# CloudNativeDataPlane/cndp

Measured on AMD Instinct MI355X. Metric: Mpps device-resident parse+hash+LPM, 64B & IMIX, at 1/2/4/8 MI355X, higher is better.
Workload: dtype u32; 1 GPU; C3 l3fwd-graph: 64B IPv4/UDP, 1024-prefix DIR-24-8 LPM + Toeplitz + RSS queue, 16M pkts/GPU device-resident; config=c3, packets_per_gpu=16777216, frame_layout=packed 64-B slots, frame_memory=torch tensor (hipMalloc), ring_batches=4, routes=1024, parallelism=dp1 (replicated FIB, sharded batches), bins_total=32665239552

## Files before the change

__graft_entry__.py:

```python
from __future__ import annotations

import os
import subprocess
import sys

ROOT = os.path.dirname(os.path.abspath(__file__))


def build() -> None:
    env = dict(os.environ)
    env.setdefault("PYTORCH_ROCM_ARCH", "gfx950")
    jobs = str(min(16, os.cpu_count() or 4))
    subprocess.run(["make", "-j", jobs, "-C", os.path.join(ROOT, "cndp_amd", "csrc"), "ARCH=gfx950"],
                   check=True, env=env)
    subprocess.run(["make", "-C", os.path.join(ROOT, "oracle")], check=True, env=env)
    subprocess.run(["make", "-C", os.path.join(ROOT, "tests", "node_harness")], check=True, env=env)
    subprocess.run(["make", "-C", os.path.join(ROOT, "tests", "c_link")], check=True, env=env)
    subprocess.run(["make", "-C", os.path.join(ROOT, "tests", "l4_host")], check=True, env=env)
    subprocess.run(["make", "-C", os.path.join(ROOT, "tests", "tcp_host")], check=True, env=env)
    subprocess.run(["make", "-C", os.path.join(ROOT, "tests", "fwd_host")], check=True, env=env)
    subprocess.run(["make", "-C", os.path.join(ROOT, "tests", "tx_host")], check=True, env=env)
    subprocess.run(["make", "-C", os.path.join(ROOT, "tests", "tcb_host")], check=True, env=env)
    subprocess.run(["make", "-C", os.path.join(ROOT, "tests", "tcpout_host")], check=True, env=env)
    if ROOT not in sys.path:
        sys.path.insert(0, ROOT)
    import cndp_amd
    from cndp_amd import native
    native.lib()
    print(f"built {native.LIB_PATH} ({native.lib().cndp_gpu_version().decode()}); "
          f"cndp_amd {cndp_amd.__version__}")


def smoke() -> None:
    if ROOT not in sys.path:
        sys.path.insert(0, ROOT)
    import numpy as np
    import torch

    from cndp_amd import pktgen
    from cndp_amd.classify import Classifier
    from cndp_amd.fib import Fib, node_ip4_route_add
    from cndp_amd import native as N
    from oracle import oracle as O

    assert torch.cuda.is_available(), "smoke() needs a GPU"
    dev = torch.device("cuda:0")
    routes = pktgen.l3fwd_routes()
    fib = Fib("smoke", N.CNE_FIB_DIR24_8, default_nh=N.IP4_LOOKUP_NEXT_PKT_DROP << 16,
              max_routes=1024, nh_sz=N.CNE_FIB_DIR24_8_4B, num_tbl8=256)
    for ip, d, nh in routes:
        assert node_ip4_route_add(fib, ip, d, nh, N.IP4_LOOKUP_NEXT_REWRITE) == 0
    cl = Classifier(0)
    cl.set_fib(fib)
    n = 1 << 16
    fr = pktgen.packed_ipv4(n, routes=routes, device=dev)
    out = cl.classify(fr, N.CNDP_MODE_L3FWD, n_bins=64)
    torch.cuda.synchronize()

    r4 = [(ip, d, nh) for ip, d, nh in routes]
    t24, t8 = O.dir24_8_build(r4, N.IP4_LOOKUP_NEXT_PKT_DROP << 16, 256)
    ref = O.classify(O.MODE_L3FWD, fr.slab.cpu().numpy(), n, stride=64, tables4=(t24, t8), n_bins=64)
    got = {k: out[k].cpu().numpy() for k in ("nh", "hash", "queue", "edge", "bins")}
    for k, dt in (("nh", np.uint32), ("hash", np.uint32), ("queue", np.uint16), ("edge", np.uint8),
                  ("bins", np.uint64)):
        g = got[k].view(dt) if got[k].dtype != dt else got[k]
        if not np.array_equal(g, ref[k]):
            bad = int(np.sum(g != ref[k]))
            raise AssertionError(f"smoke: {k} differs from the oracle in {bad} places")
    print(f"smoke OK: {n} packets, l3fwd classify on {torch.cuda.get_device_name(0)} == oracle")

    from cndp_amd.l4 import PcbTable, seg_records
    tbl = PcbTable(4)
    assert tbl.add(laddr=0x0A040001, lport=80) == 0
    assert tbl.add(laddr=0x0A040001, lport=80, faddr=0xC6120001, fport=40000) == 1
    m = 64
    ft = pktgen.tcp_socket_frames(m, [((0x0A040001, 80), (0xC6120001, 40000)), ((0x0A040001, 80), (0xC6120002, 7))],
                                  seed=2, cksum=("ok", "ok", "ok", "bad"), flags=(0x02,), payload_lens=(0, 5),
                                  device=dev)
    rx = torch.full((m,), 14 | 20 << 7, dtype=torch.int32, device=dev)
    t = cl.tcp_input(ft, {"rxmeta": rx}, tbl, sel=torch.ones(m, dtype=torch.uint8, device=dev))
    torch.cuda.synchronize()
    raw = ft.slab.cpu().numpy().reshape(m, -1)
    edge, pcb, st = t["l4edge"].cpu().numpy(), t["pcb"].cpu().numpy().view(np.uint32), t["stats"].cpu().numpy()
    seg = seg_records(t["seg"])
    for i in range(m):
        f = raw[i].tobytes()
        l4 = int.from_bytes(f[16:18], "big") - 20
        data = f[26:34] + bytes([0, 6]) + l4.to_bytes(2, "big") + f[34:34 + l4]
        data += b"\0" * (len(data) & 1)
        c = sum(int.from_bytes(data[k:k + 2], "big") for k in range(0, len(data), 2))
        while c >> 16:
            c = (c >> 16) + (c & 0xFFFF)
        want = (0x21, 1 if f[29] == 1 else 0, int.from_bytes(f[38:42], "big")) if c == 0xFFFF else (0x20, 0xFFFFFFFF, 0)
        have = (int(edge[i]), int(pcb[i]), int(seg["seq"][i]))
        if have != want:
            raise AssertionError(f"smoke: tcp_input frame {i}: got {have} want {want}")
    assert st[0] + st[2] == m and st[0] > 0 and st[2] > 0 and st[1] == st[3] == st[4] == 0, st
    print(f"smoke OK: {m} TCP segments, tcp_input: {int(st[0])} to their connection or listener, {int(st[2])} bad checksums")

    from cndp_amd.l4 import TcbTable, opt_records

    def tcp_frame(src, sport, seq, ack, flags, wnd, opts=b"", payload=b""):
        ones = lambda b: sum(int.from_bytes(b[k:k + 2], "big") for k in range(0, len(b), 2)) % 0xFFFF
        seg = bytearray(sport.to_bytes(2, "big") + (80).to_bytes(2, "big") + seq.to_bytes(4, "big") + ack.to_bytes(4, "big")
                        + bytes([(5 + len(opts) // 4) << 4, flags]) + wnd.to_bytes(2, "big") + bytes(4) + opts + payload)
        ip = bytearray(bytes([0x45, 0]) + (20 + len(seg)).to_bytes(2, "big") + bytes(4) + bytes([64, 6, 0, 0])
# ... 105 lines not shown
```

cndp_amd/classify.py:

```python
from __future__ import annotations

import ctypes

import numpy as np

from . import native as N


class Classifier:
    def __init__(self, device: int = -1):
        self._L = N.lib()
        h = ctypes.c_void_p()
        N.check(self._L.cndp_gpu_init(device, ctypes.byref(h)), "cndp_gpu_init")
        self.h = h
        self.device = self._L.cndp_gpu_device(h)
        self.reta_size = 128
        self.fib4 = None
        self.fib6 = None

    def close(self):
        if self.h:
            self._L.cndp_gpu_fini(self.h)
            self.h = None

    def __del__(self):
        try:
            self.close()
        except Exception:
            pass

    def set_rss(self, key: bytes | None = None, reta=None, nb_queues: int = 16):
        rarr = None
        size = 0
        if reta is not None:
            rarr = np.ascontiguousarray(reta, dtype=np.uint16)
            size = len(rarr)
        N.check(self._L.cndp_gpu_set_rss(self.h, key, len(key) if key else 0,
                                         rarr.ctypes.data if rarr is not None else None, size,
                                         nb_queues), "cndp_gpu_set_rss")
        self.reta_size = size or 128

    def set_tuning(self, nt: int | None = None, unroll: int | None = None,
                   blocks_per_cu: int | None = None, tile: int | None = None,
                   dir16: int | None = None, cnet_tile: int | None = None,
                   host_chunk: int | None = None, rw_wb: int | None = None,
                   cnet_spec: int | None = None, load_nt: int | None = None,
                   spec_scan: int | None = None, mbuf_hash: int | None = None,
                   cnet_fold: int | None = None, spec_grid: int | None = None,
                   spec_lists: int | None = None, spec_types: int | None = None,
                   stream_bal: int | None = None, spec_wait: int | None = None,
                   host_window: int | None = None):
        for key, v in ((N.CNDP_TUNE_CNET_FOLD, cnet_fold), (N.CNDP_TUNE_SPEC_GRID, spec_grid),
                       (N.CNDP_TUNE_SPEC_WAIT, spec_wait), (N.CNDP_TUNE_HOST_WINDOW, host_window),
                       (N.CNDP_TUNE_SPEC_LISTS, spec_lists), (N.CNDP_TUNE_SPEC_TYPES, spec_types),
                       (N.CNDP_TUNE_STREAM_BAL, stream_bal),
                       (N.CNDP_TUNE_NT, nt), (N.CNDP_TUNE_UNROLL, unroll),
                       (N.CNDP_TUNE_BLOCKS_PER_CU, blocks_per_cu), (N.CNDP_TUNE_TILE, tile),
                       (N.CNDP_TUNE_DIR16, dir16), (N.CNDP_TUNE_CNET_TILE, cnet_tile),
                       (N.CNDP_TUNE_HOST_CHUNK, host_chunk), (N.CNDP_TUNE_RW_WB, rw_wb),
                       (N.CNDP_TUNE_CNET_SPEC, cnet_spec), (N.CNDP_TUNE_LOAD_NT, load_nt),
                       (N.CNDP_TUNE_SPEC_SCAN, spec_scan), (N.CNDP_TUNE_MBUF_HASH, mbuf_hash)):
            if v is not None:
                N.check(self._L.cndp_gpu_set_tuning(self.h, key, int(v)), "cndp_gpu_set_tuning")

    def stat(self, key: int) -> int:
        self._L.cndp_gpu_get_stat.restype = ctypes.c_int64
        return int(N.check(self._L.cndp_gpu_get_stat(self.h, key), "cndp_gpu_get_stat"))

    def set_fib(self, fib4=None, fib6=None):
        N.check(self._L.cndp_gpu_set_fib(self.h, fib4.h if fib4 else None, fib6.h if fib6 else None),
                "cndp_gpu_set_fib")
        self.fib4, self.fib6 = fib4, fib6

    def alloc_outputs(self, n: int, n_bins: int = 64, device=None, edge: bool = True, meta: bool = False):
        import torch
        dev = device if device is not None else f"cuda:{self.device}"
        out = {
            "nh": torch.empty(n, dtype=torch.int32, device=dev),
            "hash": torch.empty(n, dtype=torch.int32, device=dev),
            "queue": torch.empty(n, dtype=torch.int16, device=dev),
            "edge": torch.empty(n, dtype=torch.uint8, device=dev) if edge else None,
            "bins": torch.zeros(n_bins + 2, dtype=torch.int64, device=dev),
            "n_bins": n_bins,
        }
        if meta:
            out["ptype"] = torch.empty(n, dtype=torch.int32, device=dev)
            out["rxmeta"] = torch.empty(n, dtype=torch.int32, device=dev)
        return out

    @staticmethod
    def _ptr(t):
        return t.data_ptr() if t is not None else None

    def batch(self, frames, mode: int, out: dict, buf_len: int = 1984, offsets_t=None) -> "N.Batch":
        b = N.Batch()
        b.mode = mode
        b.n = frames.n
        b.slab = frames.slab.data_ptr()
        b.slab_len = frames.slab.numel()
        b.stride = frames.stride
        off = offsets_t if offsets_t is not None else frames.offsets
        b.offsets = off.data_ptr() if off is not None else None
        b.data_off = frames.data_off
        b.buf_len = buf_len
        b.nh = self._ptr(out.get("nh"))
        b.hash = self._ptr(out.get("hash"))
        b.queue = self._ptr(out.get("queue"))
        b.edge = self._ptr(out.get("edge"))
        b.bins = self._ptr(out.get("bins"))
        b.n_bins = out.get("n_bins", 64)
        b.ptype = self._ptr(out.get("ptype"))
        b.rxmeta = self._ptr(out.get("rxmeta"))
        return b

    def classify(self, frames, mode: int = N.CNDP_MODE_L3FWD, out: dict | None = None,
                 n_bins: int = 64, buf_len: int = 1984, stream: int | None = None) -> dict:
        import torch
        if out is None:
            out = self.alloc_outputs(frames.n, n_bins, device=frames.slab.device)
        if stream is None:
            stream = torch.cuda.current_stream(frames.slab.device).cuda_stream
        b = self.batch(frames, mode, out, buf_len)
        N.check(self._L.cndp_gpu_classify(self.h, ctypes.byref(b), stream or None), "cndp_gpu_classify")
        return out

    def stream_release(self, stream: int) -> None:
        N.check(self._L.cndp_gpu_stream_release(self.h, stream or None), "cndp_gpu_stream_release")

    @staticmethod
    def _hptr(x):
        if x is None:
            return None
        if isinstance(x, np.ndarray):
            return x.ctypes.data
        return x.data_ptr()

    def classify_host(self, slab, n: int, mode: int, stride: int = 64, offsets=None,
                      data_off: int = 0, buf_len: int = 1984, n_bins: int = 64, out: dict | None = None,
# ... 225 lines not shown
```

cndp_amd/csrc/cndp_gpu.hip:

```cpp

#include <hip/hip_runtime.h>

#include <algorithm>
#include <atomic>
#include <errno.h>
#include <pthread.h>
#include <sched.h>
#include <stdint.h>
#include <stdio.h>
#include <stdlib.h>
#include <string.h>
#include <time.h>
#include <vector>

#include "fib_internal.h"
#include "node_internal.h"
#include "../../include/cndp_gpu.h"
#include "../../include/cndp_l4.h"

#define CNDP_VERSION "cndp_amd 0.1 (gfx950)"

#define HIP_TRY(expr)                                                                            \
    do {                                                                                         \
        hipError_t e_ = (expr);                                                                  \
// ... 56 lines not shown
        e = t8[(e >> 1) * 256u + (ip & 0xffu)];
    return e >> 1;
}

template <typename TP>
__device__ __forceinline__ uint32_t tz4(TP tab, uint32_t b, uint32_t x)
{
    return tab[(b + 0) * 256 + (x & 0xffu)] ^ tab[(b + 1) * 256 + ((x >> 8) & 0xffu)] ^
           tab[(b + 2) * 256 + ((x >> 16) & 0xffu)] ^ tab[(b + 3) * 256 + (x >> 24)];
}

template <typename TP>
__device__ __forceinline__ uint32_t tz4n(TP tab, uint32_t b, uint32_t x)
{
    uint32_t h = 0;
#pragma unroll
    for (uint32_t j = 0; j < 4; j++) {
        const uint32_t v = (x >> (8 * j)) & 0xffu, q = 2 * (b + j);
        h ^= tab[q * 16 + (v >> 4)] ^ tab[(q + 1) * 16 + (v & 15u)];
    }
    return h;
}

#define CNDP_RW_MAX_NH CNDP_IP4_REWRITE_MAX_NH
#define CNDP_RW_MAX_LEN CNDP_IP4_REWRITE_MAX_LEN
#define CNDP_RW_MAX_PORTS CNDP_IP4_REWRITE_MAX_PORTS

typedef uint32_t u32x4 __attribute__((ext_vector_type(4)));
typedef uint32_t u32x4a4 __attribute__((ext_vector_type(4), aligned(4)));
typedef uint32_t u32x3a4 __attribute__((ext_vector_type(3), aligned(4)));
typedef uint32_t u32x2a4 __attribute__((ext_vector_type(2), aligned(4)));
typedef uint32_t u32x2 __attribute__((ext_vector_type(2)));

struct KArgs {
    const uint8_t *slab;
    uint64_t slab_len;
    uint64_t stride;
    const uint64_t *offsets;
    uint32_t data_off;
    uint32_t n;
    uint32_t buf_len;
    uint32_t reta_mask;
    const uint32_t *tbl24;
    const uint32_t *tbl8;
    const uint32_t *tbl24_6;
    const uint32_t *tbl8_6;
    const uint32_t *dir16;
    const uint32_t *pages;
    const uint32_t *ttab;
    const uint16_t *reta;
    uint32_t *nh;
    uint32_t *hash;
    uint16_t *queue;
    uint8_t *edge;
    unsigned long long *bins;
    uint32_t n_bins;
    uint32_t *ptype;
    uint32_t *rxmeta;
    uint32_t *iplen;
    u32x4 *win;
    uint32_t *spec_nh;
    uint32_t *spec_flags;
    uint16_t *spec_t16;
    uint32_t *wl;
    uint32_t *wl_n;
    uint32_t *spec_meta;
    uint8_t *spec_cls;
    uint32_t *spec_ticket;
    uint32_t *spec_bar;
    uint8_t *spec_tile;
    uint32_t *spec_cwl;
    uint32_t *spec_cflag;
    uint32_t *spec_hint;
    uint32_t spec_B;
    uint32_t wl_fold;
    uint32_t tail_lo;
    uint32_t spec_allow;
    uint8_t *spec_c2;
    uint32_t spec_codes;
    uint32_t spec_keep_lo;
    const struct cndp_rw_nh *rw_tbl;
    uint16_t *tx_edge;
    uint32_t rw_parts;
};

#define FAST_THREADS 256
#define SPEC_CH_K 4
#define SPEC_MX 135
#define SPEC_PTRS 151
#define SPEC_ALLOW_LISTS 2u
__device__ __forceinline__ bool nh_ready_rw(uint32_t v) { return v != 0xFFFFFFFFu && (v >> 16) == 0u; }
#define TAB4_POS 12
#define TAB_POS 36
#define TABN_OFF (TAB_POS * 256)
#define TAB_WORDS (TABN_OFF + 2 * TAB_POS * 16)

template <int MODE>
__device__ __forceinline__ uint32_t bin_of(uint32_t nh, uint32_t edge, uint32_t q, uint32_t nb)
{
    if (MODE == CNDP_MODE_HASH)
        return q < nb ? q : nb + 1;
    if (MODE == CNDP_MODE_L3FWD) {
        if (edge == 0)
            return (nh & 0xffffu) < nb ? (nh & 0xffffu) : nb + 1;
        return (edge == 1 || edge == 0xFFu) ? nb : nb + 1;
    }
    if (edge == 1)
        return (nh & 0xffffffu) < nb ? (nh & 0xffffffu) : nb + 1;
    return (edge == 0 || edge == 0x80u) ? nb : nb + 1;
}

__device__ uint32_t hash_v6_global(const uint8_t *p, uint64_t avail, uint32_t ip, bool l4,
                                   const uint32_t *__restrict__ ttab)
{
    const GAS uint32_t *gt = (const GAS uint32_t *)ttab;
    uint32_t h = 0;
    for (uint32_t k = 0; k < 8; k++)
        h ^= tz4(gt, 4 * k, gld32(p, avail, ip + 8 + 4 * k));
    if (l4)
        h ^= tz4(gt, 32, gld32(p, avail, ip + 40));
    return h;
}


template <typename T>
__device__ __forceinline__ GAS T *gp(T *p)
{
    return (GAS T *)p;
}
template <typename T>
__device__ __forceinline__ const GAS T *gp(const T *p)
{
    return (const GAS T *)p;
}

template <bool NT>
__device__ __forceinline__ u32x4 ldg4(const uint8_t *p)
{
    if (NT)
        return __builtin_nontemporal_load(gp((const u32x4 *)p));
    return *gp((const u32x4 *)p);
}
template <bool NT>
__device__ __forceinline__ u32x2 ldg2(const uint8_t *p)
{
    if (NT)
        return __builtin_nontemporal_load(gp((const u32x2 *)p));
    return *gp((const u32x2 *)p);
}
template <bool NT, typename T>
__device__ __forceinline__ void stg(T *p, T v)
{
    if (NT)
        __builtin_nontemporal_store(v, gp(p));
    else
        *p = v;
}

struct FastHdr {
    const uint8_t *p;
    uint64_t avail;
    uint32_t w3, w5, w6, w7, w8, w9;
};

template <bool NT>
__device__ __forceinline__ void fast_load(const KArgs &a, uint64_t i, FastHdr &h)
// ... 415 lines not shown
                nb.hs ^= tz4(s_t, 8, alignb(h.w9, h.w8, 2));
            else
                slow = true;
        }
    }
    if (slow)
        nb.hs = fast_hash<MODE>(a, h, s_t);
    {
        const u32x4 *g = (const u32x4 *)(base + (cn < n_tiles ? cn : n_tiles - 1u) * 4096u);
        r[P][0] = ldg4<LNT>((const uint8_t *)(g + lane));
        r[P][1] = ldg4<LNT>((const uint8_t *)(g + 64 + lane));
        r[P][2] = ldg4<LNT>((const uint8_t *)(g + 128 + lane));
        r[P][3] = ldg4<LNT>((const uint8_t *)(g + 192 + lane));
    }
    if (dD)
        fast_emit<MODE, NTS>(a, cd * 64u + lane, etD, nhD, hsD, s_reta, s_bins, count);
    sd = nd;
    sc = nc;
    sb = nb;
}

template <int MODE, bool NTS, bool LNT>
__global__ __launch_bounds__(FAST_THREADS) void k_classify_stream(KArgs a, uint64_t n_tiles)
{
    __shared__ uint32_t s_t[TAB4_POS * 256];
    __shared__ uint16_t s_reta[CNDP_RETA_MAX];
    __shared__ uint32_t s_bins[CNDP_BINS_MAX + 2];
    __shared__ __attribute__((aligned(16))) u32x4 s_tile[TILE_WAVES][256];

    const uint32_t tid = threadIdx.x;
    for (uint32_t k = tid; k < TAB4_POS * 256; k += FAST_THREADS)
        s_t[k] = a.ttab[k];
    for (uint32_t k = tid; k <= a.reta_mask; k += FAST_THREADS)
        s_reta[k] = a.reta[k];
    const bool count = a.bins != nullptr;
    if (count)
        for (uint32_t k = tid; k < a.n_bins + 2; k += FAST_THREADS)
            s_bins[k] = 0;
    __syncthreads();

    const uint32_t lane = tid & 63u, wv = tid >> 6;
    u32x4 *tile = s_tile[wv];
    const uint8_t *base = a.slab + a.data_off;
    const uint64_t wstep = (uint64_t)gridDim.x * TILE_WAVES;
    const uint64_t t0 = (uint64_t)blockIdx.x * TILE_WAVES + wv;
    const uint64_t nt_w = t0 < n_tiles ? (n_tiles - t0 + wstep - 1) / wstep : 0;
    u32x4 r[2][4];
#pragma unroll
    for (uint32_t s = 0; s < 2; s++) {
        const uint64_t ts = t0 + s * wstep;
        const u32x4 *g = (const u32x4 *)(base + (ts < n_tiles ? ts : n_tiles - 1u) * 4096u);
        r[s][0] = ldg4<LNT>((const uint8_t *)(g + lane));
        r[s][1] = ldg4<LNT>((const uint8_t *)(g + 64 + lane));
        r[s][2] = ldg4<LNT>((const uint8_t *)(g + 128 + lane));
        r[s][3] = ldg4<LNT>((const uint8_t *)(g + 192 + lane));
    }
    StreamLane sb = {0, 0, 0, 0, 0, false}, sc = sb, sd = sb;
    const uint64_t trips = nt_w ? nt_w + 3 : 0;
    for (uint64_t j = 0; j < trips; j += 2) {
        stream_trip<MODE, NTS, LNT, 0>(a, n_tiles, t0 + j * wstep, t0 + (j + 2) * wstep, t0 + (j - 3) * wstep,
                                       j >= 3 && j - 3 < nt_w, lane, tile, r, sb, sc, sd, s_t, s_reta, s_bins, count);
        if (j + 1 < trips)
            stream_trip<MODE, NTS, LNT, 1>(a, n_tiles, t0 + (j + 1) * wstep, t0 + (j + 3) * wstep,
                                           t0 + (j - 2) * wstep, j >= 2 && j - 2 < nt_w, lane, tile, r, sb, sc, sd,
                                           s_t, s_reta, s_bins, count);
    }
    const uint64_t done = n_tiles * 64u;
    for (uint64_t i = done + (uint64_t)blockIdx.x * FAST_THREADS + tid; i < a.n;
         i += (uint64_t)gridDim.x * FAST_THREADS) {
        FastHdr h;
        fast_load<false>(a, i, h);
        fast_finish<MODE, false>(a, i, h, s_t, s_reta, s_bins, count);
    }
    if (count) {
        __syncthreads();
        for (uint32_t k = tid; k < a.n_bins + 2; k += FAST_THREADS)
            if (s_bins[k])
                atomicAdd(&a.bins[k], (unsigned long long)s_bins[k]);
    }
}


#define STREAM_BW 8
template <int MODE, bool NTS, bool LNT>
__global__ __launch_bounds__(STREAM_BW * 64) void k_classify_stream_bal(KArgs a, uint64_t n_tiles)
{
    __shared__ uint32_t s_t[TAB4_POS * 256];
    __shared__ uint16_t s_reta[CNDP_RETA_MAX];
    __shared__ uint32_t s_bins[CNDP_BINS_MAX + 2];
    __shared__ __attribute__((aligned(16))) u32x4 s_tile[STREAM_BW][256];
    __shared__ uint32_t s_next;
    constexpr uint32_t NT = STREAM_BW * 64;

    const uint32_t tid = threadIdx.x;
    for (uint32_t k = tid; k < TAB4_POS * 256; k += NT)
        s_t[k] = a.ttab[k];
    for (uint32_t k = tid; k <= a.reta_mask; k += NT)
        s_reta[k] = a.reta[k];
    const bool count = a.bins != nullptr;
    if (count)
        for (uint32_t k = tid; k < a.n_bins + 2; k += NT)
            s_bins[k] = 0;
    if (tid == 0)
        s_next = 3u * STREAM_BW;
    const uint32_t lane = tid & 63u, wv = tid >> 6;
    u32x4 *tile = s_tile[wv];
    const uint8_t *base = a.slab + a.data_off;
    const uint64_t G = gridDim.x, b = blockIdx.x;
    const uint64_t NONE = ~0ull;
    const uint64_t nk = b < n_tiles ? (n_tiles - b + G - 1) / G : 0;
    auto tile_of = [&](uint64_t k) { return k < nk ? b + k * G : NONE; };
    uint64_t q0 = tile_of(wv), q1 = tile_of(wv + STREAM_BW), q2 = tile_of(wv + 2u * STREAM_BW);
    u32x4 r[2][4];
#pragma unroll
    for (uint32_t s = 0; s < 2; s++) {
        const uint64_t ts = s ? q1 : q0;
        const u32x4 *g = (const u32x4 *)(base + (ts < n_tiles ? ts : n_tiles - 1u) * 4096u);
        r[s][0] = ldg4<LNT>((const uint8_t *)(g + lane));
        r[s][1] = ldg4<LNT>((const uint8_t *)(g + 64 + lane));
        r[s][2] = ldg4<LNT>((const uint8_t *)(g + 128 + lane));
        r[s][3] = ldg4<LNT>((const uint8_t *)(g + 192 + lane));
    }
    __syncthreads();
    auto draw = [&](uint64_t prev) -> uint32_t {
        uint32_t v = 0;
        if (prev != NONE && lane == 0)
            v = atomicAdd(&s_next, 1u);
        return v;
    };
    uint32_t kv = draw(q2);
    uint64_t h1 = NONE, h2 = NONE, h3 = NONE;
    StreamLane sb = {0, 0, 0, 0, 0, false}, sc = sb, sd = sb;
    for (;;) {
        if (q0 == NONE && h1 == NONE && h2 == NONE && h3 == NONE)
            break;
        stream_trip<MODE, NTS, LNT, 0>(a, n_tiles, q0, q2, h3, h3 != NONE, lane, tile, r, sb, sc, sd, s_t, s_reta,
                                       s_bins, count);
        {
            const uint64_t qn = q2 == NONE ? NONE : tile_of(__builtin_amdgcn_readfirstlane(kv));
            kv = draw(qn);
            h3 = h2;
            h2 = h1;
            h1 = q0;
            q0 = q1;
            q1 = q2;
            q2 = qn;
        }
        if (q0 == NONE && h1 == NONE && h2 == NONE && h3 == NONE)
            break;
        stream_trip<MODE, NTS, LNT, 1>(a, n_tiles, q0, q2, h3, h3 != NONE, lane, tile, r, sb, sc, sd, s_t, s_reta,
                                       s_bins, count);
        {
            const uint64_t qn = q2 == NONE ? NONE : tile_of(__builtin_amdgcn_readfirstlane(kv));
            kv = draw(qn);
            h3 = h2;
            h2 = h1;
            h1 = q0;
            q0 = q1;
            q1 = q2;
            q2 = qn;
        }
    }
    const uint64_t done = n_tiles * 64u;
    for (uint64_t i = done + (uint64_t)blockIdx.x * NT + tid; i < a.n; i += (uint64_t)gridDim.x * NT) {
        FastHdr h;
        fast_load<false>(a, i, h);
        fast_finish<MODE, false>(a, i, h, s_t, s_reta, s_bins, count);
    }
    if (count) {
        __syncthreads();
        for (uint32_t k = tid; k < a.n_bins + 2; k += NT)
            if (s_bins[k])
                atomicAdd(&a.bins[k], (unsigned long long)s_bins[k]);
    }
}

#define CNET_THREADS 512
#define WIN_DW 16
#define ROW_DW 17

struct Win {
    const uint32_t *row;
    const uint8_t *g;
    uint64_t avail;
    __device__ __forceinline__ uint32_t ld32(uint32_t o) const
    {
        if (o + 4 <= 64) {
            const uint32_t lo = row[o >> 2], hi = row[(o >> 2) + 1];
            return alignb(hi, lo, o & 3u);
        }
        return gld32(g, avail, o);
    }
    __device__ __forceinline__ uint32_t b8(uint32_t o) const
    {
        return o < 64 ? (row[o >> 2] >> ((o & 3u) * 8)) & 0xffu : gbyte(g, avail, o);
    }
    __device__ __forceinline__ uint32_t raw16(uint32_t o) const { return ld32(o) & 0xffffu; }
    __device__ __forceinline__ uint32_t be16(uint32_t o) const { return bswap16(ld32(o) & 0xffffu); }
    __device__ __forceinline__ uint32_t be32(uint32_t o) const { return bswap32(ld32(o)); }
};

#define BE16C(x) ((uint32_t)((((x) & 0xffu) << 8) | (((x) >> 8) & 0xffu)))

struct Lens {
    uint32_t l2, l3, l4;
};

__device__ __forceinline__ uint32_t pt_l3_ip(uint32_t vihl)
{
    return vihl == 0x45u ? 0x10u : (vihl >= 0x46u && vihl <= 0x4fu) ? 0x30u : 0u;
}
__device__ __forceinline__ uint32_t pt_l4(uint32_t p)
{
    return (p == 17u ? 0x200u : 0u) | (p == 6u ? 0x100u : 0u) | (p == 132u ? 0x400u : 0u);
}
__device__ __forceinline__ bool v6_ext(uint32_t p)
{
    return p == 0u || p == 43u || p == 44u || p == 50u || p == 51u || p == 60u;
}


template <class W>
__device__ int skip_v6_ext(const W &w, uint32_t proto, uint32_t &off, int &frag)
{
    frag = 0;
    for (int i = 0; i < 5; i++) {
        if (proto == 0u || proto == 43u || proto == 60u) {
            const uint32_t x = w.ld32(off);
            proto = x & 0xffu;
            off += (((x >> 8) & 0xffu) + 1u) * 8u;
        } else if (proto == 44u) {
            proto = w.b8(off);
            off += 8;
            frag = 1;
            return (int)proto;
        } else if (proto == 59u) {
            return 0;
        } else {
            return (int)proto;
        }
    }
    return -1;
}

// ... 2751 lines not shown
                s_wave[q] = acc;
                acc += t;
            }
        }
        __syncthreads();
        const uint32_t excl = s_carry + s_wave[wv] + x - v;
        if (k < total) {
            hist[k] = excl;
            if (k % tiles == 0)
                bin_start[k / tiles] = excl;
        }
        __syncthreads();
        if (threadIdx.x == 1023)
            s_carry = excl + v;
        __syncthreads();
    }
    if (threadIdx.x == 0)
        bin_start[nbt] = s_carry;
}

__global__ __launch_bounds__(PART_THREADS) void k_part_scatter(const uint16_t *__restrict__ bin_of,
                                                               uint32_t n, uint32_t nbt,
                                                               uint32_t tiles,
                                                               const uint32_t *__restrict__ off,
                                                               uint32_t *__restrict__ order)
{
    __shared__ uint32_t cur[CNDP_PART_BINS_MAX + 2];
    for (uint32_t k = threadIdx.x; k < nbt; k += PART_THREADS)
        cur[k] = off[(uint64_t)k * tiles + blockIdx.x];
    __syncthreads();
    const uint32_t lane = threadIdx.x & 63u, wv = threadIdx.x >> 6;
    const uint64_t lt_mask = lane ? (~0ULL >> (64 - lane)) : 0ULL;
    const uint32_t t0 = blockIdx.x * PART_TILE;
    for (uint32_t chunk = 0; chunk < PART_TILE; chunk += PART_THREADS) {
        for (uint32_t turn = 0; turn < PART_THREADS / 64u; turn++) {
            if (wv == turn) {
                const uint32_t i = t0 + chunk + threadIdx.x;
                const bool valid = i < n;
                const uint32_t b = valid ? bin_of[i] : 0xFFFFFFFFu;
                uint64_t todo = __ballot(valid);
                uint32_t dst = 0;
                while (todo) {
                    const uint32_t leader = (uint32_t)__builtin_ctzll(todo);
                    const uint32_t lb = __shfl(b, leader, 64);
                    const uint64_t peers = __ballot(valid && b == lb);
                    const uint32_t cnt = (uint32_t)__builtin_popcountll(peers);
                    uint32_t basev = 0;
                    if (lane == leader)
                        basev = cur[lb];
                    basev = __shfl(basev, leader, 64);
                    if (b == lb && valid)
                        dst = basev + (uint32_t)__builtin_popcountll(peers & lt_mask);
                    if (lane == leader)
                        cur[lb] = basev + cnt;
                    todo &= ~peers;
                }
                if (valid)
                    order[dst] = i;
            }
            __syncthreads();
        }
    }
}

#define CNDP_MAX_REGIONS 16
struct cndp_gpu_ctx {
    int dev;
    uint32_t *mq_iplen;
    u32x4 *mq_win;
    uint8_t key[CNDP_RSS_KEY_LEN];
    uint32_t *d_ttab;
    uint16_t *d_reta;
    uint32_t reta_size;
    struct cne_fib *fib4;
    struct cne_fib6 *fib6;
    uint32_t *d_part;
    size_t part_cap;
    int num_cu;
    int tune_nt;
    int tune_unroll;
    int tune_bpc;
    int tune_tile;
    int tune_dir16;
    int tune_cnet_tile;
    int tune_lnt;
    int tune_spec_scan;
    int tune_cnet_fold;
    int tune_spec_grid;
    int tune_spec_wait_us;
    int tune_host_window;
    int tune_spec_lists;
    int sf_clean, wl_clean;
    uint32_t host_chunk;
    int tune_rw_wb;
    uint32_t spec_burst;
    int spec_reset;
    int mbuf_hash;
    hipEvent_t ev_scratch;
    hipStream_t scratch_stream;
    int scratch_used;
    int scratch_armed;
    struct {
        uint8_t *host, *dev;
        uint64_t len;
        int refs;
    } reg[CNDP_MAX_REGIONS];
    int n_reg;
    uint32_t *sp_small;
    uint32_t *cs_wl;
    uint64_t cs_wl_cap;
    uint8_t *sp_class;
    uint32_t *sp_pt, *sp_nh, *sp_S, *sp_T, *sp_U;
    uint8_t *sp_done;
    uint32_t *sp_cwl;
    uint32_t *sp_cflag;
    uint8_t *sp_tile;
    uint8_t *sp_c2;
    int tune_spec_types;
    int tune_stream_bal;
    uint32_t *sp_hint, *sp_hint_d;
    uint64_t sp_n_cap, sp_b_cap;
    hipStream_t hs[3];
    uint8_t *h_slab;
    uint64_t h_slab_cap;
    uint64_t *h_off;
    uint64_t h_off_cap;
    uint8_t *h_out;
    uint64_t h_out_cap;
    uint8_t *m_hwin, *m_dwin;
    uint32_t *m_hres, *m_dres;
    uint32_t m_cap;
    struct cndp_rw_nh rw_tbl[CNDP_RW_MAX_NH];
    uint16_t rw_next[CNDP_RW_MAX_PORTS];
    struct cndp_rw_nh *d_rw_tbl;
    int rw_dirty;
    int rw_local;
    uint64_t rw_gen_seen;
    uint32_t rw_parts;
};

static const uint8_t ms_default_key[CNDP_RSS_KEY_LEN] = {
    0x6d, 0x5a, 0x56, 0xda, 0x25, 0x5b, 0x0e, 0xc2, 0x41, 0x67, 0x25, 0x3d, 0x43, 0xa3,
    0x8f, 0xb0, 0xd0, 0xca, 0x2b, 0xcb, 0xae, 0x7b, 0x30, 0xb4, 0x77, 0xcb, 0x2d, 0xa3,
    0x80, 0x30, 0xf2, 0x0c, 0x6a, 0x42, 0xb7, 0x3b, 0xbe, 0xac, 0x01, 0xfa};

static uint32_t key_window(const uint8_t *key, uint32_t s)
{
    uint64_t v = 0;
    for (uint32_t k = 0; k < 5; k++) {
        const uint32_t byte = s / 8 + k;
        v = (v << 8) | (byte < CNDP_RSS_KEY_LEN ? key[byte] : 0u);
    }
    return (uint32_t)(v >> (8 - (s % 8)));
}

static void build_ttab(const uint8_t *key, uint32_t *tab)
{
    for (uint32_t b = 0; b < TAB_POS; b++) {
        uint32_t wbit[8];
        for (uint32_t k = 0; k < 8; k++)
            wbit[k] = key_window(key, 8 * b + k);
        for (uint32_t v = 0; v < 256; v++) {
            uint32_t h = 0;
            for (uint32_t k = 0; k < 8; k++)
                if (v & (0x80u >> k))
                    h ^= wbit[k];
            tab[b * 256 + v] = h;
        }
    }
    for (uint32_t q = 0; q < 2 * TAB_POS; q++)
        for (uint32_t u = 0; u < 16; u++) {
            uint32_t h = 0;
            for (uint32_t k = 0; k < 4; k++)
                if (u & (0x8u >> k))
                    h ^= key_window(key, 4 * q + k);
            tab[TABN_OFF + q * 16 + u] = h;
        }
}

static int set_device(int dev)
{
    HIP_TRY(hipSetDevice(dev));
    return 0;
}

static int scratch_acquire(cndp_gpu_ctx_t *c, hipStream_t s)
{
    if (c->scratch_used && (c->scratch_armed || s != c->scratch_stream)) {
        if (!c->scratch_armed)
            HIP_TRY(hipEventRecord(c->ev_scratch, c->scratch_stream));
        HIP_TRY(hipStreamWaitEvent(s, c->ev_scratch, 0));
    }
    return 0;
}
static int scratch_release(cndp_gpu_ctx_t *c, hipStream_t s)
{
    c->scratch_stream = s;
    c->scratch_used = 1;
    c->scratch_armed = 0;
    return 0;
}

extern "C" int cndp_gpu_stream_release(cndp_gpu_ctx_t *c, void *stream)
{
    if (!c)
        return -EINVAL;
    if (!c->scratch_used || c->scratch_armed || c->scratch_stream != (hipStream_t)stream)
        return 0;
    int r;
    if ((r = set_device(c->dev)))
        return r;
    HIP_TRY(hipEventRecord(c->ev_scratch, c->scratch_stream));
    c->scratch_armed = 1;
    c->scratch_stream = nullptr;
    return 0;
}

extern "C" int cndp_gpu_init(int device, cndp_gpu_ctx_t **out)
{
    if (!out)
        return -EINVAL;
    *out = nullptr;
    int ndev = 0;
    if (hipGetDeviceCount(&ndev) != hipSuccess || ndev <= 0)
        return -ENODEV;
    if (device < 0)
        HIP_TRY(hipGetDevice(&device));
    if (device >= ndev)
        return -ENODEV;
    int r = set_device(device);
    if (r)
        return r;
    cndp_gpu_ctx_t *c = (cndp_gpu_ctx_t *)calloc(1, sizeof(*c));
    if (!c)
        return -ENOMEM;
    c->dev = device;
    c->tune_nt = 1;
    c->tune_unroll = 1;
    c->tune_bpc = 0;
    c->tune_tile = 1;
    c->tune_dir16 = 1;
    c->tune_cnet_tile = 1;
    c->tune_lnt = 1;
    c->tune_spec_lists = 1;
    c->tune_spec_wait_us = 1000000;
    c->tune_host_window = 1;
    c->host_chunk = 1u << 20;
    c->spec_burst = 256;
    c->tune_rw_wb = 2;
    hipDeviceProp_t prop;
    if (hipGetDeviceProperties(&prop, device) == hipSuccess)
        c->num_cu = prop.multiProcessorCount;
    if (c->num_cu <= 0)
        c->num_cu = 256;
    if (hipMalloc((void **)&c->d_ttab, TAB_WORDS * 4) != hipSuccess ||
        hipMalloc((void **)&c->d_reta, CNDP_RETA_MAX * 2) != hipSuccess ||
        hipEventCreateWithFlags(&c->ev_scratch, hipEventDisableTiming) != hipSuccess) {
        cndp_gpu_fini(c);
        return -ENOMEM;
    }
    r = cndp_gpu_set_rss(c, nullptr, 0, nullptr, 0, 16);
    if (r) {
        cndp_gpu_fini(c);
        return r;
    }
    *out = c;
    return 0;
}

extern "C" void cndp_gpu_fini(cndp_gpu_ctx_t *c)
{
    if (!c)
        return;
    hipSetDevice(c->dev);
    hipDeviceSynchronize();
    while (c->n_reg > 0)
        cndp_gpu_host_unregister(c, c->reg[0].host);
    if (c->ev_scratch)
        hipEventDestroy(c->ev_scratch);
    for (int k = 0; k < 3; k++)
        if (c->hs[k])
            hipStreamDestroy(c->hs[k]);
    if (c->h_slab)
        hipFree(c->h_slab);
    if (c->h_off)
        hipFree(c->h_off);
    if (c->h_out)
        hipFree(c->h_out);
    if (c->m_hwin)
        hipHostFree(c->m_hwin);
    if (c->m_hres)
        hipHostFree(c->m_hres);
    if (c->m_dwin)
        hipFree(c->m_dwin);
    if (c->m_dres)
        hipFree(c->m_dres);
    if (c->d_rw_tbl)
        hipFree(c->d_rw_tbl);
    void *sp[] = {c->sp_small, c->sp_class, c->sp_pt,   c->sp_nh,  c->sp_S,    c->sp_T,
                  c->sp_U,     c->sp_done,  c->sp_tile, c->sp_cwl, c->sp_cflag, c->sp_c2};
    for (void *q : sp)
        if (q)
            hipFree(q);
    if (c->sp_hint)
        hipHostFree(c->sp_hint);
    if (c->d_ttab)
        hipFree(c->d_ttab);
    if (c->d_reta)
        hipFree(c->d_reta);
    if (c->d_part)
        hipFree(c->d_part);
    if (c->cs_wl)
        hipFree(c->cs_wl);
    free(c);
}

extern "C" int cndp_gpu_device(const cndp_gpu_ctx_t *c) { return c ? c->dev : -EINVAL; }

extern "C" int cndp_gpu_set_rss(cndp_gpu_ctx_t *c, const uint8_t *key, uint32_t key_len,
                                const uint16_t *reta, uint32_t reta_size, uint32_t nb_queues)
{
    if (!c)
        return -EINVAL;
    if (key && key_len != CNDP_RSS_KEY_LEN)
        return -EINVAL;
    uint16_t rt[CNDP_RETA_MAX];
    if (reta) {
        if (reta_size == 0 || reta_size > CNDP_RETA_MAX || (reta_size & (reta_size - 1)))
            return -EINVAL;
        memcpy(rt, reta, reta_size * 2);
    } else {
        if (nb_queues == 0)
            return -EINVAL;
        reta_size = 128;
        for (uint32_t i = 0; i < reta_size; i++)
            rt[i] = (uint16_t)(i % nb_queues);
    }
    memcpy(c->key, key ? key : ms_default_key, CNDP_RSS_KEY_LEN);
    uint32_t *tab = (uint32_t *)malloc(TAB_WORDS * 4);
    if (!tab)
        return -ENOMEM;
    build_ttab(c->key, tab);
    int r = set_device(c->dev);
    if (!r && (hipMemcpy(c->d_ttab, tab, TAB_WORDS * 4, hipMemcpyHostToDevice) != hipSuccess ||
               hipMemcpy(c->d_reta, rt, reta_size * 2, hipMemcpyHostToDevice) != hipSuccess))
        r = -EIO;
    free(tab);
    if (!r)
        c->reta_size = reta_size;
    return r;
}

extern "C" int cndp_gpu_set_fib(cndp_gpu_ctx_t *c, struct cne_fib *f4, struct cne_fib6 *f6)
{
    if (!c)
        return -EINVAL;
    if (f4 && f4->t.nh_sz != 2)
        return -ENOTSUP;
    if (f6 && f6->t.nh_sz != 2)
        return -ENOTSUP;
    c->fib4 = f4;
    c->fib6 = f6;
    return 0;
}

extern "C" void cndp_tbl_dev_free(struct cndp_tbl *t)
{
    if (!t)
        return;
    for (uint32_t k = 0; k < CNDP_LK_SLOTS; k++) {
        struct cndp_tbl::cndp_lk_slot &sl = t->lk[k];
        if (sl.stream)
            hipStreamDestroy((hipStream_t)sl.stream);
        if (sl.host)
            hipHostFree(sl.host);
        if (sl.ticket)
            hipFree(sl.ticket);
        memset(&sl, 0, sizeof(sl));
    }
    if (t->paint_host)
        hipHostFree(t->paint_host);
    t->paint_host = nullptr;
    t->paint_cap = 0;
    if (t->dev_id < 0)
        return;
    int cur = 0;
    hipGetDevice(&cur);
    hipSetDevice(t->dev_id);
    if (t->dev_tbl24)
        hipFree(t->dev_tbl24);
    if (t->dev_tbl8)
        hipFree(t->dev_tbl8);
    if (t->dev_dir16)
        hipFree(t->dev_dir16);
    if (t->dev_pages)
        hipFree(t->dev_pages);
    if (t->lk_stream)
        hipStreamDestroy((hipStream_t)t->lk_stream);
    if (t->lk_dbuf)
        hipFree(t->lk_dbuf);
    t->lk_stream = nullptr;
    t->lk_dbuf = nullptr;
    for (uint32_t k = 0; k < t->n_old; k++)
        hipFree(t->dev_old[k]);
    free(t->dev_old);
    t->dev_old = nullptr;
    t->n_old = t->cap_old = 0;
    hipSetDevice(cur);
    t->dev_dir16 = t->dev_pages = nullptr;
    t->dev_cap_pages = 0;
    t->dev_tbl24 = t->dev_tbl8 = nullptr;
    t->dev_id = -1;
    t->dev_groups = 0;
}

static int dir16_page_alloc(struct cndp_tbl *t)
{
    if (t->n_free)
        return (int)t->page_free[--t->n_free];
    if (t->page_hwm == t->cap_pages) {
        const uint32_t ncap = t->cap_pages ? t->cap_pages * 2 : 64;
        uint32_t *np = (uint32_t *)realloc(t->pages, (size_t)ncap * 256 * 4);
        uint32_t *nf = (uint32_t *)realloc(t->page_free, (size_t)ncap * 4);
        if (!np || !nf) {
            if (np)
                t->pages = np;
            if (nf)
                t->page_free = nf;
            return -ENOMEM;
        }
        t->pages = np;
        t->page_free = nf;
        t->cap_pages = ncap;
    }
    return (int)t->page_hwm++;
}

static int dir16_update(struct cndp_tbl *t, uint32_t k0, uint32_t k1)
{
    if (!t->dir16) {
        t->dir16 = (uint32_t *)calloc(65536, 4);
        t->page_of = (int32_t *)malloc(65536 * 4);
        if (!t->dir16 || !t->page_of)
            return -ENOMEM;
        for (uint32_t k = 0; k < 65536; k++)
            t->page_of[k] = -1;
        k0 = 0;
        k1 = 65535;
        t->dd_lo = t->dp_lo = ~0ULL;
        t->dd_hi = t->dp_hi = 0;
    }
    const uint32_t *t24 = (const uint32_t *)t->tbl24;
    for (uint32_t k = k0; k <= k1; k++) {
        const uint32_t *e = t24 + (size_t)k * 256;
        const uint32_t v = e[0];
        bool uni = !(v & 1u);
        for (uint32_t b = 1; uni && b < 256; b++)
            uni = e[b] == v;
        uint32_t nd;
        if (uni) {
            if (t->page_of[k] >= 0) {
                t->page_free[t->n_free++] = (uint32_t)t->page_of[k];
                t->page_of[k] = -1;
                t->n_pages_used--;
            }
            nd = v;
        } else {
            if (t->page_of[k] < 0) {
                const int pg = dir16_page_alloc(t);
                if (pg < 0)
                    return pg;
                t->page_of[k] = pg;
                t->n_pages_used++;
            }
            const uint64_t pe = (uint64_t)t->page_of[k] * 256;
            memcpy(t->pages + pe, e, 256 * 4);
            if (pe < t->dp_lo)
                t->dp_lo = pe;
            if (pe + 256 > t->dp_hi)
                t->dp_hi = pe + 256;
            nd = ((uint32_t)t->page_of[k] << 1) | 1u;
        }
        if (t->dir16[k] != nd || t->dd_hi == 0) {
            t->dir16[k] = nd;
            if (k < t->dd_lo)
                t->dd_lo = k;
            if ((uint64_t)k + 1 > t->dd_hi)
                t->dd_hi = (uint64_t)k + 1;
        }
    }
    return 0;
}

static int tbl_dev_sweep(struct cndp_tbl *t)
{
    if (t->n_old && __atomic_load_n(&t->views, __ATOMIC_ACQUIRE) == 0) {
        const uint32_t n = t->n_old;
        t->n_old = 0;
        for (uint32_t k = 0; k < n; k++)
            HIP_TRY(hipFree(t->dev_old[k]));
    }
    return 0;
}

static int tbl_dev_retire(struct cndp_tbl *t, void *p)
{
    if (!p)
        return 0;
    if (t->n_old == t->cap_old) {
        const uint32_t cap = t->cap_old ? 2 * t->cap_old : 8;
        void **n = (void **)realloc(t->dev_old, cap * sizeof(void *));
        if (!n)
            return -ENOMEM;
        t->dev_old = n;
        t->cap_old = cap;
    }
    t->dev_old[t->n_old++] = p;
    return tbl_dev_sweep(t);
}

static int dir16_sync(struct cndp_tbl *t, hipStream_t s, const struct cndp_range *rg, uint32_t nr)
{
    for (uint32_t k = 0; k < nr || (!t->dir16 && k == 0); k++) {
        const uint64_t lo = k < nr ? rg[k].lo : 0, hi = k < nr ? rg[k].hi : 0;
        if (hi > lo || !t->dir16) {
            int r = dir16_update(t, (uint32_t)(lo >> 8), (uint32_t)((hi ? hi - 1 : 0) >> 8));
            if (r)
                return r;
        }
    }
    if (!t->dev_dir16) {
        HIP_TRY(hipMalloc(&t->dev_dir16, 65536 * 4));
        t->dd_lo = 0;
        t->dd_hi = 65536;
    }
    if (!t->dev_pages || t->dev_cap_pages < t->cap_pages) {
        int r = tbl_dev_retire(t, t->dev_pages);
        if (r)
            return r;
        t->dev_pages = nullptr;
        const uint32_t cap = t->cap_pages > 64 ? t->cap_pages : 64;
        HIP_TRY(hipMalloc(&t->dev_pages, (size_t)cap * 256 * 4));
        t->dev_cap_pages = cap;
        t->dp_lo = 0;
        t->dp_hi = (uint64_t)t->page_hwm * 256;
    }
    if (t->dd_hi > t->dd_lo)
        HIP_TRY(hipMemcpyAsync((uint32_t *)t->dev_dir16 + t->dd_lo, t->dir16 + t->dd_lo,
                               (t->dd_hi - t->dd_lo) * 4, hipMemcpyHostToDevice, s));
    if (t->dp_hi > t->dp_lo)
        HIP_TRY(hipMemcpyAsync((uint32_t *)t->dev_pages + t->dp_lo, t->pages + t->dp_lo,
                               (t->dp_hi - t->dp_lo) * 4, hipMemcpyHostToDevice, s));
    t->dd_lo = t->dp_lo = ~0ULL;
    t->dd_hi = t->dp_hi = 0;
    return 0;
}

struct TblCmd {
    uint64_t first;
    uint32_t count;
    uint32_t op;
    uint64_t arg;
};
#define PAINT_RUN_MIN 8u
#define PAINT_FILL_MAX 65536u

template <typename T>
__global__ __launch_bounds__(256) void k_tbl_paint(const TblCmd *cmds, uint32_t n, const uint8_t *payload, T *t24,
                                                   T *t8)
{
    for (uint32_t c = blockIdx.x; c < n; c += gridDim.x) {
        const TblCmd k = cmds[c];
        T *const dst = ((k.op & 1u) ? t8 : t24) + k.first;
        if (k.op & 2u) {
            const T *const src = (const T *)(payload + k.arg);
            for (uint32_t i = threadIdx.x; i < k.count; i += blockDim.x)
                dst[i] = src[i];
        } else {
            const T v = (T)k.arg;
            for (uint32_t i = threadIdx.x; i < k.count; i += blockDim.x)
                dst[i] = v;
        }
    }
}

static inline uint64_t host_ent(const uint8_t *base, uint32_t nh_sz, uint64_t i)
{
    switch (nh_sz) {
    case 0:
        return base[i];
    case 1:
        return ((const uint16_t *)(const void *)base)[i];
    case 2:
        return ((const uint32_t *)(const void *)base)[i];
    default:
        return ((const uint64_t *)(const void *)base)[i];
    }
}

static uint32_t paint_merge(struct cndp_range *r, uint32_t n)
{
    std::sort(r, r + n, [](const cndp_range &a, const cndp_range &b) { return a.lo < b.lo; });
    uint32_t m = 0;
    for (uint32_t k = 0; k < n; k++) {
        if (m && r[k].lo <= r[m - 1].hi) {
            if (r[k].hi > r[m - 1].hi)
                r[m - 1].hi = r[k].hi;
        } else {
            r[m++] = r[k];
        }
    }
    return m;
}

static void paint_plan(const struct cndp_tbl *t, uint32_t which, const uint8_t *img, const struct cndp_range *r,
                       uint32_t n, std::vector<TblCmd> &cmds, std::vector<uint8_t> &payload)
{
    const uint32_t esz = 1u << t->nh_sz;
    auto copy = [&](uint64_t lo, uint64_t hi) {
        if (hi <= lo)
            return;
        const uint64_t off = (payload.size() + 7u) & ~7ull;
        payload.resize(off + (hi - lo) * esz);
        memcpy(payload.data() + off, img + lo * esz, (hi - lo) * esz);
        for (uint64_t f = lo; f < hi; f += PAINT_FILL_MAX) {
            const uint64_t c = hi - f < PAINT_FILL_MAX ? hi - f : PAINT_FILL_MAX;
            cmds.push_back(TblCmd{f, (uint32_t)c, which | 2u, off + (f - lo) * esz});
        }
    };
    for (uint32_t k = 0; k < n; k++) {
        uint64_t i = r[k].lo, cs = i;
        while (i < r[k].hi) {
            const uint64_t v = host_ent(img, t->nh_sz, i);
            uint64_t j = i + 1;
            while (j < r[k].hi && host_ent(img, t->nh_sz, j) == v)
                j++;
            if (j - i >= PAINT_RUN_MIN) {
                copy(cs, i);
                for (uint64_t f = i; f < j; f += PAINT_FILL_MAX) {
                    const uint64_t c = j - f < PAINT_FILL_MAX ? j - f : PAINT_FILL_MAX;
                    cmds.push_back(TblCmd{f, (uint32_t)c, which, v});
                }
                cs = j;
            }
            i = j;
        }
        copy(cs, r[k].hi);
    }
}

static int tbl_dev_paint(struct cndp_tbl *t, hipStream_t s, bool paint24, bool paint8)
{
    std::vector<TblCmd> cmds;
    std::vector<uint8_t> payload;
    const uint32_t esz = 1u << t->nh_sz;
    if (paint24)
        paint_plan(t, 0, t->tbl24, t->log24, paint_merge(t->log24, t->n_log24), cmds, payload);
    if (paint8)
        paint_plan(t, 1, t->tbl8, t->log8, paint_merge(t->log8, t->n_log8), cmds, payload);
    const uint64_t cmd_bytes = cmds.size() * sizeof(TblCmd), bytes = cmd_bytes + payload.size();
    const uint64_t span = ((paint24 && t->d24_hi > t->d24_lo) ? (t->d24_hi - t->d24_lo) * esz : 0) +
                          ((paint8 && t->d8_hi > t->d8_lo) ? (t->d8_hi - t->d8_lo) * esz : 0);
    if (cmds.empty() || bytes >= span)
        return 0;
    if (bytes > t->paint_cap) {
        if (t->paint_host)
            HIP_TRY(hipHostFree(t->paint_host));
        t->paint_host = nullptr;
        t->paint_cap = 0;
        const uint64_t cap = bytes > (1u << 16) ? bytes + bytes / 2 : (1u << 16);
        HIP_TRY(hipHostMalloc(&t->paint_host, cap, hipHostMallocMapped));
        t->paint_cap = cap;
    }
    uint8_t *h = (uint8_t *)t->paint_host;
    memcpy(h, cmds.data(), cmd_bytes);
    if (!payload.empty())
        memcpy(h + cmd_bytes, payload.data(), payload.size());
    void *hd = nullptr;
    HIP_TRY(hipHostGetDevicePointer(&hd, t->paint_host, 0));
    const TblCmd *dc = (const TblCmd *)hd;
    const uint8_t *dp = (const uint8_t *)hd + cmd_bytes;
    const uint32_t n = (uint32_t)cmds.size(), g = n < 1024u ? n : 1024u;
    switch (t->nh_sz) {
    case 0:
        hipLaunchKernelGGL(k_tbl_paint<uint8_t>, dim3(g), dim3(256), 0, s, dc, n, dp, (uint8_t *)t->dev_tbl24,
                           (uint8_t *)t->dev_tbl8);
        break;
    case 1:
        hipLaunchKernelGGL(k_tbl_paint<uint16_t>, dim3(g), dim3(256), 0, s, dc, n, dp, (uint16_t *)t->dev_tbl24,
                           (uint16_t *)t->dev_tbl8);
        break;
    case 2:
        hipLaunchKernelGGL(k_tbl_paint<uint32_t>, dim3(g), dim3(256), 0, s, dc, n, dp, (uint32_t *)t->dev_tbl24,
                           (uint32_t *)t->dev_tbl8);
        break;
    default:
        hipLaunchKernelGGL(k_tbl_paint<uint64_t>, dim3(g), dim3(256), 0, s, dc, n, dp, (uint64_t *)t->dev_tbl24,
                           (uint64_t *)t->dev_tbl8);
        break;
    }
    HIP_TRY(hipGetLastError());
    t->sync_bytes += bytes;
    t->sync_cmds += n;
    return 1;
}

static int tbl_dev_sync_locked(struct cndp_tbl *t, void *stream)
{
    if (!t || !t->tbl24)
        return -EINVAL;
    int dev = 0;
    if (hipGetDevice(&dev) != hipSuccess)
        return -ENODEV;
    const size_t esz = (size_t)1 << t->nh_sz;
    const uint32_t groups = t->cap_groups + 1;
    if (t->dev_id >= 0 && t->dev_id != dev)
        return -EXDEV;
    int rs = tbl_dev_sweep(t);
    if (rs)
        return rs;
    hipStream_t s = (hipStream_t)stream;
    bool paint24 = t->dev_id >= 0, paint8 = t->dev_id >= 0 && t->dev_groups == groups;
    if (t->dev_id < 0) {
        HIP_TRY(hipMalloc(&t->dev_tbl24, (size_t)CNDP_TBL24_ENT * esz));
        HIP_TRY(hipMalloc(&t->dev_tbl8, (size_t)groups * CNDP_TBL8_GRP * esz));
        t->dev_id = dev;
        t->dev_groups = groups;
        t->d24_lo = 0;
        t->d24_hi = CNDP_TBL24_ENT;
        t->d8_lo = 0;
        t->d8_hi = (uint64_t)groups * CNDP_TBL8_GRP;
    } else if (t->dev_groups != groups) {
        void *n8 = nullptr;
        HIP_TRY(hipMalloc(&n8, (size_t)groups * CNDP_TBL8_GRP * esz));
        int r = tbl_dev_retire(t, t->dev_tbl8);
        if (r) {
            hipFree(n8);
            return r;
        }
        t->dev_tbl8 = n8;
        t->dev_groups = groups;
        t->d8_lo = 0;
        t->d8_hi = (uint64_t)groups * CNDP_TBL8_GRP;
    }
    const char *pe = getenv("CNDP_FIB_PAINT");
    const bool paint_on = !pe || atoi(pe) != 0;
    paint24 = paint_on && paint24 && t->n_log24 <= CNDP_TBL_LOG && t->d24_hi > t->d24_lo;
    if (paint24)
        t->n_log24 = paint_merge(t->log24, t->n_log24);
    paint8 = paint_on && paint8 && t->n_log8 <= CNDP_TBL_LOG && t->d8_hi > t->d8_lo;
    int painted = 0;
    if (paint24 || paint8) {
        painted = tbl_dev_paint(t, s, paint24, paint8);
        if (painted < 0)
            return painted;
    }
    if (t->d24_hi > t->d24_lo && !(painted && paint24)) {
        HIP_TRY(hipMemcpyAsync((uint8_t *)t->dev_tbl24 + t->d24_lo * esz, t->tbl24 + t->d24_lo * esz,
                               (t->d24_hi - t->d24_lo) * esz, hipMemcpyHostToDevice, s));
        t->sync_bytes += (t->d24_hi - t->d24_lo) * esz;
    }
    if (t->d8_hi > t->d8_lo && !(painted && paint8)) {
        HIP_TRY(hipMemcpyAsync((uint8_t *)t->dev_tbl8 + t->d8_lo * esz, t->tbl8 + t->d8_lo * esz,
                               (t->d8_hi - t->d8_lo) * esz, hipMemcpyHostToDevice, s));
        t->sync_bytes += (t->d8_hi - t->d8_lo) * esz;
    }
    const bool has_dir16 = !t->is_trie && t->nh_sz == 2;
    const bool dirty = t->d24_hi > t->d24_lo || t->d8_hi > t->d8_lo || (has_dir16 && !t->dev_dir16);
    if (has_dir16) {
        const struct cndp_range whole = {t->d24_lo, t->d24_hi};
        const bool logged = paint24 && t->dir16;
        int r = dir16_sync(t, s, logged ? t->log24 : &whole, logged ? t->n_log24 : 1u);
        if (r)
            return r;
    }
    if (dirty)
        HIP_TRY(hipStreamSynchronize(s));
    t->d24_lo = t->d8_lo = ~0ULL;
    t->d24_hi = t->d8_hi = 0;
    t->n_log24 = t->n_log8 = 0;
    return 0;
}

extern "C" int cndp_tbl_dev_sync(struct cndp_tbl *t, void *stream)
{
    if (!t || !t->tbl24)
        return -EINVAL;
    pthread_mutex_lock(&t->dev_lock);
    const int r = tbl_dev_sync_locked(t, stream);
    pthread_mutex_unlock(&t->dev_lock);
    return r;
}

static inline uint32_t blocks_for(uint64_t n, uint32_t threads)
{
    return (uint32_t)((n + threads - 1) / threads);
}

struct TblView {
    const void *t24, *t8;
    uint32_t nh_sz;
    const uint32_t *d16, *pages;
};
static inline TblView tbl_view(const struct cndp_tbl *t)
{
    const bool dir = t->dev_dir16 && t->dev_pages;
    return TblView{t->dev_tbl24, t->dev_tbl8, t->nh_sz, dir ? (const uint32_t *)t->dev_dir16 : nullptr,
                   dir ? (const uint32_t *)t->dev_pages : nullptr};
}
static int tbl_acquire(struct cndp_tbl *t, hipStream_t s, TblView *v)
{
    pthread_mutex_lock(&t->dev_lock);
    const int r = tbl_dev_sync_locked(t, s);
    if (!r) {
        *v = tbl_view(t);
        __atomic_add_fetch(&t->views, 1u, __ATOMIC_RELAXED);
    }
    pthread_mutex_unlock(&t->dev_lock);
    return r;
}
static inline void tbl_release(struct cndp_tbl *t)
{
    __atomic_sub_fetch(&t->views, 1u, __ATOMIC_RELEASE);
}
static int tbl_lookup4_launch(TblView v, const uint32_t *ips, uint64_t *nh, uint32_t n, hipStream_t s,
                              LkDone d = LkDone{nullptr, nullptr, 0});
static int tbl_lookup6_launch(TblView v, const uint8_t *ips, uint64_t *nh, uint32_t n, hipStream_t s,
                              LkDone d = LkDone{nullptr, nullptr, 0});

extern "C" int cndp_tbl_lookup4_dev(struct cndp_tbl *t, const uint32_t *ips, uint64_t *nh,
                                    uint32_t n, void *stream)
{
    TblView v{};
    int r = tbl_acquire(t, (hipStream_t)stream, &v);
    if (r)
        return r;
    r = tbl_lookup4_launch(v, ips, nh, n, (hipStream_t)stream);
    tbl_release(t);
    return r;
}

extern "C" int cndp_tbl_lookup6_dev(struct cndp_tbl *t, const uint8_t *ips, uint64_t *nh, uint32_t n,
                                    void *stream)
{
    TblView v{};
    int r = tbl_acquire(t, (hipStream_t)stream, &v);
    if (r)
        return r;
    r = tbl_lookup6_launch(v, ips, nh, n, (hipStream_t)stream);
    tbl_release(t);
    return r;
}

static int tbl_lookup4_launch(TblView v, const uint32_t *ips, uint64_t *nh, uint32_t n, hipStream_t s,
                              LkDone d)
{
    if (n == 0)
        return 0;
    const uint32_t g = blocks_for(n, 256);
    switch (v.nh_sz) {
    case 0:
        hipLaunchKernelGGL(k_lookup4<uint8_t>, dim3(g), dim3(256), 0, s, (const uint8_t *)v.t24,
                           (const uint8_t *)v.t8, ips, nh, n, d);
        break;
    case 1:
        hipLaunchKernelGGL(k_lookup4<uint16_t>, dim3(g), dim3(256), 0, s,
                           (const uint16_t *)v.t24, (const uint16_t *)v.t8, ips, nh, n, d);
        break;
    case 2:
        hipLaunchKernelGGL(k_lookup4<uint32_t>, dim3(g), dim3(256), 0, s,
                           (const uint32_t *)v.t24, (const uint32_t *)v.t8, ips, nh, n, d);
        break;
    default:
        hipLaunchKernelGGL(k_lookup4<uint64_t>, dim3(g), dim3(256), 0, s,
                           (const uint64_t *)v.t24, (const uint64_t *)v.t8, ips, nh, n, d);
        break;
    }
    HIP_TRY(hipGetLastError());
    return 0;
}

static int tbl_lookup6_launch(TblView v, const uint8_t *ips, uint64_t *nh, uint32_t n, hipStream_t s,
                              LkDone d)
{
    if (n == 0)
        return 0;
    const uint32_t g = blocks_for(n, 256);
    switch (v.nh_sz) {
    case 1:
        hipLaunchKernelGGL(k_lookup6<uint16_t>, dim3(g), dim3(256), 0, s,
                           (const uint16_t *)v.t24, (const uint16_t *)v.t8, ips, nh, n, d);
        break;
    case 2:
        hipLaunchKernelGGL(k_lookup6<uint32_t>, dim3(g), dim3(256), 0, s,
                           (const uint32_t *)v.t24, (const uint32_t *)v.t8, ips, nh, n, d);
        break;
// ... 168 lines not shown
{
    return lookup_host_common(t, ips, 16, nh, n, 1);
}

static int validate_batch(const cndp_gpu_ctx_t *c, const struct cndp_batch *b)
{
    if (!c || !b)
        return -EINVAL;
    if (b->mode != CNDP_MODE_L3FWD && b->mode != CNDP_MODE_CNET && b->mode != CNDP_MODE_HASH)
        return -EINVAL;
    if (b->n && !b->slab)
        return -EINVAL;
    if (b->bins && b->n_bins > CNDP_BINS_MAX)
        return -EINVAL;
    if (b->mode != CNDP_MODE_HASH && !c->fib4)
        return -EINVAL;
    if (b->mode == CNDP_MODE_CNET && !c->fib6)
        return -EINVAL;
    return 0;
}

static int spec_scratch(cndp_gpu_ctx_t *c, uint64_t n, uint64_t nb)
{
    if (!c->sp_small) {
        HIP_TRY(hipMalloc((void **)&c->sp_small, 1024 * 4));
        HIP_TRY(hipMemset(c->sp_small, 0, 1024 * 4));
        HIP_TRY(hipMalloc((void **)&c->sp_class, 2048));
        HIP_TRY(hipHostMalloc((void **)&c->sp_hint, 64, hipHostMallocMapped));
        memset(c->sp_hint, 0, 64);
        HIP_TRY(hipHostGetDevicePointer((void **)&c->sp_hint_d, c->sp_hint, 0));
    }
    if (n > c->sp_n_cap) {
        if (c->sp_pt)
            HIP_TRY(hipFree(c->sp_pt));
        if (c->sp_nh)
            HIP_TRY(hipFree(c->sp_nh));
        if (c->sp_tile)
            HIP_TRY(hipFree(c->sp_tile));
        if (c->sp_c2)
            HIP_TRY(hipFree(c->sp_c2));
        c->sp_pt = c->sp_nh = nullptr;
        c->sp_tile = c->sp_c2 = nullptr;
        c->sp_n_cap = 0;
        const uint64_t cap = n + (n >> 3) + 1024;
        HIP_TRY(hipMalloc((void **)&c->sp_pt, cap * 2));
        HIP_TRY(hipMalloc((void **)&c->sp_nh, cap * 4));
        HIP_TRY(hipMalloc((void **)&c->sp_tile, cap / 64 + 1));
        HIP_TRY(hipMalloc((void **)&c->sp_c2, (cap / 64 + 1) * 16));
        c->sp_n_cap = cap;
    }
    if (nb > c->sp_b_cap) {
        if (c->sp_S)
            HIP_TRY(hipFree(c->sp_S));
        if (c->sp_T)
            HIP_TRY(hipFree(c->sp_T));
        if (c->sp_U)
            HIP_TRY(hipFree(c->sp_U));
        if (c->sp_done)
            HIP_TRY(hipFree(c->sp_done));
        if (c->sp_cwl)
            HIP_TRY(hipFree(c->sp_cwl));
        if (c->sp_cflag)
            HIP_TRY(hipFree(c->sp_cflag));
        c->sp_S = c->sp_T = c->sp_U = c->sp_cwl = c->sp_cflag = nullptr;
        c->sp_done = nullptr;
        c->sp_b_cap = 0;
        const uint64_t cap = nb + (nb >> 3) + 64;
        HIP_TRY(hipMalloc((void **)&c->sp_S, cap * 4));
        HIP_TRY(hipMalloc((void **)&c->sp_done, cap));
        HIP_TRY(hipMalloc((void **)&c->sp_cwl, (cap + 1) * 4));
        HIP_TRY(hipMemset(c->sp_cwl, 0, (cap + 1) * 4));
        HIP_TRY(hipMalloc((void **)&c->sp_cflag, cap * 4));
        HIP_TRY(hipMemset(c->sp_cflag, 0, cap * 4));
        const uint64_t ptrs[2] = {(uint64_t)(uintptr_t)c->sp_cwl, (uint64_t)(uintptr_t)c->sp_cflag};
        HIP_TRY(hipMemcpy(c->sp_small + 1 + SPEC_PTRS, ptrs, sizeof(ptrs), hipMemcpyHostToDevice));
        HIP_TRY(hipMalloc((void **)&c->sp_T, cap * SPEC_KMAX * 4));
        HIP_TRY(hipMalloc((void **)&c->sp_U, (cap * SPEC_KMAX + (cap / SPEC_BLK + 2) * (SPEC_KMAX + 1)) * 4));
        c->sp_b_cap = cap;
    }
    return 0;
}

static int classify_cnet(cndp_gpu_ctx_t *c, const struct cndp_batch *b, KArgs &a, hipStream_t s);
static int classify_l3(cndp_gpu_ctx_t *c, const struct cndp_batch *b, KArgs &a, hipStream_t s, uint16_t *rw_tx,
                       bool *fused);

static int classify_launch(cndp_gpu_ctx_t *c, const struct cndp_batch *b, void *stream, uint16_t *rw_tx,
                           bool *fused, const TblView *v4, const TblView *v6);

static int classify_impl(cndp_gpu_ctx_t *c, const struct cndp_batch *b, void *stream, uint16_t *rw_tx,
                         bool *fused)
{
    int r = validate_batch(c, b);
    if (r)
        return r;
    r = set_device(c->dev);
    if (r)
        return r;
    struct cndp_tbl *t4 = b->mode != CNDP_MODE_HASH ? &c->fib4->t : nullptr;
    struct cndp_tbl *t6 = b->mode == CNDP_MODE_CNET ? &c->fib6->t : nullptr;
    TblView v4{}, v6{};
    if (t4 && (r = tbl_acquire(t4, (hipStream_t)stream, &v4)))
        return r;
    if (t6 && (r = tbl_acquire(t6, (hipStream_t)stream, &v6))) {
        tbl_release(t4);
        return r;
    }
    r = b->n ? classify_launch(c, b, stream, rw_tx, fused, t4 ? &v4 : nullptr, t6 ? &v6 : nullptr) : 0;
    if (t4)
        tbl_release(t4);
    if (t6)
        tbl_release(t6);
    return r;
}

static int classify_launch(cndp_gpu_ctx_t *c, const struct cndp_batch *b, void *stream, uint16_t *rw_tx,
                           bool *fused, const TblView *v4, const TblView *v6)
{
    int r;
    KArgs a;
    memset(&a, 0, sizeof(a));
    a.slab = (const uint8_t *)b->slab;
    a.slab_len = b->slab_len;
    a.stride = b->stride;
    a.offsets = b->offsets;
    a.data_off = b->data_off;
    a.n = b->n;
    a.buf_len = b->buf_len;
    a.reta_mask = c->reta_size - 1;
    if (v4) {
        a.tbl24 = (const uint32_t *)v4->t24;
        a.tbl8 = (const uint32_t *)v4->t8;
        if (c->tune_dir16 && v4->d16) {
            a.dir16 = v4->d16;
            a.pages = v4->pages;
        }
    }
    if (v6) {
        a.tbl24_6 = (const uint32_t *)v6->t24;
        a.tbl8_6 = (const uint32_t *)v6->t8;
    }
    a.ttab = c->d_ttab;
    a.reta = c->d_reta;
    a.nh = b->nh;
    a.hash = b->hash;
    a.queue = b->queue;
    a.edge = b->edge;
    a.bins = (unsigned long long *)b->bins;
    a.n_bins = b->n_bins;
    a.ptype = b->ptype;
    a.rxmeta = b->mode == CNDP_MODE_CNET ? b->rxmeta : nullptr;
    a.iplen = b->mode == CNDP_MODE_CNET && b->rxmeta ? c->mq_iplen : nullptr;
    a.win = b->mode == CNDP_MODE_CNET && b->rxmeta ? c->mq_win : nullptr;
    hipStream_t s = (hipStream_t)stream;
    if (b->mode == CNDP_MODE_CNET) {
        if ((r = scratch_acquire(c, s)))
            return r;
        r = classify_cnet(c, b, a, s);
        const int r2 = scratch_release(c, s);
        return r ? r : r2;
    }
    return classify_l3(c, b, a, s, rw_tx, fused);
}

static int classify_cnet(cndp_gpu_ctx_t *c, const struct cndp_batch *b, KArgs &a, hipStream_t s)
{
    int r;
    {
        uint32_t g = blocks_for(b->n, CNET_THREADS);
        const uint32_t cap = (uint32_t)c->num_cu * 2u;
        if (g > cap)
            g = cap;
        const uint32_t B = c->spec_burst;
        if (B && (r = spec_scratch(c, b->n, ((uint64_t)b->n + B - 1) / B)))
            return r;
        if (c->spec_reset && c->sp_small) {
            HIP_TRY(hipMemsetAsync(c->sp_small, 0, 4, s));
            c->spec_reset = 0;
        }
        if (B) {
            a.spec_t16 = (uint16_t *)c->sp_pt;
            a.spec_nh = c->sp_nh;
            a.spec_flags = c->sp_small + 66;
            if (!c->sf_clean)
                HIP_TRY(hipMemsetAsync(a.spec_flags, 0, 64 * 4, s));
            c->sf_clean = 0;
            a.spec_meta = c->sp_small + 1;
            a.spec_cls = c->sp_class;
            a.spec_ticket = c->sp_small + 512;
            a.spec_bar = c->sp_small + 142;
            a.spec_B = B;
            a.spec_allow = c->tune_spec_scan == 0 ? 1u : 0u;
            a.spec_hint = c->sp_hint_d;
        }
        if (c->tune_cnet_tile && b->n < (1u << 30)) {
            if ((uint64_t)b->n + 1 > c->cs_wl_cap) {
                if (c->cs_wl)
                    HIP_TRY(hipFree(c->cs_wl));
                c->cs_wl = nullptr;
                c->cs_wl_cap = 0;
                const uint64_t wcap = (uint64_t)b->n + (b->n >> 3) + 1024;
                HIP_TRY(hipMalloc((void **)&c->cs_wl, wcap * 4));
                c->cs_wl_cap = wcap;
                c->wl_clean = 0;
            }
            a.wl_n = c->cs_wl;
            a.wl = c->cs_wl + 1;
            if (!c->wl_clean)
                HIP_TRY(hipMemsetAsync(a.wl_n, 0, 4, s));
            c->wl_clean = 0;
            const uint64_t n_tiles = ((uint64_t)b->n + 63u) / 64u;
            const bool bal = c->tune_lnt && (c->tune_stream_bal == 2 || (c->tune_stream_bal == 0 && !b->offsets));
            const uint32_t nthr = bal ? CD_BAL_THREADS : CT_THREADS;
            uint64_t gd = (n_tiles + nthr / 64u - 1) / (nthr / 64u);
            const uint32_t bpc = c->tune_bpc ? (uint32_t)c->tune_bpc : bal ? 1u : 2u;
            if (gd > (uint64_t)c->num_cu * bpc)
                gd = (uint64_t)c->num_cu * bpc;
            static void (*const dfns[2][2][2])(KArgs, uint32_t) = {
                {{k_cnet_defer<false, false, false, false>, k_cnet_defer<false, false, false, false>},
                 {k_cnet_defer<false, true, false, false>, k_cnet_defer<false, true, false, false>}},
                {{k_cnet_defer<true, false, false, false>, k_cnet_defer<true, false, true, false>},
                 {k_cnet_defer<true, true, false, false>, k_cnet_defer<true, true, true, false>}}};
            static void (*const bfns[2][2])(KArgs, uint32_t) = {
                {k_cnet_defer<true, false, false, true>, k_cnet_defer<true, false, true, true>},
                {k_cnet_defer<true, true, false, true>, k_cnet_defer<true, true, true, true>}};
            const bool meta_out = a.ptype != nullptr || a.rxmeta != nullptr;
            a.spec_tile = B ? c->sp_tile : nullptr;
            if (B && B <= 256 && (B & 3u) == 0 && c->tune_spec_lists && c->tune_spec_scan == 0) {
                a.spec_cwl = c->sp_cwl;
                a.spec_cflag = c->sp_cflag;
                a.spec_allow |= SPEC_ALLOW_LISTS;
            }
            a.wl_fold = 0;
            const bool fold = c->tune_cnet_fold == 1 ||
                              (c->tune_cnet_fold == 0 && c->sp_hint && ((volatile uint32_t *)c->sp_hint)[0] == 0u);
            if (B && fold) {
                const uint64_t nb = ((uint64_t)b->n + B - 1) / B;
                const uint64_t t0 = nb > SPEC_TAIL ? (nb - SPEC_TAIL) * B : 0;
                a.wl_fold = 1;
                a.tail_lo = (uint32_t)t0;
            }
            if (a.spec_tile && B <= 256) {
                const uint64_t nb = ((uint64_t)b->n + B - 1) / B;
                a.spec_c2 = c->sp_c2;
                a.spec_keep_lo = nb > SPEC_TAIL ? (uint32_t)((nb - SPEC_TAIL) * B) : 0u;
                a.spec_codes = c->tune_spec_types == 2 ||
                               (c->tune_spec_types == 0 && c->sp_hint && ((volatile uint32_t *)c->sp_hint)[1]);
            }
            if (!c->tune_lnt)
                a.spec_codes = 0;
            hipLaunchKernelGGL(bal ? bfns[meta_out ? 1 : 0][a.spec_codes ? 1 : 0]
                                   : dfns[c->tune_lnt ? 1 : 0][meta_out ? 1 : 0][a.spec_codes ? 1 : 0],
                               dim3((uint32_t)gd), dim3(nthr), 0, s, a, (uint32_t)n_tiles);
            if (!a.wl_fold)
                hipLaunchKernelGGL(k_classify_cnet<true>, dim3(g), dim3(CNET_THREADS), 0, s, a);
            if (a.spec_codes)
                hipLaunchKernelGGL(k_spec_expand, dim3((uint32_t)c->num_cu * 2u), dim3(256), 0, s, a,
                                   (uint32_t)n_tiles, (const uint32_t *)(c->sp_small + 1));
        } else {
            hipLaunchKernelGGL(k_classify_cnet<false>, dim3(g), dim3(CNET_THREADS), 0, s, a);
        }
        if (B) {
            const uint64_t nb = ((uint64_t)b->n + B - 1) / B;
            uint32_t *state = c->sp_small, *meta = c->sp_small + 1;
            uint32_t *ticket = c->sp_small + 140;
            c->sf_clean = 1;
            c->wl_clean = a.wl_n != nullptr;
            const uint32_t gw = (uint32_t)((nb + 3) / 4);
            const uint32_t kfast = c->tune_spec_scan == 0 ? SPEC_KFAST : 0u;
            const uint32_t kmax = c->tune_spec_scan == 2 ? 0u : SPEC_KMAX;
            if (B <= 256) {
                const uint64_t nch = (nb + SPEC_CH - 1) / SPEC_CH;
                const uint32_t gated = c->tune_spec_scan == 0 ? 1u : 0u;
                const uint64_t nblk = (nch + SPEC_BLK - 1) / SPEC_BLK;
                uint32_t *P = c->sp_U, *Bt = c->sp_U + nch * SPEC_KMAX, *Sblk = Bt + nblk * SPEC_KMAX;
                if (gated && a.spec_tile) {
                    uint32_t gl = (uint32_t)((nch + 4 * SPEC_LQ - 1) / (4 * SPEC_LQ));
                    const bool shrink = c->tune_spec_grid == 1 ||
                                        (c->tune_spec_grid == 0 && c->sp_hint && ((volatile uint32_t *)c->sp_hint)[1]);
                    const uint32_t cap = c->tune_spec_grid == 1 ? 2u : (uint32_t)c->num_cu * 4u;
                    if (shrink && gl > cap)
                        gl = cap;
                    hipLaunchKernelGGL(k_spec_local_t<SPEC_CH>, dim3(gl), dim3(256), 0, s, a, B, nb, nch, meta,
                                       c->sp_done);
                } else if (gated) {
                    auto lo = k_spec_local<SPEC_CH, SPEC_WPB>;
                    const uint32_t gl = (uint32_t)((nch + SPEC_WPB - 1) / SPEC_WPB);
                    hipLaunchKernelGGL(lo, dim3(gl), dim3(SPEC_WPB * 64), 0, s, a, B, nb, nch, meta, c->sp_done);
                }
                hipLaunchKernelGGL(k_spec_fallback<SPEC_CH>, dim3((uint32_t)c->num_cu), dim3(256), 0, s, a, B, nb,
                                   nch, meta, (const uint8_t *)c->sp_class, c->sp_T, P, Bt, Sblk, c->sp_S,
                                   (const uint8_t *)c->sp_done, a.spec_bar, kfast, kmax, gated,
                                   c->tune_spec_wait_us < 0 ? 0u : (uint32_t)c->tune_spec_wait_us * 100u);
            } else {
                hipLaunchKernelGGL(k_spec_tables, dim3(gw), dim3(256), 0, s, (const uint16_t *)a.spec_t16, b->n, B,
                                   nb, (const uint32_t *)meta, (const uint8_t *)c->sp_class, c->sp_T);
                const uint64_t nblk = (nb + SPEC_BLK - 1) / SPEC_BLK;
                uint32_t *P = c->sp_U, *Bt = c->sp_U + nb * SPEC_KMAX, *Sblk = Bt + nblk * SPEC_KMAX;
                hipLaunchKernelGGL(k_spec_scan, dim3((uint32_t)nblk), dim3(SPEC_BLK), 0, s, nb,
                                   (const uint32_t *)meta, (const uint32_t *)c->sp_T, P, Bt,
                                   (const uint8_t *)c->sp_class, Sblk, state, ticket,
                                   (const uint16_t *)a.spec_t16, b->n, B, nb, c->sp_S, kfast, kmax, 0u);
                hipLaunchKernelGGL(k_spec_emit, dim3(gw), dim3(256), 0, s, a, B, nb, kfast, kmax,
                                   (const uint32_t *)meta, (const uint8_t *)c->sp_class, (const uint32_t *)P,
                                   (const uint32_t *)Sblk, (const uint32_t *)c->sp_S);
            }
        }
    }
    HIP_TRY(hipGetLastError());
    return 0;
}

static int classify_l3(cndp_gpu_ctx_t *c, const struct cndp_batch *b, KArgs &a, hipStream_t s, uint16_t *rw_tx,
                       bool *fused)
{
    {
        uint32_t g = blocks_for(b->n, FAST_THREADS);
        const uint32_t bpc = c->tune_bpc ? (uint32_t)c->tune_bpc : !rw_tx ? 2u : 4u;
        const uint32_t cap = (uint32_t)c->num_cu * bpc;
        if (g > cap)
            g = cap;
        const uint64_t n_tiles = b->n / 64u;
        const bool tile_ok = c->tune_tile && !b->offsets && b->stride == 64 &&
                             (((uintptr_t)b->slab + b->data_off) & 15u) == 0 && n_tiles > 0 &&
                             b->data_off + n_tiles * 4096u <= b->slab_len;
        const int mi = b->mode == CNDP_MODE_L3FWD ? 0 : 1, nti = c->tune_nt ? 1 : 0, li = c->tune_lnt ? 1 : 0;
        if (tile_ok) {
            uint32_t gt = (uint32_t)((n_tiles + TILE_WAVES - 1) / TILE_WAVES);
            if (gt > cap)
                gt = cap;
            typedef void (*tile_fn)(KArgs, uint64_t);
            if (rw_tx && b->mode == CNDP_MODE_L3FWD && b->n % 256u == 0 && c->d_rw_tbl) {
                static const tile_fn rfns[2][2] = {
                    {k_classify_tile<CNDP_MODE_L3FWD, 2, false, true, false>,
                     k_classify_tile<CNDP_MODE_L3FWD, 2, false, true, true>},
                    {k_classify_tile<CNDP_MODE_L3FWD, 2, true, true, false>,
                     k_classify_tile<CNDP_MODE_L3FWD, 2, true, true, true>}};
                a.rw_tbl = c->d_rw_tbl;
                a.tx_edge = rw_tx;
                a.rw_parts = c->tune_rw_wb == 1 ? 4u : c->tune_rw_wb == 2 ? 5u : c->rw_parts;
                *fused = true;
                hipLaunchKernelGGL(rfns[nti][li], dim3(gt), dim3(FAST_THREADS), 0, s, a, n_tiles);
                HIP_TRY(hipGetLastError());
                return 0;
            }
            if (c->tune_stream_bal != 1) {
                static const tile_fn bfns[2][2][2] = {
                    {{k_classify_stream_bal<CNDP_MODE_L3FWD, false, false>,
                      k_classify_stream_bal<CNDP_MODE_L3FWD, false, true>},
                     {k_classify_stream_bal<CNDP_MODE_L3FWD, true, false>,
                      k_classify_stream_bal<CNDP_MODE_L3FWD, true, true>}},
                    {{k_classify_stream_bal<CNDP_MODE_HASH, false, false>,
                      k_classify_stream_bal<CNDP_MODE_HASH, false, true>},
                     {k_classify_stream_bal<CNDP_MODE_HASH, true, false>,
                      k_classify_stream_bal<CNDP_MODE_HASH, true, true>}}};
                uint32_t gb = (uint32_t)c->num_cu * (c->tune_bpc ? (uint32_t)c->tune_bpc : 1u);
                if ((uint64_t)gb > n_tiles)
                    gb = (uint32_t)n_tiles;
                hipLaunchKernelGGL(bfns[mi][nti][li], dim3(gb), dim3(STREAM_BW * 64), 0, s, a, n_tiles);
                HIP_TRY(hipGetLastError());
                return 0;
            }
            static const tile_fn sfns[2][2][2] = {
                {{k_classify_stream<CNDP_MODE_L3FWD, false, false>, k_classify_stream<CNDP_MODE_L3FWD, false, true>},
                 {k_classify_stream<CNDP_MODE_L3FWD, true, false>, k_classify_stream<CNDP_MODE_L3FWD, true, true>}},
                {{k_classify_stream<CNDP_MODE_HASH, false, false>, k_classify_stream<CNDP_MODE_HASH, false, true>},
                 {k_classify_stream<CNDP_MODE_HASH, true, false>, k_classify_stream<CNDP_MODE_HASH, true, true>}}};
            hipLaunchKernelGGL(sfns[mi][nti][li], dim3(gt), dim3(FAST_THREADS), 0, s, a, n_tiles);
            HIP_TRY(hipGetLastError());
            return 0;
        }
        typedef void (*fast_fn)(KArgs);
        static const fast_fn ffns[2][2] = {{k_classify_fast<CNDP_MODE_L3FWD, false, 1>, k_classify_fast<CNDP_MODE_L3FWD, true, 1>},
                                           {k_classify_fast<CNDP_MODE_HASH, false, 1>, k_classify_fast<CNDP_MODE_HASH, true, 1>}};
        hipLaunchKernelGGL(ffns[mi][nti], dim3(g), dim3(FAST_THREADS), 0, s, a);
    }
    HIP_TRY(hipGetLastError());
    return 0;
}

static bool spec_err_take(cndp_gpu_ctx_t *c)
{
    if (!c->sp_hint || !__atomic_load_n(&c->sp_hint[SPEC_HINT_ERR], __ATOMIC_ACQUIRE))
        return false;
    __atomic_store_n(&c->sp_hint[SPEC_HINT_ERR], 0u, __ATOMIC_RELAXED);
    c->spec_reset = 1;
    return true;
}

extern "C" int cndp_gpu_classify(cndp_gpu_ctx_t *c, const struct cndp_batch *b, void *stream)
{
    if (c && b && b->mode == CNDP_MODE_CNET && spec_err_take(c))
        return -EIO;
    return classify_impl(c, b, stream, nullptr, nullptr);
}

static int grow(void **buf, uint64_t *cap, uint64_t need)
{
    if (*cap >= need && *buf)
        return 0;
    if (*buf)
        HIP_TRY(hipFree(*buf));
    *buf = nullptr;
    *cap = 0;
    const uint64_t sz = need + (need >> 3) + 4096;
    HIP_TRY(hipMalloc(buf, sz));
    *cap = sz;
    return 0;
}

#define CNDP_HOST_SEG (64ull << 20)
#define CNDP_HOST_REACH (16ull << 10)
#define CNDP_HOST_WIN 64ull

extern "C" int cndp_gpu_classify_host(cndp_gpu_ctx_t *c, const struct cndp_batch *hb)
{
    int r = validate_batch(c, hb);
    if (r)
        return r;
    if ((r = set_device(c->dev)))
        return r;
    const uint64_t n = hb->n;
    const uint64_t o_nh = 0, o_hash = o_nh + n * 4, o_q = o_hash + n * 4, o_e = o_q + ((n * 2 + 15) & ~15ull),
                   o_b = o_e + ((n + 15) & ~15ull), o_pt = o_b + ((uint64_t)hb->n_bins + 2) * 8,
                   o_rm = o_pt + n * 4, out_bytes = o_rm + n * 4;
    for (int k = 0; k < 3; k++)
// ... 2104 lines not shown
    MqSlot *op = &q->slot[q->open];
    if (op->state == MQ_OPEN && op->n) {
        const uint64_t age = now_ns() - op->t_open_ns, dmax = (uint64_t)q->conf.max_delay_us * 1000u;
        const bool idle = q->in_flight == 0 && (op->n >= q->conf.batch / 2u || age >= dmax / 2u);
        if (idle || age >= dmax) {
            const int r = mq_launch(q);
            if (r)
                q->err = r;
        }
    }
    uint32_t got = 0;
    while (got < max) {
        const uint32_t hi = q->head;
        MqSlot *sl = &q->slot[hi];
        if (sl->state == MQ_FLIGHT) {
            if (__atomic_load_n(&q->flags[hi * 16u], __ATOMIC_ACQUIRE) != sl->seq)
                break;
            sl->state = MQ_DONE;
            q->in_flight--;
            if (q->conf.mode == CNDP_MQ_CNET && spec_err_take(q->c)) {
                sl->failed = 1;
                uint16_t *ed = (uint16_t *)(sl->h + q->h_edge);
                for (uint32_t i = 0; i < sl->n; i++)
                    ed[i] = (uint16_t)MQ_EDGE_NONE;
                q->err = -EIO;
            }
        }
        if (sl->state != MQ_DONE)
            break;
        const uint32_t take = sl->n - sl->polled < max - got ? sl->n - sl->polled : max - got;
        if (!sl->failed)
            mq_writeback(q, sl, sl->polled, sl->polled + take);
        memcpy(mbufs + got, sl->mb + sl->polled, (size_t)take * sizeof(void *));
        memcpy(edges + got, (const uint16_t *)(sl->h + q->h_edge) + sl->polled, (size_t)take * 2);
        sl->polled += take;
        got += take;
        q->pending -= take;
        if (sl->polled == sl->n) {
            sl->state = MQ_FREE;
            q->head = (q->head + 1) % q->conf.depth;
        }
    }
    return (int)got;
}

extern "C" int64_t cndp_gpu_mq_stat(const cndp_gpu_mq_t *q, int key)
{
    if (!q)
        return -EINVAL;
    switch (key) {
    case CNDP_MQ_STAT_BATCHES:
        return (int64_t)q->n_batches;
    case CNDP_MQ_STAT_MBUFS:
        return (int64_t)q->n_mbufs;
    default:
        return -EINVAL;
    }
}

#define CNDP_MQ_WAIT_S 30
extern "C" int cndp_gpu_mq_wait(cndp_gpu_mq_t *q)
{
    if (!q)
        return -EINVAL;
    const uint32_t hi = q->head;
    MqSlot *sl = &q->slot[hi];
    if (sl->state != MQ_FLIGHT)
        return 0;
    const uint64_t t0 = now_ns();
    for (uint32_t spin = 0; __atomic_load_n(&q->flags[hi * 16u], __ATOMIC_ACQUIRE) != sl->seq; spin++) {
        if ((spin & 255u) == 255u) {
            if (now_ns() - t0 > CNDP_MQ_WAIT_S * 1000000000ull)
                return -ETIMEDOUT;
            sched_yield();
        } else {
            __builtin_ia32_pause();
        }
    }
    return 0;
}

extern "C" int64_t cndp_gpu_get_stat(cndp_gpu_ctx_t *c, int key)
{
    if (!c || (key != CNDP_STAT_CNET_WORKLIST && key != CNDP_STAT_CNET_UNIFORM && key != CNDP_STAT_SPEC_ERR))
        return -EINVAL;
    if (!c->sp_hint)
        return 0;
    return ((volatile uint32_t *)c->sp_hint)[key == CNDP_STAT_CNET_WORKLIST ? 0
                                             : key == CNDP_STAT_CNET_UNIFORM ? 1
                                                                             : SPEC_HINT_ERR];
}

extern "C" int cndp_gpu_set_tuning(cndp_gpu_ctx_t *c, int key, int value)
{
    if (!c)
        return -EINVAL;
    switch (key) {
    case CNDP_TUNE_NT:
        c->tune_nt = value ? 1 : 0;
        return 0;
    case CNDP_TUNE_UNROLL:
        if (value != 1)
            return -EINVAL;
        c->tune_unroll = value;
        return 0;
    case CNDP_TUNE_BLOCKS_PER_CU:
        if (value < 0 || value > 64)
            return -EINVAL;
        c->tune_bpc = value;
        return 0;
    case CNDP_TUNE_TILE:
        if (value < 0 || value > 1)
            return -EINVAL;
        c->tune_tile = value;
        return 0;
    case CNDP_TUNE_DIR16:
        c->tune_dir16 = value ? 1 : 0;
        return 0;
    case CNDP_TUNE_CNET_TILE:
        if (value < 0 || value > 1)
            return -EINVAL;
        c->tune_cnet_tile = value;
        return 0;
    case CNDP_TUNE_LOAD_NT:
        c->tune_lnt = value ? 1 : 0;
        return 0;
    case CNDP_TUNE_SPEC_SCAN:
        if (value < 0 || value > 2)
            return -EINVAL;
        c->tune_spec_scan = value;
        return 0;
    case CNDP_TUNE_RW_WB:
        if (value < 0 || value > 2)
            return -EINVAL;
        c->tune_rw_wb = value;
        return 0;
    case CNDP_TUNE_CNET_SPEC:
        if (value < 0)
            return -EINVAL;
        c->spec_burst = (uint32_t)value;
        c->spec_reset = 1;
        return 0;
    case CNDP_TUNE_MBUF_HASH:
        c->mbuf_hash = value ? 1 : 0;
        return 0;
    case CNDP_TUNE_CNET_FOLD:
        if (value < 0 || value > 2)
            return -EINVAL;
        c->tune_cnet_fold = value;
        return 0;
    case CNDP_TUNE_SPEC_GRID:
        if (value < 0 || value > 2)
            return -EINVAL;
        c->tune_spec_grid = value;
        return 0;
    case CNDP_TUNE_SPEC_LISTS:
        if (value < 0 || value > 1)
            return -EINVAL;
        c->tune_spec_lists = value;
        return 0;
    case CNDP_TUNE_SPEC_TYPES:
        if (value < 0 || value > 2)
            return -EINVAL;
        c->tune_spec_types = value;
        return 0;
    case CNDP_TUNE_STREAM_BAL:
        if (value < 0 || value > 2)
            return -EINVAL;
        c->tune_stream_bal = value;
        return 0;
    case CNDP_TUNE_HOST_WINDOW:
        c->tune_host_window = value ? 1 : 0;
        return 0;
    case CNDP_TUNE_SPEC_WAIT:
        if (value == 0 || value < -1 || value > 40000000)
            return -EINVAL;
        c->tune_spec_wait_us = value;
        return 0;
    case CNDP_TUNE_HOST_CHUNK:
        if (value < 1024)
            return -EINVAL;
        c->host_chunk = (uint32_t)value;
        return 0;
    default:
        return -EINVAL;
    }
}

#if CD_STAMP
extern "C" int cndp_gpu_debug_stamps(unsigned long long *out, uint32_t n)
{
    if (n > CD_STAMP_WAVES * 16)
        n = CD_STAMP_WAVES * 16;
    HIP_TRY(hipDeviceSynchronize());
    HIP_TRY(hipMemcpyFromSymbol(out, HIP_SYMBOL(cd_stamps), (size_t)n * 8));
    return 0;
}

extern "C" int cndp_gpu_debug_spec_stamps(unsigned long long *out, uint32_t n)
{
    if (n > SP_STAMP_BLOCKS * 16 + 8)
        n = SP_STAMP_BLOCKS * 16 + 8;
    HIP_TRY(hipDeviceSynchronize());
    HIP_TRY(hipMemcpyFromSymbol(out, HIP_SYMBOL(sp_stamps), (size_t)n * 8));
    return 0;
}
#endif

extern "C" const char *cndp_gpu_version(void) { return CNDP_VERSION; }
```

cndp_amd/csrc/fib.c:

```c
#include "fib_internal.h"

#include <errno.h>
#include <stdio.h>
#include <stdlib.h>
#include <string.h>

typedef unsigned __int128 u128;

static inline uint64_t ent_get(const struct cndp_tbl *t, const uint8_t *base, uint64_t i)
{
    switch (t->nh_sz) {
    case 0:
        return base[i];
    case 1:
        return ((const uint16_t *)(const void *)base)[i];
    case 2:
        return ((const uint32_t *)(const void *)base)[i];
    default:
        return ((const uint64_t *)(const void *)base)[i];
    }
}

static inline void ent_set(struct cndp_tbl *t, uint8_t *base, uint64_t i, uint64_t v)
{
// ... 25 lines not shown
            return;
        }
    }
    if (*n < CNDP_TBL_LOG) {
        log[*n].lo = lo;
        log[*n].hi = hi;
    }
    (*n)++;
}

static inline void dirty24(struct cndp_tbl *t, uint64_t lo, uint64_t hi)
{
    if (lo < t->d24_lo)
        t->d24_lo = lo;
    if (hi > t->d24_hi)
        t->d24_hi = hi;
    log_range(t->log24, &t->n_log24, lo, hi);
}

static inline void dirty8(struct cndp_tbl *t, uint64_t lo, uint64_t hi)
{
    if (lo < t->d8_lo)
        t->d8_lo = lo;
    if (hi > t->d8_hi)
        t->d8_hi = hi;
    log_range(t->log8, &t->n_log8, lo, hi);
}

static inline uint64_t t24_get(const struct cndp_tbl *t, uint64_t i) { return ent_get(t, t->tbl24, i); }
static inline void t24_set(struct cndp_tbl *t, uint64_t i, uint64_t v)
{
    ent_set(t, t->tbl24, i, v);
    dirty24(t, i, i + 1);
}
static inline uint64_t t8_get(const struct cndp_tbl *t, uint64_t i) { return ent_get(t, t->tbl8, i); }
static inline void t8_set(struct cndp_tbl *t, uint64_t i, uint64_t v)
{
    ent_set(t, t->tbl8, i, v);
    dirty8(t, i, i + 1);
}

static int tbl_init(struct cndp_tbl *t, uint32_t nh_sz, uint32_t is_trie, uint32_t num_tbl8,
                    uint64_t def_nh)
{
    memset(t, 0, sizeof(*t));
    pthread_mutex_init(&t->dev_lock, NULL);
    t->def_nh = def_nh;
    t->nh_sz = nh_sz;
    t->is_trie = is_trie;
    t->num_tbl8 = num_tbl8;
    t->cap_groups = num_tbl8 ? num_tbl8 : 64;
    t->dev_id = -1;
    size_t esz = (size_t)1 << nh_sz;
    t->tbl24 = malloc((size_t)CNDP_TBL24_ENT * esz);
    t->tbl8 = calloc((size_t)(t->cap_groups + 1) * CNDP_TBL8_GRP, esz);
    t->used = calloc((t->cap_groups + 63) / 64, sizeof(uint64_t));
    if (!t->tbl24 || !t->tbl8 || !t->used) {
        free(t->tbl24);
        free(t->tbl8);
        free(t->used);
        pthread_mutex_destroy(&t->dev_lock);
        return -ENOMEM;
    }
    uint64_t v = def_nh << 1;
    for (uint64_t i = 0; i < CNDP_TBL24_ENT; i++)
        ent_set(t, t->tbl24, i, v);
    t->d24_lo = 0;
    t->d24_hi = CNDP_TBL24_ENT;
    t->d8_lo = 0;
    t->d8_hi = (uint64_t)(t->cap_groups + 1) * CNDP_TBL8_GRP;
    return 0;
}

static void tbl_fini(struct cndp_tbl *t)
{
    cndp_tbl_dev_free(t);
    free(t->tbl24);
    free(t->tbl8);
    free(t->used);
    free(t->dir16);
    free(t->page_of);
    free(t->pages);
    free(t->page_free);
    pthread_mutex_destroy(&t->dev_lock);
    memset(t, 0, sizeof(*t));
}

static int grow_pool(struct cndp_tbl *t)
{
    uint32_t ncap = t->cap_groups * 2;
    size_t esz = (size_t)1 << t->nh_sz;
    uint8_t *n8 = realloc(t->tbl8, (size_t)(ncap + 1) * CNDP_TBL8_GRP * esz);
    if (!n8)
        return -ENOMEM;
    memset(n8 + (size_t)(t->cap_groups + 1) * CNDP_TBL8_GRP * esz, 0,
           (size_t)(ncap - t->cap_groups) * CNDP_TBL8_GRP * esz);
    t->tbl8 = n8;
    uint64_t *nu = realloc(t->used, ((ncap + 63) / 64) * sizeof(uint64_t));
    if (!nu)
        return -ENOMEM;
    memset(nu + (t->cap_groups + 63) / 64, 0,
           (((ncap + 63) / 64) - (t->cap_groups + 63) / 64) * sizeof(uint64_t));
    t->used = nu;
    dirty8(t, (uint64_t)(t->cap_groups + 1) * CNDP_TBL8_GRP, (uint64_t)(ncap + 1) * CNDP_TBL8_GRP);
    t->cap_groups = ncap;
    return 0;
}

static int group_alloc(struct cndp_tbl *t)
{
    for (;;) {
        uint32_t words = (t->cap_groups + 63) / 64;
        for (uint32_t w = 0; w < words; w++) {
            if (t->used[w] == ~0ULL)
                continue;
            uint32_t b = (uint32_t)__builtin_ctzll(~t->used[w]);
            uint32_t g = w * 64 + b;
            if (g >= t->cap_groups)
                break;
            t->used[w] |= 1ULL << b;
            t->cur_tbl8s++;
            return (int)g;
        }
        if (t->num_tbl8)
            return -ENOSPC;
        if (grow_pool(t))
            return -ENOMEM;
    }
}

static void group_free(struct cndp_tbl *t, uint64_t g)
{
    uint64_t base = g * CNDP_TBL8_GRP;
    memset(t->tbl8 + (base << t->nh_sz), 0, (size_t)CNDP_TBL8_GRP << t->nh_sz);
    dirty8(t, base, base + CNDP_TBL8_GRP);
    t->used[g / 64] &= ~(1ULL << (g % 64));
    t->cur_tbl8s--;
}

static void trie_free_chain(struct cndp_tbl *t, uint64_t e)
{
    if (!(e & 1u))
        return;
    uint64_t g = e >> 1;
    for (uint32_t k = 0; k < CNDP_TBL8_GRP; k++)
        trie_free_chain(t, t8_get(t, g * CNDP_TBL8_GRP + k));
    group_free(t, g);
}

static int group_uniform(const struct cndp_tbl *t, uint64_t g, uint64_t *v)
{
    uint64_t base = g * CNDP_TBL8_GRP;
    uint64_t first = t8_get(t, base);
    if (t->is_trie && (first & 1u))
        return 0;
    for (uint32_t k = 1; k < CNDP_TBL8_GRP; k++)
        if (t8_get(t, base + k) != first)
            return 0;
    *v = first;
    return 1;
}

static int dir24_install(struct cndp_tbl *t, uint32_t p, uint32_t len, uint64_t nh)
{
    if (len <= 24) {
        uint64_t first = p >> 8, cnt = 1ull << (24 - len);
// ... 809 lines not shown
```

cndp_amd/csrc/fib_internal.h:

```cpp
#ifndef CNDP_FIB_INTERNAL_H
#define CNDP_FIB_INTERNAL_H

#include <pthread.h>
#include <stddef.h>
#include <stdint.h>

#include "rib.h"
#include "../../include/cndp_fib.h"

#ifdef __cplusplus
extern "C" {
#endif

#define CNDP_TBL24_ENT (1u << 24)
#define CNDP_TBL8_GRP 256u
#define CNDP_LK_SLOTS 16u
#define CNDP_TBL_LOG 1024u

struct cndp_range {
    uint64_t lo, hi;
};

struct cndp_tbl {
    uint32_t nh_sz;
    uint32_t is_trie;
    uint8_t *tbl24;
    uint8_t *tbl8;
    uint64_t *used;
    uint32_t num_tbl8;
    uint32_t cap_groups;
    uint32_t cur_tbl8s;
    uint64_t d24_lo, d24_hi, d8_lo, d8_hi;
    struct cndp_range log24[CNDP_TBL_LOG], log8[CNDP_TBL_LOG];
    uint32_t n_log24, n_log8;
    uint64_t sync_bytes;
    uint64_t sync_cmds;
    void *paint_host;
    uint64_t paint_cap;
    int dev_id;
    void *dev_tbl24;
    void *dev_tbl8;
    uint32_t dev_groups;
    uint32_t *dir16;
    int32_t *page_of;
    uint32_t *pages;
    uint32_t cap_pages;
    uint32_t *page_free;
    uint32_t n_free, n_pages_used, page_hwm;
    uint64_t dd_lo, dd_hi;
    uint64_t dp_lo, dp_hi;
    void *dev_dir16;
    void *dev_pages;
    uint32_t dev_cap_pages;
    uint64_t def_nh;
    pthread_mutex_t dev_lock;
    struct cndp_lk_slot {
        int busy;
        void *stream;
        uint8_t *host;
        uint8_t *hdev;
        uint32_t *ticket;
        uint32_t seq;
    } lk[CNDP_LK_SLOTS];
    void *lk_stream;
    uint8_t *lk_dbuf;
    void **dev_old;
    uint32_t n_old, cap_old;
    uint32_t views;
};

struct cne_fib {
    char name[64];
    enum cne_fib_type type;
    uint64_t def_nh;
    int lookup_type;
    uint32_t rsvd_tbl8s;
    struct cndp_rib rib;
    struct cndp_tbl t;
};

struct cne_fib6 {
    char name[64];
    enum cne_fib_type type;
    uint64_t def_nh;
    int lookup_type;
    uint32_t rsvd_tbl8s;
    struct cndp_rib rib;
    struct cndp_tbl t;
};

int cndp_tbl_dev_sync(struct cndp_tbl *t, void *stream);
void cndp_tbl_dev_free(struct cndp_tbl *t);
int cndp_tbl_lookup4_host(struct cndp_tbl *t, const uint32_t *ips, uint64_t *nh, uint32_t n);
int cndp_tbl_lookup6_host(struct cndp_tbl *t, const uint8_t *ips16, uint64_t *nh, uint32_t n);
int cndp_tbl_lookup4_dev(struct cndp_tbl *t, const uint32_t *ips, uint64_t *nh, uint32_t n,
                         void *stream);
int cndp_tbl_lookup6_dev(struct cndp_tbl *t, const uint8_t *ips16, uint64_t *nh, uint32_t n,
                         void *stream);

#ifdef __cplusplus
}
#endif
#endif
```

cndp_amd/fib.py:

```python
from __future__ import annotations

import ctypes

import numpy as np

from . import native as N


def _conf(type_, default_nh, max_routes, nh_sz, num_tbl8):
    c = N.FibConf()
    c.type = type_
    c.default_nh = default_nh
    c.max_routes = max_routes
    c.dir24_8.nh_sz = nh_sz
    c.dir24_8.num_tbl8 = num_tbl8
    return c


class Fib:

    def __init__(self, name="fib", type=N.CNE_FIB_DIR24_8, default_nh=0, max_routes=1024,
                 nh_sz=N.CNE_FIB_DIR24_8_4B, num_tbl8=256, lookup=None):
        self._L = N.lib()
        conf = _conf(type, default_nh, max_routes, nh_sz, num_tbl8)
        self.h = self._L.cne_fib_create(name.encode() if name is not None else None,
                                        ctypes.byref(conf))
        if not self.h:
            raise ValueError("cne_fib_create rejected the configuration")
        self.type = type
        self.default_nh = default_nh
        if lookup is not None:
            N.check(self.select_lookup(lookup), "cne_fib_select_lookup")

    @staticmethod
    def create_raw(name, conf: "N.FibConf"):
        return N.lib().cne_fib_create(name, ctypes.byref(conf) if conf is not None else None)

    def close(self):
        if self.h:
            self._L.cne_fib_free(self.h)
            self.h = None

    def __del__(self):
        try:
            self.close()
        except Exception:
            pass

    def add(self, ip: int, depth: int, nh: int) -> int:
        return self._L.cne_fib_add(self.h, ip & 0xFFFFFFFF, depth, nh)

    def delete(self, ip: int, depth: int) -> int:
        return self._L.cne_fib_delete(self.h, ip & 0xFFFFFFFF, depth)

    def lookup_bulk(self, ips) -> np.ndarray:
        ips = np.ascontiguousarray(ips, dtype=np.uint32)
        out = np.zeros(len(ips), dtype=np.uint64)
        N.check(self._L.cne_fib_lookup_bulk(self.h, ips.ctypes.data, out.ctypes.data, len(ips)),
                "cne_fib_lookup_bulk")
        return out

    def lookup_dev(self, ips_ptr: int, out_ptr: int, n: int, stream: int = 0) -> None:
        N.check(self._L.cndp_fib_lookup_dev(self.h, ips_ptr, out_ptr, n, stream or None),
                "cndp_fib_lookup_dev")

    def select_lookup(self, t: int) -> int:
        return self._L.cne_fib_select_lookup(self.h, t)

    def sync(self, stream: int = 0) -> None:
        N.check(self._L.cndp_fib_sync(self.h, stream or None), "cndp_fib_sync")

    def image(self):
        im = N.FibImage()
        N.check(self._L.cndp_fib_image(self.h, ctypes.byref(im)), "cndp_fib_image")
        dt = {0: np.uint8, 1: np.uint16, 2: np.uint32, 3: np.uint64}[im.nh_sz]
        esz = 1 << im.nh_sz
        t24 = np.ctypeslib.as_array((ctypes.c_uint8 * ((1 << 24) * esz)).from_address(im.tbl24))
        t8 = np.ctypeslib.as_array((ctypes.c_uint8 * (im.tbl8_groups * 256 * esz)).from_address(im.tbl8))
        return t24.view(dt), t8.view(dt)

    def stats(self):
        r, u, s = ctypes.c_uint32(), ctypes.c_uint32(), ctypes.c_uint32()
        N.check(self._L.cndp_fib_stats(self.h, ctypes.byref(r), ctypes.byref(u), ctypes.byref(s)),
                "cndp_fib_stats")
        return {"routes": r.value, "tbl8_used": u.value, "rsvd_tbl8s": s.value}


class Fib6:

    def __init__(self, name="fib6", type=N.CNE_FIB_TRIE, default_nh=0, max_routes=1024,
                 nh_sz=N.CNE_FIB_TRIE_4B, num_tbl8=1 << 15, lookup=None):
        self._L = N.lib()
        conf = _conf(type, default_nh, max_routes, nh_sz, num_tbl8)
        self.h = self._L.cne_fib6_create(name.encode() if name is not None else None,
                                         ctypes.byref(conf))
        if not self.h:
            raise ValueError("cne_fib6_create rejected the configuration")
        self.type = type
        self.default_nh = default_nh
        if lookup is not None:
            N.check(self.select_lookup(lookup), "cne_fib6_select_lookup")

    @staticmethod
    def create_raw(name, conf):
        return N.lib().cne_fib6_create(name, ctypes.byref(conf) if conf is not None else None)

    def close(self):
        if self.h:
            self._L.cne_fib6_free(self.h)
            self.h = None

    def __del__(self):
        try:
            self.close()
        except Exception:
            pass

    @staticmethod
    def _ip(ip) -> bytes:
        if isinstance(ip, int):
            return ip.to_bytes(16, "big")
        b = bytes(ip)
        assert len(b) == 16
        return b

    def add(self, ip, depth: int, nh: int) -> int:
        return self._L.cne_fib6_add(self.h, self._ip(ip), depth, nh)

    def delete(self, ip, depth: int) -> int:
        return self._L.cne_fib6_delete(self.h, self._ip(ip), depth)

    def lookup_bulk(self, ips) -> np.ndarray:
        ips = np.ascontiguousarray(ips, dtype=np.uint8).reshape(-1, 16)
        out = np.zeros(len(ips), dtype=np.uint64)
        N.check(self._L.cne_fib6_lookup_bulk(self.h, ips.ctypes.data, out.ctypes.data, len(ips)),
                "cne_fib6_lookup_bulk")
        return out

    def lookup_dev(self, ips_ptr: int, out_ptr: int, n: int, stream: int = 0) -> None:
        N.check(self._L.cndp_fib6_lookup_dev(self.h, ips_ptr, out_ptr, n, stream or None),
                "cndp_fib6_lookup_dev")

    def select_lookup(self, t: int) -> int:
        return self._L.cne_fib6_select_lookup(self.h, t)

    def sync(self, stream: int = 0) -> None:
        N.check(self._L.cndp_fib6_sync(self.h, stream or None), "cndp_fib6_sync")

    def image(self):
        im = N.FibImage()
        N.check(self._L.cndp_fib6_image(self.h, ctypes.byref(im)), "cndp_fib6_image")
        dt = {1: np.uint16, 2: np.uint32, 3: np.uint64}[im.nh_sz]
        esz = 1 << im.nh_sz
        t24 = np.ctypeslib.as_array((ctypes.c_uint8 * ((1 << 24) * esz)).from_address(im.tbl24))
        t8 = np.ctypeslib.as_array((ctypes.c_uint8 * (im.tbl8_groups * 256 * esz)).from_address(im.tbl8))
        return t24.view(dt), t8.view(dt)

    def stats(self):
        r, u, s = ctypes.c_uint32(), ctypes.c_uint32(), ctypes.c_uint32()
        N.check(self._L.cndp_fib6_stats(self.h, ctypes.byref(r), ctypes.byref(u), ctypes.byref(s)),
                "cndp_fib6_stats")
        return {"routes": r.value, "tbl8_used": u.value, "rsvd_tbl8s": s.value}

# ... 37 lines not shown
```

cndp_amd/native.py:

```python
from __future__ import annotations

import ctypes
import os
from ctypes import (POINTER, Structure, Union, c_char_p, c_int, c_uint8, c_uint16,
                    c_uint32, c_uint64, c_void_p)

HERE = os.path.dirname(os.path.abspath(__file__))
LIB_PATH = os.environ.get("CNDP_GPU_LIB") or os.path.join(HERE, "lib", "libcndp_gpu.so")

CNE_FIB_DUMMY, CNE_FIB_DIR24_8, CNE_FIB_TRIE = 0, 1, 2
CNE_FIB_DIR24_8_1B, CNE_FIB_DIR24_8_2B, CNE_FIB_DIR24_8_4B, CNE_FIB_DIR24_8_8B = 0, 1, 2, 3
CNE_FIB_TRIE_2B, CNE_FIB_TRIE_4B, CNE_FIB_TRIE_8B = 1, 2, 3
(CNE_FIB_LOOKUP_DEFAULT, CNE_FIB_LOOKUP_DIR24_8_SCALAR_MACRO, CNE_FIB_LOOKUP_DIR24_8_SCALAR_INLINE,
 CNE_FIB_LOOKUP_DIR24_8_SCALAR_UNI, CNE_FIB_LOOKUP_DIR24_8_VECTOR_AVX512, CNE_FIB_LOOKUP_TRIE_SCALAR,
 CNE_FIB_LOOKUP_TRIE_VECTOR_AVX512, CNE_FIB_LOOKUP_GPU) = range(8)
CNE_FIB_MAXDEPTH = 32
CNE_FIB6_MAXDEPTH = 128

CNDP_MODE_L3FWD, CNDP_MODE_CNET, CNDP_MODE_HASH = 0, 1, 2
CNDP_NH_INVALID = 0xFFFFFFFF
CNDP_EDGE_CLS_DROP = 0xFF
CNDP_RSS_KEY_LEN = 40
CNDP_RETA_MAX = 512
CNDP_BINS_MAX = 1024
CNDP_PART_BINS_MAX = 4096
CNDP_FRAMES_CACHED = 1
CNDP_TUNE_NT, CNDP_TUNE_UNROLL, CNDP_TUNE_BLOCKS_PER_CU, CNDP_TUNE_TILE, CNDP_TUNE_DIR16 = 1, 2, 3, 4, 5
CNDP_TUNE_CNET_TILE = 6
CNDP_TUNE_HOST_CHUNK = 7
CNDP_TUNE_RW_WB = 8
CNDP_TUNE_CNET_SPEC = 9
CNDP_TUNE_LOAD_NT = 10
CNDP_TUNE_SPEC_SCAN = 11
CNDP_STAT_CNET_WORKLIST, CNDP_STAT_CNET_UNIFORM, CNDP_STAT_SPEC_ERR = 1, 2, 3
CNDP_TUNE_MBUF_HASH = 12
CNDP_TUNE_CNET_FOLD = 13
CNDP_TUNE_SPEC_GRID = 14
CNDP_TUNE_SPEC_LISTS = 15
CNDP_TUNE_SPEC_TYPES = 16
CNDP_TUNE_STREAM_BAL = 17
CNDP_TUNE_SPEC_WAIT = 18
CNDP_TUNE_HOST_WINDOW = 19
CNDP_MQ_IP4_LOOKUP, CNDP_MQ_CNET, CNDP_MQ_MAC_SWAP, CNDP_MQ_IP4_REWRITE = 0, 1, 2, 3
CNDP_MQ_F_HASH, CNDP_MQ_F_NO_METADATA, CNDP_MQ_F_DEVICE_HEADERS, CNDP_MQ_F_RX_PARSE = 1, 2, 4, 8
CNDP_MQ_F_REWRITE = 16
CNDP_MQ_F_HOST_WRITEBACK = 1 << 5
CNDP_MQ_EDGE_NONE = 0xFFFF
CNDP_MQ_EDGE_CLS_DROP = 0xFFFE
CNDP_MQ_EDGE_LOOKUP_DROP = 0xFFFD
CNDP_MQ_STAT_BATCHES, CNDP_MQ_STAT_MBUFS = 1, 2
CNDP_MQ_NODE_PTYPE, CNDP_MQ_NODE_IP4, CNDP_MQ_NODE_IP6 = 0, 1, 2
CNDP_MBUF_EDGE_CLS_DROP = 0xFFFF

IP4_LOOKUP_NEXT_REWRITE, IP4_LOOKUP_NEXT_PKT_DROP = 0, 1
IP4_INPUT_NEXT_PKT_DROP, IP4_INPUT_NEXT_FORWARD, IP4_INPUT_NEXT_PROTO = 0, 1, 2

CNDP_PCB_MAX_ENTRIES = 4096
CNDP_PCB_NONE = 0xFFFFFFFF
CNDP_UDP_CHKSUM_FLAG = 0x0080
CNDP_L4_NODE_IP4_PROTO, CNDP_L4_NODE_UDP_INPUT = 0, 1
CNDP_L4_EDGE_NONE = 0xFF
CNDP_IP4_PROTO_DROP, CNDP_IP4_PROTO_TCP = 0, 2
CNDP_UDP_INPUT_PKT_DROP, CNDP_UDP_INPUT_CHNL_RECV, CNDP_UDP_INPUT_PKT_PUNT = 0, 1, 2
CNDP_L4_STAT_RECV, CNDP_L4_STAT_NOMATCH, CNDP_L4_STAT_CKSUM, CNDP_L4_STAT_PROTO_DROP = 0, 1, 2, 3

CNDP_L4_NODE_TCP_INPUT = 2
CNDP_TCP_INPUT_PKT_DROP, CNDP_TCP_INPUT_SEGMENT, CNDP_TCP_INPUT_PKT_PUNT = 0, 1, 2
(CNDP_TCP_STAT_SEGMENT, CNDP_TCP_STAT_NOMATCH, CNDP_TCP_STAT_CKSUM, CNDP_TCP_STAT_BADOFF,
 CNDP_TCP_STAT_RSVD) = range(5)
CNDP_TCP_NSTATS = 5

(CNDP_TCPS_FREE, CNDP_TCPS_CLOSED, CNDP_TCPS_LISTEN, CNDP_TCPS_SYN_SENT, CNDP_TCPS_SYN_RCVD, CNDP_TCPS_ESTABLISHED,
 CNDP_TCPS_CLOSE_WAIT, CNDP_TCPS_FIN_WAIT_1, CNDP_TCPS_CLOSING, CNDP_TCPS_LAST_ACK, CNDP_TCPS_FIN_WAIT_2,
 CNDP_TCPS_TIME_WAIT) = range(12)
CNDP_TCB_REASS_EMPTY = 1
CNDP_SEG_TS_PRESENT, CNDP_SEG_MSS_PRESENT, CNDP_SEG_WS_PRESENT, CNDP_SEG_SACK_PERMIT = 0x8000, 0x4000, 0x2000, 0x1000
CNDP_SEG_REQ_SCALE = 0x000F
(CNDP_TCPSEG_NONE, CNDP_TCPSEG_RESET, CNDP_TCPSEG_CLOSED, CNDP_TCPSEG_BADOPT, CNDP_TCPSEG_SLOW,
 CNDP_TCPSEG_PRED_ACK, CNDP_TCPSEG_PRED_DATA, CNDP_TCPSEG_PRED_NONE) = range(8)
CNDP_TCPSEG_NSTATS = 8
CNDP_TCPSEG_VERDICT, CNDP_TCPSEG_TS_UPDATE, CNDP_TCPSEG_FIRST = 0x0F, 0x40, 0x80

CNDP_TCBF_REQ_SCALE, CNDP_TCBF_RCVD_SCALE, CNDP_TCBF_REQ_TSTAMP, CNDP_TCBF_RCVD_TSTAMP = 0x01, 0x02, 0x04, 0x08
CNDP_TCPOUT_SEGMENT, CNDP_TCPOUT_RESPOND = 0, 1
(CNDP_TCPOUT_STAT_SENT, CNDP_TCPOUT_STAT_NOTSEL, CNDP_TCPOUT_STAT_NOPCB, CNDP_TCPOUT_STAT_NOLADDR,
 CNDP_TCPOUT_STAT_TOOBIG, CNDP_TCPOUT_STAT_RST_IN, CNDP_TCPOUT_STAT_MCAST, CNDP_TCPOUT_STAT_OPTS) = range(8)
CNDP_TCPOUT_NSTATS = 8

CNDP_FWD_OBJS_MAX = 1 << 24
CNDP_FWD_NETIFS = 256
CNDP_FWD_NONE = 0xFFFFFFFF
CNDP_FWD_EDGE_PKT_DROP, CNDP_FWD_EDGE_ARP_REQUEST, CNDP_FWD_EDGE_OUTPUT = 0, 1, 2
CNDP_FWD_EDGE_NONE = 0xFFFF
CNDP_FWD_STAT_DIRECT, CNDP_FWD_STAT_GATEWAY, CNDP_FWD_STAT_ARP_REQUEST = 0, 1, 2

CNDP_TX_UDP, CNDP_TX_IP4 = 0, 1
CNDP_TX_EDGE_PKT_DROP, CNDP_TX_EDGE_ARP_REQUEST, CNDP_TX_EDGE_OUTPUT = 0, 1, 2
CNDP_TX_EDGE_NONE = 0xFFFF
(CNDP_TX_STAT_SENT, CNDP_TX_STAT_ARP_REQUEST, CNDP_TX_STAT_DROP_HEADROOM, CNDP_TX_STAT_DROP_NOROUTE,
 CNDP_TX_STAT_DROP_PROTO, CNDP_TX_STAT_CKSUM) = range(6)
CNDP_TX_NSTATS = 6


def CNDP_L4_EDGE(node: int, e: int) -> int:
    return (node << 4) | e


MS_RSS_KEY = bytes.fromhex(
    "6d5a56da255b0ec24167253d43a38fb0d0ca2bcbae7b30b477cb2da38030f20c6a42b73bbeac01fa")


class _Dir24(Structure):
    _fields_ = [("nh_sz", c_int), ("num_tbl8", c_uint32)]


class _ConfU(Union):
    _fields_ = [("dir24_8", _Dir24), ("trie", _Dir24)]


class FibConf(Structure):
    _anonymous_ = ("u",)
    _fields_ = [("type", c_int), ("default_nh", c_uint64), ("max_routes", c_int), ("u", _ConfU)]


class FibImage(Structure):
    _fields_ = [("nh_sz", c_uint32), ("tbl8_groups", c_uint32), ("tbl24", c_void_p),
                ("tbl8", c_void_p), ("def_nh", c_uint64)]


class Batch(Structure):
    _fields_ = [("mode", c_uint32), ("n", c_uint32), ("slab", c_void_p), ("slab_len", c_uint64),
                ("stride", c_uint64), ("offsets", c_void_p), ("data_off", c_uint32),
                ("buf_len", c_uint32), ("nh", c_void_p), ("hash", c_void_p), ("queue", c_void_p),
                ("edge", c_void_p), ("bins", c_void_p), ("n_bins", c_uint32), ("ptype", c_void_p),
                ("rxmeta", c_void_p)]


class MqConf(Structure):
    _fields_ = [("mode", c_uint32), ("flags", c_uint32), ("batch", c_uint32), ("depth", c_uint32),
                ("max_delay_us", c_uint32), ("stage_max", c_uint32), ("umem", c_void_p),
                ("lport", c_uint16), ("rsvd", c_uint16 * 3), ("metadata", c_void_p)]


class PcbEntry(Structure):
    _fields_ = [("laddr", c_uint32), ("faddr", c_uint32), ("lport", c_uint16), ("fport", c_uint16),
                ("opt_flag", c_uint16)]


class L4Io(Structure):
    _fields_ = [("sel", c_void_p), ("l4edge", c_void_p), ("pcb", c_void_p), ("ports", c_void_p),
                ("payload_off", c_void_p), ("bin_of", c_void_p), ("n_bins", c_uint32),
                ("stats", c_void_p)]


class TcpIo(Structure):
    _fields_ = [("sel", c_void_p), ("l4edge", c_void_p), ("pcb", c_void_p), ("ports", c_void_p),
                ("seg", c_void_p), ("bin_of", c_void_p), ("n_bins", c_uint32), ("stats", c_void_p)]


class Tcb(Structure):
    _fields_ = [("rcv_nxt", c_uint32), ("snd_una", c_uint32), ("snd_nxt", c_uint32), ("snd_max", c_uint32),
                ("snd_wnd", c_uint32), ("snd_cwnd", c_uint32), ("ts_recent", c_uint32),
                ("last_ack_sent", c_uint32), ("rcv_space", c_uint32), ("max_mss", c_uint16), ("state", c_uint8),
                ("snd_scale", c_uint8), ("flags", c_uint8), ("rsvd", c_uint8 * 7)]


class TcpSegIo(Structure):
    _fields_ = [("sel", c_void_p), ("l4edge", c_void_p), ("pcb", c_void_p), ("seg", c_void_p),
                ("opt", c_void_p), ("verdict", c_void_p), ("stats", c_void_p)]


class TcbTx(Structure):
    _fields_ = [("tflags", c_uint8), ("req_recv_scale", c_uint8), ("rcv_scale", c_uint8), ("rsvd", c_uint8)]


class TcpOutIo(Structure):
    _fields_ = [("sel", c_void_p), ("pcb", c_void_p), ("txseg", c_void_p), ("seg", c_void_p), ("verdict", c_void_p),
                ("rxmeta", c_void_p), ("snd", c_void_p), ("snd_len", c_uint64), ("src_off", c_void_p),
                ("len", c_void_p), ("faddr", c_void_p), ("laddr", c_void_p), ("taken", c_void_p),
                ("stats", c_void_p)]


class FwdArp(Structure):
    _fields_ = [("netif_idx", c_uint16), ("ha", c_uint8 * 6)]


class FwdRt(Structure):
    _fields_ = [("gateway", c_uint32), ("netif_idx", c_uint16)]


class FwdIo(Structure):
    _fields_ = [("sel", c_void_p), ("fwd_edge", c_void_p), ("arp_idx", c_void_p), ("bin_of", c_void_p),
                ("n_bins", c_uint32), ("stats", c_void_p)]


class PcbTx(Structure):
    _fields_ = [("tos", c_uint8), ("ttl", c_uint8), ("ip_proto", c_uint8)]


class TxIo(Structure):
    _fields_ = [("sel", c_void_p), ("pcb", c_void_p), ("faddr", c_void_p), ("laddr", c_void_p),
                ("ports", c_void_p), ("len", c_void_p), ("tx_edge", c_void_p), ("bin_of", c_void_p),
                ("n_bins", c_uint32), ("stats", c_void_p)]


class NativeLibraryMissing(RuntimeError):
    pass


_lib = None


def lib():
    global _lib
    if _lib is not None:
        return _lib
    if not os.path.exists(LIB_PATH):
        raise NativeLibraryMissing(
            f"{LIB_PATH} is missing: build it with `python -c 'import __graft_entry__ as g; g.build()'`"
            " (no CPU fallback exists)")
    L = ctypes.CDLL(LIB_PATH)
    sig = {
        "cne_fib_create": (c_void_p, [c_char_p, POINTER(FibConf)]),
        "cne_fib_free": (None, [c_void_p]),
        "cne_fib_add": (c_int, [c_void_p, c_uint32, c_uint8, c_uint64]),
        "cne_fib_delete": (c_int, [c_void_p, c_uint32, c_uint8]),
        "cne_fib_lookup_bulk": (c_int, [c_void_p, c_void_p, c_void_p, c_int]),
        "cne_fib_get_dp": (c_void_p, [c_void_p]),
        "cne_fib_get_rib": (c_void_p, [c_void_p]),
        "cne_fib_select_lookup": (c_int, [c_void_p, c_int]),
        "cne_fib6_create": (c_void_p, [c_char_p, POINTER(FibConf)]),
        "cne_fib6_free": (None, [c_void_p]),
        "cne_fib6_add": (c_int, [c_void_p, c_void_p, c_uint8, c_uint64]),
        "cne_fib6_delete": (c_int, [c_void_p, c_void_p, c_uint8]),
        "cne_fib6_lookup_bulk": (c_int, [c_void_p, c_void_p, c_void_p, c_int]),
        "cne_fib6_get_dp": (c_void_p, [c_void_p]),
        "cne_fib6_get_rib": (c_void_p, [c_void_p]),
        "cne_fib6_select_lookup": (c_int, [c_void_p, c_int]),
        "cndp_fib_image": (c_int, [c_void_p, POINTER(FibImage)]),
        "cndp_fib6_image": (c_int, [c_void_p, POINTER(FibImage)]),
        "cndp_fib_sync": (c_int, [c_void_p, c_void_p]),
        "cndp_fib6_sync": (c_int, [c_void_p, c_void_p]),
        "cndp_fib_lookup_dev": (c_int, [c_void_p, c_void_p, c_void_p, c_uint32, c_void_p]),
        "cndp_fib6_lookup_dev": (c_int, [c_void_p, c_void_p, c_void_p, c_uint32, c_void_p]),
        "cndp_fib_stats": (c_int, [c_void_p, POINTER(c_uint32), POINTER(c_uint32), POINTER(c_uint32)]),
        "cndp_fib6_stats": (c_int, [c_void_p, POINTER(c_uint32), POINTER(c_uint32), POINTER(c_uint32)]),
        "cndp_fib_sync_stats": (c_int, [c_void_p, POINTER(c_uint64), POINTER(c_uint64)]),
        "cndp_fib6_sync_stats": (c_int, [c_void_p, POINTER(c_uint64), POINTER(c_uint64)]),
        "cne_node_ip4_route_add": (c_int, [c_uint32, c_uint8, c_uint16, c_int]),
        "cne_node_ip4_rewrite_add": (c_int, [c_uint16, c_void_p, c_uint8, c_uint16]),
        "ip4_rewrite_set_next": (c_int, [c_uint16, c_uint16]),
        "cne_node_ip4_add_input": (c_int, [c_void_p, c_uint32, c_uint8, c_uint32]),
        "cne_node_ip6_add_input": (c_int, [c_void_p, c_void_p, c_uint8, c_uint32]),
        "cndp_node_ip4_lookup_init": (c_int, []),
        "cndp_node_ip4_lookup_fib": (c_void_p, []),
        "cndp_node_ip4_lookup_fini": (None, []),
        "cndp_node_ip4_rewrite_get": (c_int, [c_uint16, c_void_p, POINTER(c_uint16), POINTER(c_uint16),
                                              POINTER(c_uint16)]),
        "cndp_node_ip4_rewrite_reset": (None, []),
        "cndp_node_gpu_umem_add": (c_int, [c_void_p, c_uint64]),
        "cndp_node_gpu_umem_get": (c_int, [c_uint32, POINTER(c_void_p), POINTER(c_uint64)]),
        "cndp_node_gpu_umem_reset": (None, []),
        "cndp_gpu_init": (c_int, [c_int, POINTER(c_void_p)]),
        "cndp_gpu_fini": (None, [c_void_p]),
        "cndp_gpu_device": (c_int, [c_void_p]),
        "cndp_gpu_set_rss": (c_int, [c_void_p, c_char_p, c_uint32, c_void_p, c_uint32, c_uint32]),
        "cndp_gpu_set_fib": (c_int, [c_void_p, c_void_p, c_void_p]),
        "cndp_gpu_classify": (c_int, [c_void_p, POINTER(Batch), c_void_p]),
        "cndp_gpu_stream_release": (c_int, [c_void_p, c_void_p]),
        "cndp_gpu_classify_host": (c_int, [c_void_p, POINTER(Batch)]),
        "cndp_gpu_host_register": (c_int, [c_void_p, c_void_p, c_uint64, POINTER(c_void_p)]),
        "cndp_gpu_host_unregister": (c_int, [c_void_p, c_void_p]),
        "cndp_gpu_frames_alloc": (c_int, [c_int, c_uint64, c_uint32, POINTER(c_void_p)]),
        "cndp_gpu_frames_free": (c_int, [c_void_p]),
        "cndp_gpu_l3fwd_mbufs": (c_int, [c_void_p, c_void_p, c_uint32, c_void_p, c_void_p]),
        "cndp_gpu_ip4_rewrite_set_next": (c_int, [c_void_p, c_uint16, c_uint16]),
        "cndp_gpu_ip4_rewrite_add": (c_int, [c_void_p, c_uint16, c_void_p, c_uint8, c_uint16]),
        "cndp_gpu_ip4_rewrite": (c_int, [c_void_p, POINTER(Batch), c_uint32, c_void_p, c_void_p]),
        "cndp_gpu_mac_swap": (c_int, [c_void_p, POINTER(Batch), c_void_p]),
        "cndp_gpu_classify_rewrite": (c_int, [c_void_p, POINTER(Batch), c_uint32, c_void_p, c_void_p]),
        "cndp_gpu_bin_partition": (c_int, [c_void_p, c_void_p, c_uint32, c_uint32, c_void_p,
                                           c_void_p, c_void_p]),
        "cndp_gpu_bin_ids": (c_int, [c_void_p, c_uint32, c_void_p, c_void_p, c_void_p, c_uint32,
                                     c_uint32, c_void_p, c_void_p]),
        "cndp_gpu_set_tuning": (c_int, [c_void_p, c_int, c_int]),
        "cndp_gpu_mq_create": (c_int, [c_void_p, POINTER(MqConf), POINTER(c_void_p)]),
        "cndp_gpu_mq_free": (None, [c_void_p]),
        "cndp_gpu_mq_submit": (c_int, [c_void_p, c_void_p, c_uint32]),
        "cndp_gpu_mq_flush": (c_int, [c_void_p]),
        "cndp_gpu_mq_poll": (c_int, [c_void_p, c_void_p, c_void_p, c_uint32]),
        "cndp_gpu_mq_wait": (c_int, [c_void_p]),
        "cndp_gpu_mq_pending": (c_uint32, [c_void_p]),
        "cndp_gpu_mq_stat": (ctypes.c_int64, [c_void_p, c_int]),
        "cndp_gpu_get_stat": (ctypes.c_int64, [c_void_p, c_int]),
        "cndp_gpu_version": (c_char_p, []),
        "cndp_pcb_create": (c_int, [c_uint32, POINTER(c_void_p)]),
        "cndp_pcb_free": (None, [c_void_p]),
        "cndp_pcb_add": (c_int, [c_void_p, POINTER(PcbEntry)]),
        "cndp_pcb_del": (c_int, [c_void_p, c_uint32]),
        "cndp_pcb_set_flags": (c_int, [c_void_p, c_int, c_int]),
        "cndp_pcb_count": (c_int, [c_void_p]),
        "cndp_pcb_lookup": (c_int, [c_void_p, c_void_p, c_uint32, c_void_p]),
        "cndp_gpu_udp_input": (c_int, [c_void_p, c_void_p, POINTER(Batch), POINTER(L4Io), c_void_p]),
        "cndp_pcb_lookup_indexed": (c_int, [c_void_p, c_void_p, c_uint32, c_void_p]),
        "cndp_gpu_tcp_input": (c_int, [c_void_p, c_void_p, POINTER(Batch), POINTER(TcpIo), c_void_p]),
        "cndp_tcb_tbl_create": (c_int, [c_void_p, POINTER(c_void_p)]),
        "cndp_tcb_tbl_destroy": (None, [c_void_p]),
        "cndp_tcb_set": (c_int, [c_void_p, c_uint32, POINTER(Tcb)]),
        "cndp_tcb_clear": (c_int, [c_void_p, c_uint32]),
        "cndp_tcb_get": (c_int, [c_void_p, c_uint32, POINTER(Tcb)]),
        "cndp_gpu_tcp_segment": (c_int, [c_void_p, c_void_p, POINTER(Batch), POINTER(TcpSegIo), c_uint32, c_void_p]),
        "cndp_tcp_segment_host": (c_int, [c_void_p, c_uint32, POINTER(Batch), POINTER(TcpSegIo)]),
        "cndp_tcb_tx_set": (c_int, [c_void_p, c_uint32, POINTER(TcbTx)]),
        "cndp_tcb_tx_get": (c_int, [c_void_p, c_uint32, POINTER(TcbTx)]),
        "cndp_tcp_output_host": (c_int, [c_void_p, c_uint32, c_uint32, c_void_p, c_uint64, c_uint64, c_void_p,
                                         c_uint32, c_uint32, POINTER(TcpOutIo)]),
        "cndp_tcp_send_optlen": (c_uint32, [c_uint8, c_uint8]),
        "cndp_fwd_create": (c_int, [c_void_p, c_void_p, c_uint32, c_uint32, POINTER(c_void_p)]),
        "cndp_fwd_free": (None, [c_void_p]),
        "cndp_fwd_arp_set": (c_int, [c_void_p, c_uint32, POINTER(FwdArp)]),
        "cndp_fwd_arp_clear": (c_int, [c_void_p, c_uint32]),
        "cndp_fwd_rt_set": (c_int, [c_void_p, c_uint32, POINTER(FwdRt)]),
        "cndp_fwd_rt_clear": (c_int, [c_void_p, c_uint32]),
        "cndp_fwd_netif_set": (c_int, [c_void_p, c_uint32, c_void_p]),
        "cndp_fwd_max_netif": (c_int, [c_void_p]),
        "cndp_fwd_lookup": (c_int, [c_void_p, c_void_p, c_uint32, c_void_p]),
        "cndp_gpu_ip4_forward": (c_int, [c_void_p, c_void_p, POINTER(Batch), c_uint32, POINTER(FwdIo), c_void_p]),
        "cndp_pcb_tx_set": (c_int, [c_void_p, c_uint32, POINTER(PcbTx)]),
        "cndp_pcb_tx_get": (c_int, [c_void_p, c_uint32, POINTER(PcbTx)]),
        "cndp_fwd_netif_ident_set": (c_int, [c_void_p, c_uint32, c_uint16]),
        "cndp_fwd_netif_ident_get": (c_int, [c_void_p, c_uint32, POINTER(c_uint16)]),
# ... 36 lines not shown
```

include/cndp_fib.h:

```cpp
#ifndef CNDP_FIB_H
#define CNDP_FIB_H

#include <stdint.h>

#ifdef __cplusplus
extern "C" {
#endif

struct cne_fib;
struct cne_fib6;
struct cne_rib;
struct cne_rib6;

#ifndef CNE_FIB6_MAXDEPTH
#define CNE_FIB6_MAXDEPTH 128
#endif

#ifndef _CNE_FIB_H_
#define _CNE_FIB_H_
#define CNE_FIB_MAXDEPTH 32
#define IPV6_ADDR_LEN 16

enum cne_fib_type {
    CNE_FIB_DUMMY,
// ... 16 lines not shown
    CNE_FIB_DIR24_8_2B,
    CNE_FIB_DIR24_8_4B,
    CNE_FIB_DIR24_8_8B,
};

enum cne_fib_trie_nh_sz { CNE_FIB_TRIE_2B = 1, CNE_FIB_TRIE_4B, CNE_FIB_TRIE_8B };

enum cne_fib_lookup_type {
    CNE_FIB_LOOKUP_DEFAULT,
    CNE_FIB_LOOKUP_DIR24_8_SCALAR_MACRO,
    CNE_FIB_LOOKUP_DIR24_8_SCALAR_INLINE,
    CNE_FIB_LOOKUP_DIR24_8_SCALAR_UNI,
    CNE_FIB_LOOKUP_DIR24_8_VECTOR_AVX512,
    CNE_FIB_LOOKUP_TRIE_SCALAR,
    CNE_FIB_LOOKUP_TRIE_VECTOR_AVX512,
    CNE_FIB_LOOKUP_GPU
};

struct cne_fib_conf {
    enum cne_fib_type type;
    uint64_t default_nh;
    int max_routes;
    union {
        struct {
            enum cne_fib_dir24_8_nh_sz nh_sz;
            uint32_t num_tbl8;
        } dir24_8;
        struct {
            enum cne_fib_trie_nh_sz nh_sz;
            uint32_t num_tbl8;
        } trie;
    };
};
#endif
#ifndef _CNE_FIB6_H_
#define _CNE_FIB6_H_
#endif
#define CNDP_FIB_LOOKUP_GPU 7

struct cne_fib *cne_fib_create(const char *name, struct cne_fib_conf *conf);
void cne_fib_free(struct cne_fib *fib);
int cne_fib_add(struct cne_fib *fib, uint32_t ip, uint8_t depth, uint64_t next_hop);
int cne_fib_delete(struct cne_fib *fib, uint32_t ip, uint8_t depth);
int cne_fib_lookup_bulk(struct cne_fib *fib, uint32_t *ips, uint64_t *next_hops, int n);
void *cne_fib_get_dp(struct cne_fib *fib);
struct cne_rib *cne_fib_get_rib(struct cne_fib *fib);
int cne_fib_select_lookup(struct cne_fib *fib, enum cne_fib_lookup_type type);

struct cne_fib6 *cne_fib6_create(const char *name, struct cne_fib_conf *conf);
void cne_fib6_free(struct cne_fib6 *fib);
int cne_fib6_add(struct cne_fib6 *fib, const uint8_t ip[IPV6_ADDR_LEN], uint8_t depth,
                 uint64_t next_hop);
int cne_fib6_delete(struct cne_fib6 *fib, const uint8_t ip[IPV6_ADDR_LEN], uint8_t depth);
int cne_fib6_lookup_bulk(struct cne_fib6 *fib, uint8_t ips[][IPV6_ADDR_LEN], uint64_t *next_hops,
                         int n);
void *cne_fib6_get_dp(struct cne_fib6 *fib);
struct cne_rib6 *cne_fib6_get_rib(struct cne_fib6 *fib);
int cne_fib6_select_lookup(struct cne_fib6 *fib, enum cne_fib_lookup_type type);

struct cndp_fib_image {
    uint32_t nh_sz;
    uint32_t tbl8_groups;
    const void *tbl24;
    const void *tbl8;
    uint64_t def_nh;
};
int cndp_fib_image(struct cne_fib *fib, struct cndp_fib_image *out);
int cndp_fib6_image(struct cne_fib6 *fib, struct cndp_fib_image *out);

int cndp_fib_sync(struct cne_fib *fib, void *stream);
int cndp_fib6_sync(struct cne_fib6 *fib, void *stream);

int cndp_fib_lookup_dev(struct cne_fib *fib, const uint32_t *ips, uint64_t *next_hops, uint32_t n,
                        void *stream);
int cndp_fib6_lookup_dev(struct cne_fib6 *fib, const uint8_t *ips16, uint64_t *next_hops,
                         uint32_t n, void *stream);

int cndp_fib_stats(struct cne_fib *fib, uint32_t *routes, uint32_t *tbl8_used, uint32_t *rsvd);
int cndp_fib6_stats(struct cne_fib6 *fib, uint32_t *routes, uint32_t *tbl8_used, uint32_t *rsvd);

int cndp_fib_sync_stats(struct cne_fib *fib, uint64_t *bytes, uint64_t *cmds);
int cndp_fib6_sync_stats(struct cne_fib6 *fib, uint64_t *bytes, uint64_t *cmds);

#ifdef __cplusplus
}
#endif
#endif
```

include/cndp_gpu.h:

```cpp
#ifndef CNDP_GPU_H
#define CNDP_GPU_H

#include <stdint.h>

#include "cndp_fib.h"

#ifdef __cplusplus
extern "C" {
#endif

#define CNDP_MODE_L3FWD 0u
#define CNDP_MODE_CNET 1u
#define CNDP_MODE_HASH 2u

#define CNDP_NH_INVALID 0xFFFFFFFFu
#define CNDP_EDGE_CLS_DROP 0xFFu
#define CNDP_RSS_KEY_LEN 40u
#define CNDP_RETA_MAX 512u
#define CNDP_BINS_MAX 1024u
#define CNDP_PART_BINS_MAX 4096u

typedef struct cndp_gpu_ctx cndp_gpu_ctx_t;

struct cndp_batch {
// ... 46 lines not shown
#define CNDP_MQ_F_HASH (1u << 0)
#define CNDP_MQ_F_NO_METADATA (1u << 1)
#define CNDP_MQ_F_DEVICE_HEADERS (1u << 2)
#define CNDP_MQ_F_RX_PARSE (1u << 3)
#define CNDP_MQ_EDGE_CLS_DROP 0xFFFEu
#define CNDP_MQ_F_REWRITE (1u << 4)
#define CNDP_MQ_F_HOST_WRITEBACK (1u << 5)
#define CNDP_MQ_EDGE_LOOKUP_DROP 0xFFFDu
#define CNDP_MQ_NODE_PTYPE 0u
#define CNDP_MQ_NODE_IP4 1u
#define CNDP_MQ_NODE_IP6 2u
#define CNDP_MQ_EDGE(node, e) ((uint16_t)(((node) << 8) | (e)))
#define CNDP_MQ_EDGE_NONE 0xFFFFu
#define CNDP_MQ_DEPTH_MAX 16u

struct cndp_mq_conf {
    uint32_t mode;
    uint32_t flags;
    uint32_t batch;
    uint32_t depth;
    uint32_t max_delay_us;
    uint32_t stage_max;
    void *umem;
    uint16_t lport;
    uint16_t rsvd[3];
    void *(*metadata)(const void *m);
};

int cndp_gpu_mq_create(cndp_gpu_ctx_t *ctx, const struct cndp_mq_conf *conf, cndp_gpu_mq_t **out);
void cndp_gpu_mq_free(cndp_gpu_mq_t *q);
int cndp_gpu_mq_submit(cndp_gpu_mq_t *q, void *const *mbufs, uint32_t n);
int cndp_gpu_mq_flush(cndp_gpu_mq_t *q);
int cndp_gpu_mq_poll(cndp_gpu_mq_t *q, void **mbufs, uint16_t *edges, uint32_t max);
int cndp_gpu_mq_wait(cndp_gpu_mq_t *q);
uint32_t cndp_gpu_mq_pending(const cndp_gpu_mq_t *q);
#define CNDP_MQ_STAT_BATCHES 1
#define CNDP_MQ_STAT_MBUFS 2
int64_t cndp_gpu_mq_stat(const cndp_gpu_mq_t *q, int key);

int cndp_gpu_ip4_rewrite_set_next(cndp_gpu_ctx_t *ctx, uint16_t port_id, uint16_t next_index);
int cndp_gpu_ip4_rewrite_add(cndp_gpu_ctx_t *ctx, uint16_t next_hop, const uint8_t *rewrite_data,
                             uint8_t rewrite_len, uint16_t dst_port);
int cndp_gpu_ip4_rewrite(cndp_gpu_ctx_t *ctx, const struct cndp_batch *b, uint32_t burst,
                         uint16_t *tx_edge, void *stream);

int cndp_gpu_classify_rewrite(cndp_gpu_ctx_t *ctx, const struct cndp_batch *b, uint32_t burst,
                              uint16_t *tx_edge, void *stream);

int cndp_gpu_mac_swap(cndp_gpu_ctx_t *ctx, const struct cndp_batch *b, void *stream);

int cndp_gpu_host_register(cndp_gpu_ctx_t *ctx, void *ptr, uint64_t len, void **dev_ptr);
int cndp_gpu_host_unregister(cndp_gpu_ctx_t *ctx, void *ptr);

#define CNDP_FRAMES_CACHED 1u
int cndp_gpu_frames_alloc(int device, uint64_t bytes, uint32_t flags, void **dptr);
int cndp_gpu_frames_free(void *dptr);

int cndp_gpu_bin_partition(cndp_gpu_ctx_t *ctx, const uint16_t *bin_of, uint32_t n,
                           uint32_t n_bins, uint32_t *bin_start, uint32_t *order, void *stream);

int cndp_gpu_bin_ids(cndp_gpu_ctx_t *ctx, uint32_t mode, const uint32_t *nh, const uint8_t *edge,
                     const uint16_t *queue, uint32_t n, uint32_t n_bins, uint16_t *bin_of,
                     void *stream);

#define CNDP_TUNE_NT 1
#define CNDP_TUNE_UNROLL 2
#define CNDP_TUNE_BLOCKS_PER_CU 3
#define CNDP_TUNE_TILE 4
#define CNDP_TUNE_DIR16 5
#define CNDP_TUNE_CNET_TILE 6
#define CNDP_TUNE_HOST_CHUNK 7
#define CNDP_TUNE_RW_WB 8
#define CNDP_TUNE_CNET_SPEC 9
#define CNDP_TUNE_LOAD_NT 10
#define CNDP_TUNE_SPEC_SCAN 11
#define CNDP_TUNE_MBUF_HASH 12
#define CNDP_TUNE_CNET_FOLD 13
#define CNDP_TUNE_SPEC_GRID 14
#define CNDP_TUNE_SPEC_LISTS 15
#define CNDP_TUNE_SPEC_TYPES 16
#define CNDP_TUNE_STREAM_BAL 17
#define CNDP_TUNE_SPEC_WAIT 18
#define CNDP_TUNE_HOST_WINDOW 19
int cndp_gpu_set_tuning(cndp_gpu_ctx_t *ctx, int key, int value);

#define CNDP_STAT_CNET_WORKLIST 1
#define CNDP_STAT_CNET_UNIFORM 2
#define CNDP_STAT_SPEC_ERR 3
int64_t cndp_gpu_get_stat(cndp_gpu_ctx_t *ctx, int key);

const char *cndp_gpu_version(void);

#ifdef __cplusplus
}
#endif
#endif
```

Before: 80670 Mpps.

## Stage compact multi-level FIB image in LDS for stream classify kernel

Adds a host-built compact near image of the LPM table (a top-level 256-entry directory, mid-level pages, and dir16 pages) that fits in shared memory. A new stream kernel copies this image into LDS per block and resolves the first three LPM levels from LDS, going to global memory only for the tbl8 level. The aim is to cut random global-memory lookups per packet for small route sets. The cost is a per-block LDS fill, higher LDS use that may lower occupancy, and extra host-side table maintenance. The path is on by default and is guarded by a fits check.

```diff
diff --git a/__graft_entry__.py b/__graft_entry__.py
--- a/__graft_entry__.py
+++ b/__graft_entry__.py
@@ -22,6 +22,7 @@
     subprocess.run(["make", "-C", os.path.join(ROOT, "tests", "tx_host")], check=True, env=env)
     subprocess.run(["make", "-C", os.path.join(ROOT, "tests", "tcb_host")], check=True, env=env)
     subprocess.run(["make", "-C", os.path.join(ROOT, "tests", "tcpout_host")], check=True, env=env)
+    subprocess.run(["make", "-C", os.path.join(ROOT, "tests", "fib_near_host")], check=True, env=env)
     if ROOT not in sys.path:
         sys.path.insert(0, ROOT)
     import cndp_amd
diff --git a/cndp_amd/classify.py b/cndp_amd/classify.py
--- a/cndp_amd/classify.py
+++ b/cndp_amd/classify.py
@@ -49,11 +49,11 @@
                    cnet_fold: int | None = None, spec_grid: int | None = None,
                    spec_lists: int | None = None, spec_types: int | None = None,
                    stream_bal: int | None = None, spec_wait: int | None = None,
-                   host_window: int | None = None):
+                   host_window: int | None = None, fib_lds: int | None = None):
         for key, v in ((N.CNDP_TUNE_CNET_FOLD, cnet_fold), (N.CNDP_TUNE_SPEC_GRID, spec_grid),
                        (N.CNDP_TUNE_SPEC_WAIT, spec_wait), (N.CNDP_TUNE_HOST_WINDOW, host_window),
                        (N.CNDP_TUNE_SPEC_LISTS, spec_lists), (N.CNDP_TUNE_SPEC_TYPES, spec_types),
-                       (N.CNDP_TUNE_STREAM_BAL, stream_bal),
+                       (N.CNDP_TUNE_STREAM_BAL, stream_bal), (N.CNDP_TUNE_FIB_LDS, fib_lds),
                        (N.CNDP_TUNE_NT, nt), (N.CNDP_TUNE_UNROLL, unroll),
                        (N.CNDP_TUNE_BLOCKS_PER_CU, blocks_per_cu), (N.CNDP_TUNE_TILE, tile),
                        (N.CNDP_TUNE_DIR16, dir16), (N.CNDP_TUNE_CNET_TILE, cnet_tile),
diff --git a/cndp_amd/csrc/cndp_gpu.hip b/cndp_amd/csrc/cndp_gpu.hip
--- a/cndp_amd/csrc/cndp_gpu.hip
+++ b/cndp_amd/csrc/cndp_gpu.hip
@@ -162,6 +162,12 @@
     const struct cndp_rw_nh *rw_tbl;
     uint16_t *tx_edge;
     uint32_t rw_parts;
+};
+
+struct NearArgs {
+    const uint32_t *img;
+    uint32_t n_mid;
+    uint32_t n_pages;
 };
 
 #define FAST_THREADS 256
@@ -743,6 +749,8 @@
 
 
 #define STREAM_BW 8
+#define CNDP_FIB_LDS_DEFAULT 1
+#define CNDP_FIB_LDS_SD 2
 template <int MODE, bool NTS, bool LNT>
 __global__ __launch_bounds__(STREAM_BW * 64) void k_classify_stream_bal(KArgs a, uint64_t n_tiles)
 {
@@ -821,6 +829,208 @@
             q1 = q2;
             q2 = qn;
         }
+    }
+    const uint64_t done = n_tiles * 64u;
+    for (uint64_t i = done + (uint64_t)blockIdx.x * NT + tid; i < a.n; i += (uint64_t)gridDim.x * NT) {
+        FastHdr h;
+        fast_load<false>(a, i, h);
+        fast_finish<MODE, false>(a, i, h, s_t, s_reta, s_bins, count);
+    }
+    if (count) {
+        __syncthreads();
+        for (uint32_t k = tid; k < a.n_bins + 2; k += NT)
+            if (s_bins[k])
+                atomicAdd(&a.bins[k], (unsigned long long)s_bins[k]);
+    }
+}
+
+struct ImgLane {
+    uint32_t et, hs;
+    uint32_t e;
+    uint32_t raw;
+};
+
+template <bool NTS, bool LNT, int P, int SD>
+__device__ __forceinline__ void stream_trip_img(const KArgs &a, uint64_t n_tiles, uint64_t c, uint64_t cn, uint64_t cd,
+                                                bool dD, uint32_t lane, u32x4 *tile, u32x4 (&r)[2][4],
+                                                ImgLane (&st)[SD], const uint32_t *s_t, const uint16_t *s_reta,
+                                                uint32_t *s_bins, bool count, const uint32_t *s_img,
+                                                uint32_t pg_off)
+{
+    constexpr int MODE = CNDP_MODE_L3FWD;
+    const uint8_t *base = a.slab + a.data_off;
+    const uint32_t fr_in_k = lane >> 2, part = lane & 3u;
+    const ImgLane od = st[SD - 1];
+    uint32_t nhD = CNDP_NH_INVALID;
+    if (od.et == 0x0800u)
+        nhD = ((od.e & 1u) ? od.raw : od.e) >> 1;
+#pragma unroll
+    for (uint32_t k = 0; k < 4; k++) {
+        const uint32_t f = 16u * k + fr_in_k;
+        tile[f * 4u + (part ^ ((f >> 2) & 3u))] = r[P][k];
+    }
+    __builtin_amdgcn_wave_barrier();
+    const uint32_t sw = (lane >> 2) & 3u;
+    const u32x4 p0 = tile[lane * 4u + (0u ^ sw)];
+    const u32x4 p1 = tile[lane * 4u + (1u ^ sw)];
+    const u32x4 p2 = tile[lane * 4u + (2u ^ sw)];
+    __builtin_amdgcn_wave_barrier();
+    FastHdr h;
+    const uint64_t i = (c < n_tiles ? c : n_tiles - 1u) * 64u + lane;
+    h.p = base + i * 64u;
+    h.avail = a.slab_len - (a.data_off + i * 64u);
+    h.w3 = p0.w;
+    h.w5 = p1.y;
+    h.w6 = p1.z;
+    h.w7 = p1.w;
+    h.w8 = p2.x;
+    h.w9 = p2.y;
+    const uint32_t et = bswap16(h.w3 & 0xffffu);
+    const uint32_t dst = alignb(h.w8, h.w7, 2);
+    const uint32_t ip = bswap32(dst);
+    ImgLane nb;
+    nb.et = et;
+    uint32_t e = 0;
+    if (et == 0x0800u) {
+        e = s_img[ip >> 24];
+        if (e & 1u)
+            e = s_img[256u + (e >> 1) * 256u + ((ip >> 16) & 0xffu)];
+        if (e & 1u)
+            e = s_img[pg_off + (e >> 1) * 256u + ((ip >> 8) & 0xffu)];
+    }
+    nb.e = e;
+    nb.raw = a.tbl8[(e & 1u) ? (e >> 1) * 256u + (ip & 0xffu) : 0u];
+    nb.hs = 0;
+    bool slow = et == 0x86DDu;
+    if (et == 0x0800u) {
+        const uint32_t ihl = (h.w3 >> 16) & 0xfu;
+        const uint32_t proto = h.w5 >> 24;
+        const uint32_t frag = bswap16(h.w5 & 0xffffu) & 0x3fffu;
+        nb.hs = tz4(s_t, 0, alignb(h.w7, h.w6, 2)) ^ tz4(s_t, 4, dst);
+        if (ihl >= 5 && (proto == 6u || proto == 17u) && frag == 0) {
+            if (ihl == 5)
+                nb.hs ^= tz4(s_t, 8, alignb(h.w9, h.w8, 2));
+            else
+                slow = true;
+        }
+    }
+    if (slow)
+        nb.hs = fast_hash<MODE>(a, h, s_t);
+    {
+        const u32x4 *g = (const u32x4 *)(base + (cn < n_tiles ? cn : n_tiles - 1u) * 4096u);
+        r[P][0] = ldg4<LNT>((const uint8_t *)(g + lane));
+        r[P][1] = ldg4<LNT>((const uint8_t *)(g + 64 + lane));
+        r[P][2] = ldg4<LNT>((const uint8_t *)(g + 128 + lane));
+        r[P][3] = ldg4<LNT>((const uint8_t *)(g + 192 + lane));
+    }
+    if (dD)
+        fast_emit<MODE, NTS>(a, cd * 64u + lane, od.et, nhD, od.hs, s_reta, s_bins, count);
+#pragma unroll
+    for (int k = SD - 1; k > 0; k--)
+        st[k] = st[k - 1];
+    st[0] = nb;
+}
+
+static int stream_img_init(void);
+static void stream_img_launch(bool nts, uint32_t blocks, uint32_t lds, hipStream_t s, const KArgs &a,
+                              uint64_t n_tiles, const NearArgs &nr);
+
+extern __shared__ __attribute__((aligned(16))) uint32_t s_near_img[];
+
+template <bool NTS, bool LNT, int SD>
+__global__ __launch_bounds__(STREAM_BW * 64) void k_classify_stream_img(KArgs a, uint64_t n_tiles, NearArgs nr)
+{
+    __shared__ uint32_t s_t[TAB4_POS * 256];
+    __shared__ uint16_t s_reta[CNDP_RETA_MAX];
+    __shared__ uint32_t s_bins[CNDP_BINS_MAX + 2];
+    __shared__ __attribute__((aligned(16))) u32x4 s_tile[STREAM_BW][256];
+    __shared__ uint32_t s_next;
+    constexpr uint32_t NT = STREAM_BW * 64;
+    constexpr int MODE = CNDP_MODE_L3FWD;
+
+    const uint32_t tid = threadIdx.x;
+    for (uint32_t k = tid; k < TAB4_POS * 256; k += NT)
+        s_t[k] = a.ttab[k];
+    for (uint32_t k = tid; k <= a.reta_mask; k += NT)
+        s_reta[k] = a.reta[k];
+    const bool count = a.bins != nullptr;
+    if (count)
+        for (uint32_t k = tid; k < a.n_bins + 2; k += NT)
+            s_bins[k] = 0;
+    if (tid == 0)
+        s_next = 3u * STREAM_BW;
+    const uint32_t lane = tid & 63u, wv = tid >> 6;
+    u32x4 *tile = s_tile[wv];
+    const uint8_t *base = a.slab + a.data_off;
+    const uint64_t G = gridDim.x, b = blockIdx.x;
+    const uint64_t NONE = ~0ull;
+    const uint64_t nk = b < n_tiles ? (n_tiles - b + G - 1) / G : 0;
+    auto tile_of = [&](uint64_t k) { return k < nk ? b + k * G : NONE; };
+    uint64_t q0 = tile_of(wv), q1 = tile_of(wv + STREAM_BW), q2 = tile_of(wv + 2u * STREAM_BW);
+    u32x4 r[2][4];
+#pragma unroll
+    for (uint32_t s = 0; s < 2; s++) {
+        const uint64_t ts = s ? q1 : q0;
+        const u32x4 *g = (const u32x4 *)(base + (ts < n_tiles ? ts : n_tiles - 1u) * 4096u);
+        r[s][0] = ldg4<LNT>((const uint8_t *)(g + lane));
+        r[s][1] = ldg4<LNT>((const uint8_t *)(g + 64 + lane));
+        r[s][2] = ldg4<LNT>((const uint8_t *)(g + 128 + lane));
+        r[s][3] = ldg4<LNT>((const uint8_t *)(g + 192 + lane));
+    }
+    {
+        const uint32_t n4a = 64u * (1u + nr.n_mid), n4b = 64u * nr.n_pages;
+        u32x4 *d = (u32x4 *)s_near_img;
+        const u32x4 *sa = (const u32x4 *)nr.img, *sp = (const u32x4 *)a.pages;
+        for (uint32_t k = tid; k < n4a; k += NT)
+            d[k] = sa[k];
+        for (uint32_t k = tid; k < n4b; k += NT)
+            d[n4a + k] = sp[k];
+    }
+    __syncthreads();
+    auto draw = [&](uint64_t prev) -> uint32_t {
+        uint32_t v = 0;
+        if (prev != NONE && lane == 0)
+            v = atomicAdd(&s_next, 1u);
+        return v;
+    };
+    uint32_t kv = draw(q2);
+    const uint32_t pg_off = 256u + nr.n_mid * 256u;
+    uint64_t hs[SD];
+    ImgLane st[SD];
+#pragma unroll
+    for (int k = 0; k < SD; k++) {
+        hs[k] = NONE;
+        st[k] = ImgLane{0, 0, 0, 0};
+    }
+    auto idle = [&]() {
+        bool z = q0 == NONE;
+#pragma unroll
+        for (int k = 0; k < SD; k++)
+            z = z && hs[k] == NONE;
+        return z;
+    };
+    auto advance = [&]() {
+        const uint64_t qn = q2 == NONE ? NONE : tile_of(__builtin_amdgcn_readfirstlane(kv));
+        kv = draw(qn);
+#pragma unroll
+        for (int k = SD - 1; k > 0; k--)
+            hs[k] = hs[k - 1];
+        hs[0] = q0;
+        q0 = q1;
+        q1 = q2;
+        q2 = qn;
+    };
+    for (;;) {
+        if (idle())
+            break;
+        stream_trip_img<NTS, LNT, 0, SD>(a, n_tiles, q0, q2, hs[SD - 1], hs[SD - 1] != NONE, lane, tile, r, st, s_t,
+                                         s_reta, s_bins, count, s_near_img, pg_off);
+        advance();
+        if (idle())
+            break;
+        stream_trip_img<NTS, LNT, 1, SD>(a, n_tiles, q0, q2, hs[SD - 1], hs[SD - 1] != NONE, lane, tile, r, st, s_t,
+                                         s_reta, s_bins, count, s_near_img, pg_off);
+        advance();
     }
     const uint64_t done = n_tiles * 64u;
     for (uint64_t i = done + (uint64_t)blockIdx.x * NT + tid; i < a.n; i += (uint64_t)gridDim.x * NT) {
@@ -3738,6 +3948,9 @@
     int tune_bpc;
     int tune_tile;
     int tune_dir16;
+    int tune_fib_lds;
+    int fib_lds_ok;
+    uint64_t n_fib_lds;
     int tune_cnet_tile;
     int tune_lnt;
     int tune_spec_scan;
@@ -3896,6 +4109,12 @@
     c->tune_bpc = 0;
     c->tune_tile = 1;
     c->tune_dir16 = 1;
+    {
+        const char *fe = getenv("CNDP_TUNE_FIB_LDS");
+        const int fv = fe ? atoi(fe) : CNDP_FIB_LDS_DEFAULT;
+        c->tune_fib_lds = fv < 0 || fv > 1 ? CNDP_FIB_LDS_DEFAULT : fv;
+        c->fib_lds_ok = stream_img_init();
+    }
     c->tune_cnet_tile = 1;
     c->tune_lnt = 1;
     c->tune_spec_lists = 1;
@@ -4051,6 +4270,8 @@
         hipFree(t->dev_dir16);
     if (t->dev_pages)
         hipFree(t->dev_pages);
+    if (t->dev_near)
+        hipFree(t->dev_near);
     if (t->lk_stream)
         hipStreamDestroy((hipStream_t)t->lk_stream);
     if (t->lk_dbuf)
@@ -4063,90 +4284,13 @@
     t->dev_old = nullptr;
     t->n_old = t->cap_old = 0;
     hipSetDevice(cur);
-    t->dev_dir16 = t->dev_pages = nullptr;
+    t->dev_dir16 = t->dev_pages = t->dev_near = nullptr;
     t->dev_cap_pages = 0;
     t->dev_tbl24 = t->dev_tbl8 = nullptr;
     t->dev_id = -1;
     t->dev_groups = 0;
 }
 
-static int dir16_page_alloc(struct cndp_tbl *t)
-{
-    if (t->n_free)
-        return (int)t->page_free[--t->n_free];
-    if (t->page_hwm == t->cap_pages) {
-        const uint32_t ncap = t->cap_pages ? t->cap_pages * 2 : 64;
-        uint32_t *np = (uint32_t *)realloc(t->pages, (size_t)ncap * 256 * 4);
-        uint32_t *nf = (uint32_t *)realloc(t->page_free, (size_t)ncap * 4);
-        if (!np || !nf) {
-            if (np)
-                t->pages = np;
-            if (nf)
-                t->page_free = nf;
-            return -ENOMEM;
-        }
-        t->pages = np;
-        t->page_free = nf;
-        t->cap_pages = ncap;
-    }
-    return (int)t->page_hwm++;
-}
-
-static int dir16_update(struct cndp_tbl *t, uint32_t k0, uint32_t k1)
-{
-    if (!t->dir16) {
-        t->dir16 = (uint32_t *)calloc(65536, 4);
-        t->page_of = (int32_t *)malloc(65536 * 4);
-        if (!t->dir16 || !t->page_of)
-            return -ENOMEM;
-        for (uint32_t k = 0; k < 65536; k++)
-            t->page_of[k] = -1;
-        k0 = 0;
-        k1 = 65535;
-        t->dd_lo = t->dp_lo = ~0ULL;
-        t->dd_hi = t->dp_hi = 0;
-    }
-    const uint32_t *t24 = (const uint32_t *)t->tbl24;
-    for (uint32_t k = k0; k <= k1; k++) {
-        const uint32_t *e = t24 + (size_t)k * 256;
-        const uint32_t v = e[0];
-        bool uni = !(v & 1u);
-        for (uint32_t b = 1; uni && b < 256; b++)
-            uni = e[b] == v;
-        uint32_t nd;
-        if (uni) {
-            if (t->page_of[k] >= 0) {
-                t->page_free[t->n_free++] = (uint32_t)t->page_of[k];
-                t->page_of[k] = -1;
-                t->n_pages_used--;
-            }
-            nd = v;
-        } else {
-            if (t->page_of[k] < 0) {
-                const int pg = dir16_page_alloc(t);
-                if (pg < 0)
-                    return pg;
-                t->page_of[k] = pg;
-                t->n_pages_used++;
-            }
-            const uint64_t pe = (uint64_t)t->page_of[k] * 256;
-            memcpy(t->pages + pe, e, 256 * 4);
-            if (pe < t->dp_lo)
-                t->dp_lo = pe;
-            if (pe + 256 > t->dp_hi)
-                t->dp_hi = pe + 256;
-            nd = ((uint32_t)t->page_of[k] << 1) | 1u;
-        }
-        if (t->dir16[k] != nd || t->dd_hi == 0) {
-            t->dir16[k] = nd;
-            if (k < t->dd_lo)
-                t->dd_lo = k;
-            if ((uint64_t)k + 1 > t->dd_hi)
-                t->dd_hi = (uint64_t)k + 1;
-        }
-    }
-    return 0;
-}
 
 static int tbl_dev_sweep(struct cndp_tbl *t)
 {
@@ -4180,7 +4324,7 @@
     for (uint32_t k = 0; k < nr || (!t->dir16 && k == 0); k++) {
         const uint64_t lo = k < nr ? rg[k].lo : 0, hi = k < nr ? rg[k].hi : 0;
         if (hi > lo || !t->dir16) {
-            int r = dir16_update(t, (uint32_t)(lo >> 8), (uint32_t)((hi ? hi - 1 : 0) >> 8));
+            int r = cndp_tbl_dir16_update(t, (uint32_t)(lo >> 8), (uint32_t)((hi ? hi - 1 : 0) >> 8));
             if (r)
                 return r;
         }
@@ -4209,6 +4353,26 @@
                                (t->dp_hi - t->dp_lo) * 4, hipMemcpyHostToDevice, s));
     t->dd_lo = t->dp_lo = ~0ULL;
     t->dd_hi = t->dp_hi = 0;
+    return 0;
+}
+
+static int near_upload(struct cndp_tbl *t, hipStream_t s, bool *copied)
+{
+    if (!t->near_img)
+        return 0;
+    if (!t->dev_near) {
+        HIP_TRY(hipMalloc(&t->dev_near, (size_t)CNDP_NEAR_ENT * 4));
+        HIP_TRY(hipMemsetAsync(t->dev_near, 0, (size_t)CNDP_NEAR_ENT * 4, s));
+        t->dn_lo = 0;
+        t->dn_hi = 256u + (uint64_t)t->mid_hwm * 256u;
+    }
+    if (t->dn_hi > t->dn_lo) {
+        HIP_TRY(hipMemcpyAsync((uint32_t *)t->dev_near + t->dn_lo, t->near_img + t->dn_lo,
+                               (t->dn_hi - t->dn_lo) * 4, hipMemcpyHostToDevice, s));
+        *copied = true;
+    }
+    t->dn_lo = ~0ULL;
+    t->dn_hi = 0;
     return 0;
 }
 
@@ -4361,7 +4525,7 @@
     return 1;
 }
 
-static int tbl_dev_sync_locked(struct cndp_tbl *t, void *stream)
+static int tbl_dev_sync_locked(struct cndp_tbl *t, void *stream, bool near = false)
 {
     if (!t || !t->tbl24)
         return -EINVAL;
@@ -4430,7 +4594,15 @@
         if (r)
             return r;
     }
-    if (dirty)
+    bool near_up = false;
+    if (near && has_dir16) {
+        int r = cndp_tbl_near_refresh(t);
+        if (!r && cndp_tbl_near_fits(t))
+            r = near_upload(t, s, &near_up);
+        if (r)
+            return r;
+    }
+    if (dirty || near_up)
         HIP_TRY(hipStreamSynchronize(s));
     t->d24_lo = t->d8_lo = ~0ULL;
     t->d24_hi = t->d8_hi = 0;
@@ -4457,17 +4629,21 @@
     const void *t24, *t8;
     uint32_t nh_sz;
     const uint32_t *d16, *pages;
+    const uint32_t *near;
+    uint32_t n_mid, page_hwm;
 };
 static inline TblView tbl_view(const struct cndp_tbl *t)
 {
     const bool dir = t->dev_dir16 && t->dev_pages;
+    const bool near = dir && t->dev_near && t->dn_hi <= t->dn_lo && cndp_tbl_near_fits(t);
     return TblView{t->dev_tbl24, t->dev_tbl8, t->nh_sz, dir ? (const uint32_t *)t->dev_dir16 : nullptr,
-                   dir ? (const uint32_t *)t->dev_pages : nullptr};
-}
-static int tbl_acquire(struct cndp_tbl *t, hipStream_t s, TblView *v)
+                   dir ? (const uint32_t *)t->dev_pages : nullptr, near ? (const uint32_t *)t->dev_near : nullptr,
+                   near ? t->mid_hwm : 0u, near ? t->page_hwm : 0u};
+}
+static int tbl_acquire(struct cndp_tbl *t, hipStream_t s, TblView *v, bool near = false)
 {
     pthread_mutex_lock(&t->dev_lock);
-    const int r = tbl_dev_sync_locked(t, s);
+    const int r = tbl_dev_sync_locked(t, s, near);
     if (!r) {
         *v = tbl_view(t);
         __atomic_add_fetch(&t->views, 1u, __ATOMIC_RELAXED);
@@ -4802,8 +4978,8 @@
 }
 
 static int classify_cnet(cndp_gpu_ctx_t *c, const struct cndp_batch *b, KArgs &a, hipStream_t s);
-static int classify_l3(cndp_gpu_ctx_t *c, const struct cndp_batch *b, KArgs &a, hipStream_t s, uint16_t *rw_tx,
-                       bool *fused);
+static int classify_l3(cndp_gpu_ctx_t *c, const struct cndp_batch *b, KArgs &a, const NearArgs &nr, hipStream_t s,
+                       uint16_t *rw_tx, bool *fused);
 
 static int classify_launch(cndp_gpu_ctx_t *c, const struct cndp_batch *b, void *stream, uint16_t *rw_tx,
                            bool *fused, const TblView *v4, const TblView *v6);
@@ -4820,7 +4996,8 @@
     struct cndp_tbl *t4 = b->mode != CNDP_MODE_HASH ? &c->fib4->t : nullptr;
     struct cndp_tbl *t6 = b->mode == CNDP_MODE_CNET ? &c->fib6->t : nullptr;
     TblView v4{}, v6{};
-    if (t4 && (r = tbl_acquire(t4, (hipStream_t)stream, &v4)))
+    const bool near = b->mode == CNDP_MODE_L3FWD && c->tune_fib_lds && c->fib_lds_ok && c->tune_dir16;
+    if (t4 && (r = tbl_acquire(t4, (hipStream_t)stream, &v4, near)))
         return r;
     if (t6 && (r = tbl_acquire(t6, (hipStream_t)stream, &v6))) {
         tbl_release(t4);
@@ -4840,6 +5017,7 @@
     int r;
     KArgs a;
     memset(&a, 0, sizeof(a));
+    NearArgs nr{nullptr, 0, 0};
     a.slab = (const uint8_t *)b->slab;
     a.slab_len = b->slab_len;
     a.stride = b->stride;
@@ -4854,6 +5032,8 @@
         if (c->tune_dir16 && v4->d16) {
             a.dir16 = v4->d16;
             a.pages = v4->pages;
+            if (v4->near)
+                nr = NearArgs{v4->near, v4->n_mid, v4->page_hwm};
         }
     }
     if (v6) {
@@ -4880,7 +5060,7 @@
         const int r2 = scratch_release(c, s);
         return r ? r : r2;
     }
-    return classify_l3(c, b, a, s, rw_tx, fused);
+    return classify_l3(c, b, a, nr, s, rw_tx, fused);
 }
 
 static int classify_cnet(cndp_gpu_ctx_t *c, const struct cndp_batch *b, KArgs &a, hipStream_t s)
@@ -5031,8 +5211,8 @@
     return 0;
 }
 
-static int classify_l3(cndp_gpu_ctx_t *c, const struct cndp_batch *b, KArgs &a, hipStream_t s, uint16_t *rw_tx,
-                       bool *fused)
+static int classify_l3(cndp_gpu_ctx_t *c, const struct cndp_batch *b, KArgs &a, const NearArgs &nr, hipStream_t s,
+                       uint16_t *rw_tx, bool *fused)
 {
     {
         uint32_t g = blocks_for(b->n, FAST_THREADS);
@@ -5062,6 +5242,17 @@
                 *fused = true;
                 hipLaunchKernelGGL(rfns[nti][li], dim3(gt), dim3(FAST_THREADS), 0, s, a, n_tiles);
                 HIP_TRY(hipGetLastError());
+                return 0;
+            }
+            if (c->tune_stream_bal != 1 && c->tune_fib_lds && c->fib_lds_ok && li && nr.img &&
+                b->mode == CNDP_MODE_L3FWD) {
+                const uint32_t lds = (1u + nr.n_mid + nr.n_pages) * 1024u;
+                uint32_t gb = (uint32_t)c->num_cu * (c->tune_bpc ? (uint32_t)c->tune_bpc : 1u);
+                if ((uint64_t)gb > n_tiles)
+                    gb = (uint32_t)n_tiles;
+                stream_img_launch(nti != 0, gb, lds, s, a, n_tiles, nr);
+                HIP_TRY(hipGetLastError());
+                __atomic_add_fetch(&c->n_fib_lds, 1u, __ATOMIC_RELAXED);
                 return 0;
             }
             if (c->tune_stream_bal != 1) {
@@ -7332,6 +7523,8 @@
 
 extern "C" int64_t cndp_gpu_get_stat(cndp_gpu_ctx_t *c, int key)
 {
+    if (c && key == CNDP_STAT_FIB_LDS)
+        return (int64_t)__atomic_load_n(&c->n_fib_lds, __ATOMIC_RELAXED);
     if (!c || (key != CNDP_STAT_CNET_WORKLIST && key != CNDP_STAT_CNET_UNIFORM && key != CNDP_STAT_SPEC_ERR))
         return -EINVAL;
     if (!c->sp_hint)
@@ -7422,6 +7615,11 @@
     case CNDP_TUNE_HOST_WINDOW:
         c->tune_host_window = value ? 1 : 0;
         return 0;
+    case CNDP_TUNE_FIB_LDS:
+        if (value < 0 || value > 1)
+            return -EINVAL;
+        c->tune_fib_lds = value;
+        return 0;
     case CNDP_TUNE_SPEC_WAIT:
         if (value == 0 || value < -1 || value > 40000000)
             return -EINVAL;
@@ -7458,3 +7656,24 @@
 #endif
 
 extern "C" const char *cndp_gpu_version(void) { return CNDP_VERSION; }
+
+typedef void (*stream_img_fn)(KArgs, uint64_t, NearArgs);
+static const stream_img_fn stream_img_fns[2] = {k_classify_stream_img<false, true, CNDP_FIB_LDS_SD>,
+                                                k_classify_stream_img<true, true, CNDP_FIB_LDS_SD>};
+
+static int stream_img_init(void)
+{
+    int ok = 1;
+    for (int k = 0; k < 2; k++)
+        if (hipFuncSetAttribute((const void *)stream_img_fns[k], hipFuncAttributeMaxDynamicSharedMemorySize,
+                                (int)(CNDP_NEAR_CAP_KIB * 1024u)) != hipSuccess)
+            ok = 0;
+    (void)hipGetLastError();
+    return ok;
+}
+
+static void stream_img_launch(bool nts, uint32_t blocks, uint32_t lds, hipStream_t s, const KArgs &a,
+                              uint64_t n_tiles, const NearArgs &nr)
+{
+    hipLaunchKernelGGL(stream_img_fns[nts ? 1 : 0], dim3(blocks), dim3(STREAM_BW * 64), lds, s, a, n_tiles, nr);
+}
diff --git a/cndp_amd/csrc/fib.c b/cndp_amd/csrc/fib.c
--- a/cndp_amd/csrc/fib.c
+++ b/cndp_amd/csrc/fib.c
@@ -131,6 +131,7 @@
     free(t->page_of);
     free(t->pages);
     free(t->page_free);
+    free(t->near_img);
     pthread_mutex_destroy(&t->dev_lock);
     memset(t, 0, sizeof(*t));
 }
diff --git a/cndp_amd/csrc/fib_internal.h b/cndp_amd/csrc/fib_internal.h
--- a/cndp_amd/csrc/fib_internal.h
+++ b/cndp_amd/csrc/fib_internal.h
@@ -52,6 +52,13 @@
     void *dev_dir16;
     void *dev_pages;
     uint32_t dev_cap_pages;
+    uint32_t *near_img;
+    int16_t mid_of[256];
+    uint8_t mid_free[256];
+    uint32_t n_mid_free, n_mid_used, mid_hwm;
+    uint64_t near_stale[4];
+    uint64_t dn_lo, dn_hi;
+    void *dev_near;
     uint64_t def_nh;
     pthread_mutex_t dev_lock;
     struct cndp_lk_slot {
@@ -89,6 +96,22 @@
     struct cndp_tbl t;
 };
 
+#define CNDP_NEAR_ENT (257u * 256u)
+#define CNDP_NEAR_CAP_KIB 32u
+int cndp_tbl_dir16_update(struct cndp_tbl *t, uint32_t k0, uint32_t k1);
+int cndp_tbl_dir16_refresh(struct cndp_tbl *t);
+static inline uint32_t cndp_tbl_near_kib(const struct cndp_tbl *t)
+{
+    return 1u + t->mid_hwm + t->page_hwm;
+}
+int cndp_tbl_near_refresh(struct cndp_tbl *t);
+static inline int cndp_tbl_near_fits(const struct cndp_tbl *t)
+{
+    return t->near_img && !(t->near_stale[0] | t->near_stale[1] | t->near_stale[2] | t->near_stale[3]) &&
+           cndp_tbl_near_kib(t) <= CNDP_NEAR_CAP_KIB;
+}
+uint32_t cndp_tbl_near_lookup(const struct cndp_tbl *t, uint32_t ip);
+
 int cndp_tbl_dev_sync(struct cndp_tbl *t, void *stream);
 void cndp_tbl_dev_free(struct cndp_tbl *t);
 int cndp_tbl_lookup4_host(struct cndp_tbl *t, const uint32_t *ips, uint64_t *nh, uint32_t n);
diff --git a/cndp_amd/csrc/fib_near.c b/cndp_amd/csrc/fib_near.c
--- /dev/null
+++ b/cndp_amd/csrc/fib_near.c
@@ -0,0 +1,238 @@
+#include <errno.h>
+#include <stdlib.h>
+#include <string.h>
+
+#include "fib_internal.h"
+
+static inline int uniform256(const uint32_t *e)
+{
+    return memcmp(e, e + 1, 255 * 4) == 0;
+}
+
+static int dir16_page_alloc(struct cndp_tbl *t)
+{
+    if (t->n_free)
+        return (int)t->page_free[--t->n_free];
+    if (t->page_hwm == t->cap_pages) {
+        const uint32_t ncap = t->cap_pages ? t->cap_pages * 2 : 64;
+        uint32_t *np = (uint32_t *)realloc(t->pages, (size_t)ncap * 256 * 4);
+        if (np)
+            t->pages = np;
+        uint32_t *nf = (uint32_t *)realloc(t->page_free, (size_t)ncap * 4);
+        if (nf)
+            t->page_free = nf;
+        if (!np || !nf)
+            return -ENOMEM;
+        t->cap_pages = ncap;
+    }
+    return (int)t->page_hwm++;
+}
+
+static inline void near_dirty(struct cndp_tbl *t, uint64_t lo, uint64_t hi)
+{
+    if (lo < t->dn_lo)
+        t->dn_lo = lo;
+    if (hi > t->dn_hi)
+        t->dn_hi = hi;
+}
+
+static int near_update(struct cndp_tbl *t, uint32_t a0, uint32_t a1)
+{
+    if (!t->near_img) {
+        t->near_img = (uint32_t *)calloc(CNDP_NEAR_ENT, 4);
+        if (!t->near_img)
+            return -ENOMEM;
+        for (uint32_t a = 0; a < 256; a++)
+            t->mid_of[a] = -1;
+        t->n_mid_free = t->n_mid_used = t->mid_hwm = 0;
+        a0 = 0;
+        a1 = 255;
+        t->dn_lo = 0;
+        t->dn_hi = 256;
+    }
+    for (uint32_t a = a0; a <= a1; a++) {
+        const uint32_t *d = t->dir16 + (size_t)a * 256;
+        const uint32_t v = d[0];
+        const int uni = !(v & 1u) && uniform256(d);
+        uint32_t nt;
+        if (uni) {
+            if (t->mid_of[a] >= 0) {
+                t->mid_free[t->n_mid_free++] = (uint8_t)t->mid_of[a];
+                t->mid_of[a] = -1;
+                t->n_mid_used--;
+            }
+            nt = v;
+        } else {
+            if (t->mid_of[a] < 0) {
+                t->mid_of[a] = t->n_mid_free ? (int16_t)t->mid_free[--t->n_mid_free] : (int16_t)t->mid_hwm++;
+                t->n_mid_used++;
+            }
+            const uint32_t slot = (uint32_t)t->mid_of[a];
+            const uint64_t base = 256u + (uint64_t)slot * 256u;
+            uint32_t *m = t->near_img + base;
+            uint32_t lo = 256, hi = 0;
+            for (uint32_t b = 0; b < 256; b++)
+                if (m[b] != d[b]) {
+                    m[b] = d[b];
+                    if (b < lo)
+                        lo = b;
+                    hi = b + 1;
+                }
+            if (hi > lo)
+                near_dirty(t, base + lo, base + hi);
+            nt = (slot << 1) | 1u;
+        }
+        if (t->near_img[a] != nt) {
+            t->near_img[a] = nt;
+            near_dirty(t, a, a + 1u);
+        }
+    }
+    return 0;
+}
+
+int cndp_tbl_near_refresh(struct cndp_tbl *t)
+{
+    if (!t->dir16)
+        return 0;
+    if (!t->near_img) {
+        const int r = near_update(t, 0, 255);
+        if (r)
+            return r;
+    } else {
+        for (uint32_t w = 0; w < 4; w++)
+            for (uint64_t m = t->near_stale[w]; m; m &= m - 1) {
+                const uint32_t a = w * 64u + (uint32_t)__builtin_ctzll(m);
+                const int r = near_update(t, a, a);
+                if (r)
+                    return r;
+            }
+    }
+    memset(t->near_stale, 0, sizeof(t->near_stale));
+    return 0;
+}
+
+int cndp_tbl_dir16_update(struct cndp_tbl *t, uint32_t k0, uint32_t k1)
+{
+    if (!t->dir16) {
+        t->dir16 = (uint32_t *)calloc(65536, 4);
+        t->page_of = (int32_t *)malloc(65536 * 4);
+        if (!t->dir16 || !t->page_of)
+            return -ENOMEM;
+        for (uint32_t k = 0; k < 65536; k++)
+            t->page_of[k] = -1;
+        k0 = 0;
+        k1 = 65535;
+        t->dd_lo = t->dp_lo = ~0ULL;
+        t->dd_hi = t->dp_hi = 0;
+    }
+    const uint32_t *t24 = (const uint32_t *)(const void *)t->tbl24;
+    for (uint32_t k = k0; k <= k1; k++) {
+        const uint32_t *e = t24 + (size_t)k * 256;
+        const uint32_t v = e[0];
+        const int uni = !(v & 1u) && uniform256(e);
+        uint32_t nd;
+        if (uni) {
+            if (t->page_of[k] >= 0) {
+                t->page_free[t->n_free++] = (uint32_t)t->page_of[k];
+                t->page_of[k] = -1;
+                t->n_pages_used--;
+            }
+            nd = v;
+        } else {
+            if (t->page_of[k] < 0) {
+                const int pg = dir16_page_alloc(t);
+                if (pg < 0)
+                    return pg;
+                t->page_of[k] = pg;
+                t->n_pages_used++;
+            }
+            const uint64_t pe = (uint64_t)t->page_of[k] * 256;
+            memcpy(t->pages + pe, e, 256 * 4);
+            if (pe < t->dp_lo)
+                t->dp_lo = pe;
+            if (pe + 256 > t->dp_hi)
+                t->dp_hi = pe + 256;
+            nd = ((uint32_t)t->page_of[k] << 1) | 1u;
+        }
+        if (t->dir16[k] != nd || t->dd_hi == 0) {
+            t->dir16[k] = nd;
+            if (k < t->dd_lo)
+                t->dd_lo = k;
+            if ((uint64_t)k + 1 > t->dd_hi)
+                t->dd_hi = (uint64_t)k + 1;
+        }
+    }
+    for (uint32_t a = k0 >> 8; a <= k1 >> 8; a++)
+        t->near_stale[a >> 6] |= 1ULL << (a & 63u);
+    return 0;
+}
+
+int cndp_tbl_dir16_refresh(struct cndp_tbl *t)
+{
+    if (!t || !t->tbl24 || t->is_trie || t->nh_sz != 2)
+        return -ENOTSUP;
+    int r = 0;
+    if (!t->dir16)
+        r = cndp_tbl_dir16_update(t, 0, 65535);
+    else if (t->d24_hi <= t->d24_lo)
+        r = 0;
+    else if (t->n_log24 <= CNDP_TBL_LOG)
+        for (uint32_t k = 0; !r && k < t->n_log24; k++)
+            r = cndp_tbl_dir16_update(t, (uint32_t)(t->log24[k].lo >> 8), (uint32_t)((t->log24[k].hi - 1) >> 8));
+    else
+        r = cndp_tbl_dir16_update(t, (uint32_t)(t->d24_lo >> 8), (uint32_t)((t->d24_hi - 1) >> 8));
+    return r ? r : cndp_tbl_near_refresh(t);
+}
+
+uint32_t cndp_tbl_near_lookup(const struct cndp_tbl *t, uint32_t ip)
+{
+    uint32_t e = t->near_img[ip >> 24];
+    if (e & 1u)
+        e = t->near_img[256u + (e >> 1) * 256u + ((ip >> 16) & 0xffu)];
+    if (e & 1u)
+        e = t->pages[(size_t)(e >> 1) * 256u + ((ip >> 8) & 0xffu)];
+    if (e & 1u)
+        e = ((const uint32_t *)(const void *)t->tbl8)[(size_t)(e >> 1) * 256u + (ip & 0xffu)];
+    return e >> 1;
+}
+
+int cndp_fib_near_refresh(struct cne_fib *fib)
+{
+    if (!fib)
+        return -EINVAL;
+    pthread_mutex_lock(&fib->t.dev_lock);
+    const int r = cndp_tbl_dir16_refresh(&fib->t);
+    pthread_mutex_unlock(&fib->t.dev_lock);
+    return r;
+}
+
+int cndp_fib_near_info(struct cne_fib *fib, struct cndp_fib_near_info *out)
+{
+    if (!fib || !out)
+        return -EINVAL;
+    struct cndp_tbl *t = &fib->t;
+    pthread_mutex_lock(&t->dev_lock);
+    const int have = t->near_img != NULL;
+    out->kib = have ? cndp_tbl_near_kib(t) : 0;
+    out->cap_kib = CNDP_NEAR_CAP_KIB;
+    out->mid_used = t->n_mid_used;
+    out->mid_hwm = t->mid_hwm;
+    out->pages_used = t->n_pages_used;
+    out->page_hwm = t->page_hwm;
+    out->fits = (uint32_t)cndp_tbl_near_fits(t);
+    pthread_mutex_unlock(&t->dev_lock);
+    return have ? 0 : -ENOENT;
+}
+
+int cndp_fib_near_lookup(struct cne_fib *fib, const uint32_t *ips, uint64_t *next_hops, uint32_t n)
+{
+    if (!fib || (n && (!ips || !next_hops)))
+        return -EINVAL;
+    struct cndp_tbl *t = &fib->t;
+    pthread_mutex_lock(&t->dev_lock);
+    int r = cndp_tbl_dir16_refresh(t);
+    for (uint32_t i = 0; !r && i < n; i++)
+        next_hops[i] = cndp_tbl_near_lookup(t, ips[i]);
+    pthread_mutex_unlock(&t->dev_lock);
+    return r;
+}
diff --git a/cndp_amd/fib.py b/cndp_amd/fib.py
--- a/cndp_amd/fib.py
+++ b/cndp_amd/fib.py
@@ -79,6 +79,19 @@
         t8 = np.ctypeslib.as_array((ctypes.c_uint8 * (im.tbl8_groups * 256 * esz)).from_address(im.tbl8))
         return t24.view(dt), t8.view(dt)
 
+    def near_info(self) -> dict:
+        N.check(self._L.cndp_fib_near_refresh(self.h), "cndp_fib_near_refresh")
+        im = N.FibNearInfo()
+        N.check(self._L.cndp_fib_near_info(self.h, ctypes.byref(im)), "cndp_fib_near_info")
+        return {k: getattr(im, k) for k, _ in N.FibNearInfo._fields_}
+
+    def near_lookup(self, ips) -> np.ndarray:
+        ips = np.ascontiguousarray(ips, dtype=np.uint32)
+        out = np.zeros(len(ips), dtype=np.uint64)
+        N.check(self._L.cndp_fib_near_lookup(self.h, ips.ctypes.data, out.ctypes.data, len(ips)),
+                "cndp_fib_near_lookup")
+        return out
+
     def stats(self):
         r, u, s = ctypes.c_uint32(), ctypes.c_uint32(), ctypes.c_uint32()
         N.check(self._L.cndp_fib_stats(self.h, ctypes.byref(r), ctypes.byref(u), ctypes.byref(s)),
diff --git a/cndp_amd/native.py b/cndp_amd/native.py
--- a/cndp_amd/native.py
+++ b/cndp_amd/native.py
@@ -33,12 +33,14 @@
 CNDP_TUNE_LOAD_NT = 10
 CNDP_TUNE_SPEC_SCAN = 11
 CNDP_STAT_CNET_WORKLIST, CNDP_STAT_CNET_UNIFORM, CNDP_STAT_SPEC_ERR = 1, 2, 3
+CNDP_STAT_FIB_LDS = 4
 CNDP_TUNE_MBUF_HASH = 12
 CNDP_TUNE_CNET_FOLD = 13
 CNDP_TUNE_SPEC_GRID = 14
 CNDP_TUNE_SPEC_LISTS = 15
 CNDP_TUNE_SPEC_TYPES = 16
 CNDP_TUNE_STREAM_BAL = 17
+CNDP_TUNE_FIB_LDS = 20
 CNDP_TUNE_SPEC_WAIT = 18
 CNDP_TUNE_HOST_WINDOW = 19
 CNDP_MQ_IP4_LOOKUP, CNDP_MQ_CNET, CNDP_MQ_MAC_SWAP, CNDP_MQ_IP4_REWRITE = 0, 1, 2, 3
@@ -126,6 +128,11 @@
 class FibImage(Structure):
     _fields_ = [("nh_sz", c_uint32), ("tbl8_groups", c_uint32), ("tbl24", c_void_p),
                 ("tbl8", c_void_p), ("def_nh", c_uint64)]
+
+
+class FibNearInfo(Structure):
+    _fields_ = [("kib", c_uint32), ("cap_kib", c_uint32), ("fits", c_uint32), ("mid_used", c_uint32),
+                ("mid_hwm", c_uint32), ("pages_used", c_uint32), ("page_hwm", c_uint32)]
 
 
 class Batch(Structure):
@@ -247,6 +254,9 @@
         "cndp_fib6_stats": (c_int, [c_void_p, POINTER(c_uint32), POINTER(c_uint32), POINTER(c_uint32)]),
         "cndp_fib_sync_stats": (c_int, [c_void_p, POINTER(c_uint64), POINTER(c_uint64)]),
         "cndp_fib6_sync_stats": (c_int, [c_void_p, POINTER(c_uint64), POINTER(c_uint64)]),
+        "cndp_fib_near_refresh": (c_int, [c_void_p]),
+        "cndp_fib_near_info": (c_int, [c_void_p, POINTER(FibNearInfo)]),
+        "cndp_fib_near_lookup": (c_int, [c_void_p, c_void_p, c_void_p, c_uint32]),
         "cne_node_ip4_route_add": (c_int, [c_uint32, c_uint8, c_uint16, c_int]),
         "cne_node_ip4_rewrite_add": (c_int, [c_uint16, c_void_p, c_uint8, c_uint16]),
         "ip4_rewrite_set_next": (c_int, [c_uint16, c_uint16]),
diff --git a/include/cndp_fib.h b/include/cndp_fib.h
--- a/include/cndp_fib.h
+++ b/include/cndp_fib.h
@@ -122,6 +122,15 @@
 int cndp_fib_sync_stats(struct cne_fib *fib, uint64_t *bytes, uint64_t *cmds);
 int cndp_fib6_sync_stats(struct cne_fib6 *fib, uint64_t *bytes, uint64_t *cmds);
 
+struct cndp_fib_near_info {
+    uint32_t kib, cap_kib, fits;
+    uint32_t mid_used, mid_hwm;
+    uint32_t pages_used, page_hwm;
+};
+int cndp_fib_near_refresh(struct cne_fib *fib);
+int cndp_fib_near_info(struct cne_fib *fib, struct cndp_fib_near_info *out);
+int cndp_fib_near_lookup(struct cne_fib *fib, const uint32_t *ips, uint64_t *next_hops, uint32_t n);
+
 #ifdef __cplusplus
 }
 #endif
diff --git a/include/cndp_gpu.h b/include/cndp_gpu.h
--- a/include/cndp_gpu.h
+++ b/include/cndp_gpu.h
@@ -152,11 +152,13 @@
 #define CNDP_TUNE_STREAM_BAL 17
 #define CNDP_TUNE_SPEC_WAIT 18
 #define CNDP_TUNE_HOST_WINDOW 19
+#define CNDP_TUNE_FIB_LDS 20
 int cndp_gpu_set_tuning(cndp_gpu_ctx_t *ctx, int key, int value);
 
 #define CNDP_STAT_CNET_WORKLIST 1
 #define CNDP_STAT_CNET_UNIFORM 2
 #define CNDP_STAT_SPEC_ERR 3
+#define CNDP_STAT_FIB_LDS 4
 int64_t cndp_gpu_get_stat(cndp_gpu_ctx_t *ctx, int key);
 
 const char *cndp_gpu_version(void);
```

New measurement: 84250 Mpps (median of 6 runs). +4.4%, better.
